# mohammadasim98/mv-ldm

Hardware: AMD Instinct MI355X
Metric: denoised views/sec @ 256x256, 4 views, 50 DDIM steps (higher is better)
Workload: dtype bf16

## Files before the change

### include/mvldm.h

```cpp
#ifndef MVLDM_H
#define MVLDM_H

#include <stddef.h>
#include <stdint.h>

#ifdef __cplusplus
extern "C" {
#endif

#define MVLDM_ABI_VERSION 7

typedef void* mvldm_stream_t;

enum { MVLDM_F32 = 0, MVLDM_BF16 = 1, MVLDM_F16 = 2 };
enum { MVLDM_OK = 0, MVLDM_ERR_ARG = -1, MVLDM_ERR_HIP = -2, MVLDM_ERR_UNSUPPORTED = -3 };

enum { MVLDM_EPI_NONE = 0, MVLDM_EPI_SILU = 1, MVLDM_EPI_GEGLU = 2, MVLDM_EPI_GELU = 3  };
enum { MVLDM_ELT_COPY = 0, MVLDM_ELT_SILU = 1, MVLDM_ELT_GELU = 2 };

int mvldm_abi_version(void);
int mvldm_build_flags(void);
const char* mvldm_last_error(void);
int mvldm_device_info(int* cu_count, size_t* hbm_bytes, char* arch, int arch_len);

typedef struct mvldm_igemm_desc {
    const void* src0;
    const void* src1;
    const void* weight;
    const float* bias;
    const float* row_bias;
    const void* residual;
    void* dst;
    float* workspace;
    int32_t c0, c1;
    int32_t n_img, h_in, w_in, h_out, w_out;
    int32_t ksize, stride, pad, upsample;
    int32_t n_out, n_pad, k_pad;
    int32_t row_bias_ld;
    int32_t epilogue;
    int32_t act_dtype;
    int32_t dst_dtype;
    int32_t splitk;
    int32_t tile;
    int32_t k_order;
    int32_t dst_ld;
    float out_scale;
    size_t workspace_bytes;
} mvldm_igemm_desc;
int mvldm_igemm_fwd(const mvldm_igemm_desc* d, mvldm_stream_t stream);
size_t mvldm_igemm_workspace_bytes(const mvldm_igemm_desc* d);

int mvldm_pack_weight(const float* src, void* dst, int n_out, int c_in, int ksize, int c_pad, int n_pad,
                      int k_pad, int geglu, int k_order, int dst_dtype, int transpose, int c_off, int n_rows,
                      mvldm_stream_t stream);

int mvldm_pack_skinny(const void* packed, void* dst, int n_pad, int k_pad, int geglu, int dtype, mvldm_stream_t stream);
int mvldm_igemm_skinny_config(const mvldm_igemm_desc* d);

typedef struct mvldm_pack_job {
    const float* src; void* dst;
    int n_out, c_in, ksize, c_pad, n_pad, k_pad, geglu, k_order, transpose, c_off, n_rows;
    int kind;
    int blocks;
    int block0;
} mvldm_pack_job;
int mvldm_pack_job_prepare(mvldm_pack_job* job , int dst_dtype);
int mvldm_pack_weight_batch(const mvldm_pack_job* jobs , int n_jobs, const int32_t* block_job, int total_blocks,
                            int dst_dtype, mvldm_stream_t stream);

#define MVLDM_GN_MAX_CHUNKS 32
int mvldm_groupnorm_fwd(const void* x0, const void* x1, void* y, const float* gamma, const float* beta, int n_img,
                        int hw, int c0, int c1, int groups, float eps, int silu, int dtype, void* stats_ws,
                        float* stats_out, mvldm_stream_t stream);
int mvldm_groupnorm_passes(int n_img, int hw, int c, int groups, int dtype);

int mvldm_layernorm_fwd(const void* x, void* y, const float* gamma, const float* beta, int rows, int c, float eps,
                        int dtype, mvldm_stream_t stream);

int mvldm_attention_fwd(const void* q, const void* k, const void* v, void* out, int ld_q, int ld_k, int ld_v,
                        int ld_o, int heads, int head_dim, const int32_t* seg, int n_seg, int max_q_len,
                        float scale, int dtype, float* lse, int lse_ld, mvldm_stream_t stream);

int mvldm_timestep_embed_fwd(const int64_t* timesteps, const float* freqs, void* out, int n, int dim,
                             int flip_sin_to_cos, int dst_dtype, mvldm_stream_t stream);

int mvldm_eltwise_fwd(const void* x, void* y, size_t n, int op, int src_dtype, int dst_dtype, mvldm_stream_t stream);

int mvldm_ddim_cfg_step(const float* eps, const float* x_t, float* x_next, const int32_t* cond_img,
                        const int32_t* uncond_img, int n_tgt, int hw, int c, float cfg_scale, const float* coef,
                        const int32_t* step_ptr, void* unet_in, int unet_in_c, int unet_in_dtype, int n_steps,
                        float clip_range, mvldm_stream_t stream);
int mvldm_ddpm_cfg_step(const float* eps_c, const float* eps_u, const float* x_t, const float* noise, float* x_next, size_t n,
                        float cfg_scale, const float* coef, float clip_range, mvldm_stream_t stream);
int mvldm_ddim_advance(int32_t* step_ptr, const int64_t* t_table, int n_steps, int64_t* timesteps,
                       const int32_t* tgt_rows, int n_rows, mvldm_stream_t stream);

int mvldm_nchw_to_nhwc(const float* src, void* dst, int n_img, int c, int hw, int dst_c, int dst_c_off,
                       int dst_dtype, float scale, float shift, const int32_t* img_map, mvldm_stream_t stream);
int mvldm_nhwc_to_nchw(const void* src, float* dst, int n_img, int c, int hw, int src_c, int src_c_off,
                       int src_dtype, float scale, float shift, int clamp01, mvldm_stream_t stream);

enum { MVLDM_RAYS_RAW = 0, MVLDM_RAYS_POSITIONAL = 1, MVLDM_RAYS_SRT = 2 };
int mvldm_ray_channels(int mode, int n_origin_octaves, int n_dir_octaves);
int mvldm_ray_encode(const float* extrinsics, const float* intrinsics, int n_cam, int h, int w, float* out_nchw,
                     void* out_nhwc, int nhwc_c, int nhwc_c_off, int nhwc_dtype, const int32_t* img_map, int mode,
                     int n_origin_octaves, int n_dir_octaves, int plucker, mvldm_stream_t stream);

int mvldm_posterior_sample(const float* moments, const float* noise, float* out, int n, int c, int hw, float scale,
                           mvldm_stream_t stream);


typedef struct mvldm_wgrad_desc {
    const void* src0; const void* src1; const void* dy;
    float* grad;
    float* workspace; size_t workspace_bytes;
    int32_t c0, c1, c_in;
    int32_t n_img, h_in, w_in, h_out, w_out;
    int32_t ksize, stride, pad, upsample;
    int32_t n_out, dy_ld;
    int32_t act_dtype;
    int32_t accumulate;
} mvldm_wgrad_desc;
int mvldm_igemm_wgrad(const mvldm_wgrad_desc* d, mvldm_stream_t stream);

int mvldm_colsum(const void* x, float* dst, float* workspace, size_t workspace_bytes, int n_seg, int rows_per_seg, int n,
                 int ld, int ld_dst, int per_seg, int accumulate, int dtype, mvldm_stream_t stream);

#define MVLDM_NORM_BWD_STORE 0x100
int mvldm_groupnorm_bwd(const void* x0, const void* x1, const void* dy, void* dx0, void* dx1, const float* gamma,
                        const float* beta, const float* stats, float* dgamma, float* dbeta, int n_img, int hw, int c0,
                        int c1, int groups, int silu, int dtype, float* workspace, size_t workspace_bytes,
                        mvldm_stream_t stream);
int mvldm_layernorm_bwd(const void* x, const void* dy, void* dx, const float* gamma, float* dgamma, float* dbeta,
                        int rows, int c, float eps, int dtype, float* workspace, size_t workspace_bytes,
                        mvldm_stream_t stream);

typedef struct mvldm_attn_bwd_desc {
    const void* q; const void* k; const void* v; const void* out; const void* dout;
    void* dq; void* dk; void* dv;
    const float* lse; float* delta;
    const int32_t* seg;
    int32_t ld_q, ld_k, ld_v, ld_o, ld_do, ld_dq, ld_dk, ld_dv;
    int32_t heads, head_dim, n_seg, max_q_len, max_kv_len, total_q_rows, stat_ld, dtype;
    float scale;
} mvldm_attn_bwd_desc;
int mvldm_attention_bwd(const mvldm_attn_bwd_desc* d, mvldm_stream_t stream);

enum { MVLDM_TE_SILU_BWD = 0, MVLDM_TE_ADD = 1, MVLDM_TE_GEGLU_FWD = 2, MVLDM_TE_GEGLU_BWD = 3, MVLDM_TE_GELU_BWD = 4 };
int mvldm_train_eltwise(int op, const void* a, const void* b, void* out, size_t rows, int d, int a_dtype, int dtype,
                        mvldm_stream_t stream);
int mvldm_pool2x2_sum(const void* du, void* dx, int n_img, int h, int w, int c, int dtype, mvldm_stream_t stream);
int mvldm_zero_insert2x(const void* x, void* out, int n_img, int h, int w, int c, int dtype, mvldm_stream_t stream);

int mvldm_add_noise(const float* x0, const float* noise, const float* coef, void* dst, int n, int c, int hw, int dst_c,
                    int dst_c_off, int dst_dtype, const int32_t* img_map, mvldm_stream_t stream);
int mvldm_mse_loss(const float* pred, const float* noise, const int32_t* tgt_img, int n_tgt, int hw, int c, float* loss,
                   int accumulate, float loss_scale, void* dpred, int dpred_c, int dpred_dtype, float grad_scale,
                   double* workspace, mvldm_stream_t stream);

typedef struct mvldm_amp_state {
    float scale;
    int32_t growth_tracker;
    int32_t adam_step;
    int32_t found_inf;
    int32_t skipped;
    int32_t reserved[3];
} mvldm_amp_state;
int mvldm_mse_loss_amp(const float* pred, const float* noise, const int32_t* tgt_img, int n_tgt, int hw, int c, float* loss,
                       int accumulate, float loss_scale, void* dpred, int dpred_c, int dpred_dtype, float grad_scale,
                       const float* amp_scale, double* workspace, mvldm_stream_t stream);

int mvldm_grad_norm(const float* g, size_t n, const float* sumsq_in, float max_norm, float* norm_out, double* workspace,
                    mvldm_stream_t stream);
int mvldm_adamw_step(float* p, const float* g, float* m, float* v, size_t n, float lr, float beta1, float beta2, float eps,
                     float weight_decay, int step, float grad_scale, const float* clip, mvldm_stream_t stream);
int mvldm_grad_norm_amp(const float* g, size_t n, const float* sumsq_in, float max_norm, float* norm_out, mvldm_amp_state* amp,
                        double* workspace, mvldm_stream_t stream);
int mvldm_adamw_step_amp(float* p, const float* g, float* m, float* v, size_t n, float lr, float beta1, float beta2, float eps,
                         float weight_decay, float grad_scale, const float* clip, const mvldm_amp_state* amp, mvldm_stream_t stream);
int mvldm_amp_update(mvldm_amp_state* amp, float growth_factor, float backoff_factor, int growth_interval, mvldm_stream_t stream);

int mvldm_ema_update(float* avg, const float* p, size_t n, float weight, mvldm_stream_t stream);

int mvldm_gather_rows(const void* src, void* dst, const int32_t* src_index, const int32_t* dst_index, int n_rows, size_t row_bytes,
                      mvldm_stream_t stream);

int mvldm_attention_merge(const void* oa, const float* lse_a, const void* ob, const float* lse_b, void* out, const int32_t* a_img,
                          const int32_t* b_img, const int32_t* out_img, int n_img, int tokens, int heads, int head_dim, int ld_a, int ld_b,
                          int ld_o, int lse_ld_a, int lse_ld_b, int dtype, mvldm_stream_t stream);

size_t mvldm_image_metrics_workspace_bytes(int n_img, int c, int h, int w);
int mvldm_image_metrics(const float* pred, const float* gt, int n_img, int c, int h, int w, int use_sample_covariance, float* psnr,
                        float* ssim, double* workspace, size_t workspace_bytes, mvldm_stream_t stream);

size_t mvldm_lpips_workspace_bytes(int n_img, int h, int w);
int mvldm_lpips_tap_slots(int h, int w, int c);
int mvldm_lpips_prep(const float* in0, const float* in1, void* dst, int n_img, int h, int w, int c_pad, int dtype, int normalize,
                     mvldm_stream_t stream);
int mvldm_lpips_relu(void* x, size_t n, int dtype, mvldm_stream_t stream);
int mvldm_lpips_tap(const void* feat, const float* weight, void* pooled, int n_img, int h, int w, int c, int dtype, double* workspace,
                    size_t workspace_bytes, int slot0, int slots_per_image, mvldm_stream_t stream);
int mvldm_lpips_fold(const double* workspace, size_t workspace_bytes, int n_img, int h, int w, float* out, mvldm_stream_t stream);

enum {
    MVLDM_OP_IGEMM = 1, MVLDM_OP_GROUPNORM, MVLDM_OP_LAYERNORM, MVLDM_OP_ATTENTION, MVLDM_OP_TIMESTEP_EMBED,
    MVLDM_OP_ELTWISE, MVLDM_OP_DDIM_STEP, MVLDM_OP_DDIM_ADVANCE, MVLDM_OP_NCHW_TO_NHWC, MVLDM_OP_NHWC_TO_NCHW,
    MVLDM_OP_MEMCPY, MVLDM_OP_RAY_ENCODE, MVLDM_OP_POSTERIOR_SAMPLE,
    MVLDM_OP_WGRAD, MVLDM_OP_ATTENTION_BWD, MVLDM_OP_GROUPNORM_BWD, MVLDM_OP_LAYERNORM_BWD, MVLDM_OP_COLSUM,
    MVLDM_OP_TRAIN_ELTWISE, MVLDM_OP_POOL2X2, MVLDM_OP_ZERO_INSERT, MVLDM_OP_ADD_NOISE, MVLDM_OP_MSE_LOSS, MVLDM_OP_FILL_ZERO,
    MVLDM_OP_PAR_BEGIN, MVLDM_OP_PAR_NEXT, MVLDM_OP_PAR_END,
// ... 68 lines not shown
```

### mv_ldm_amd/_lib.py

```python
from __future__ import annotations

import ctypes as C
from pathlib import Path

LIB_PATH = Path(__file__).resolve().parent / "csrc" / "libmvldm_hip.so"

ABI_VERSION = 7
F32, BF16, F16 = 0, 1, 2
EPI_NONE, EPI_SILU, EPI_GEGLU, EPI_GELU = 0, 1, 2, 3
RAYS_RAW, RAYS_POSITIONAL, RAYS_SRT = 0, 1, 2
ELT_COPY, ELT_SILU, ELT_GELU = 0, 1, 2
NORM_BWD_STORE = 0x100
GN_MAX_CHUNKS = 32

(OP_IGEMM, OP_GROUPNORM, OP_LAYERNORM, OP_ATTENTION, OP_TIMESTEP_EMBED, OP_ELTWISE, OP_DDIM_STEP, OP_DDIM_ADVANCE,
 OP_NCHW_TO_NHWC, OP_NHWC_TO_NCHW, OP_MEMCPY, OP_RAY_ENCODE, OP_POSTERIOR_SAMPLE,
 OP_WGRAD, OP_ATTENTION_BWD, OP_GROUPNORM_BWD, OP_LAYERNORM_BWD, OP_COLSUM, OP_TRAIN_ELTWISE, OP_POOL2X2, OP_ZERO_INSERT,
 OP_ADD_NOISE, OP_MSE_LOSS, OP_FILL_ZERO, OP_PAR_BEGIN, OP_PAR_NEXT, OP_PAR_END, OP_GATHER_ROWS, OP_ATTN_MERGE) = range(1, 30)
TE_SILU_BWD, TE_ADD, TE_GEGLU_FWD, TE_GEGLU_BWD, TE_GELU_BWD = 0, 1, 2, 3, 4

vp, i32, f32, sz = C.c_void_p, C.c_int32, C.c_float, C.c_size_t


class IgemmDesc(C.Structure):
# ... 10 lines not shown
class _GroupNorm(C.Structure):
    _fields_ = [("x", vp), ("x1", vp), ("y", vp), ("gamma", vp), ("beta", vp), ("stats_ws", vp),
                ("n_img", i32), ("hw", i32), ("c0", i32), ("c1", i32), ("groups", i32), ("silu", i32), ("dtype", i32),
                ("eps", f32), ("stats_out", vp)]


class _LayerNorm(C.Structure):
    _fields_ = [("x", vp), ("y", vp), ("gamma", vp), ("beta", vp), ("rows", i32), ("c", i32), ("dtype", i32), ("eps", f32)]


class _Attention(C.Structure):
    _fields_ = [("q", vp), ("k", vp), ("v", vp), ("out", vp), ("seg", vp),
                ("ld_q", i32), ("ld_k", i32), ("ld_v", i32), ("ld_o", i32), ("heads", i32), ("head_dim", i32),
                ("n_seg", i32), ("max_q_len", i32), ("dtype", i32), ("scale", f32), ("lse", vp), ("lse_ld", i32)]


class _Temb(C.Structure):
    _fields_ = [("timesteps", vp), ("freqs", vp), ("out", vp), ("n", i32), ("dim", i32), ("flip", i32), ("dst_dtype", i32)]


class _Eltwise(C.Structure):
    _fields_ = [("x", vp), ("y", vp), ("n", sz), ("op", i32), ("src_dtype", i32), ("dst_dtype", i32)]


class _Ddim(C.Structure):
    _fields_ = [("eps", vp), ("x_t", vp), ("x_next", vp), ("cond_img", vp), ("uncond_img", vp), ("coef", vp),
                ("step_ptr", vp), ("unet_in", vp),
                ("n_tgt", i32), ("hw", i32), ("c", i32), ("unet_in_c", i32), ("unet_in_dtype", i32), ("cfg_scale", f32),
                ("n_steps", i32), ("clip_range", f32)]


class _Advance(C.Structure):
    _fields_ = [("step_ptr", vp), ("t_table", vp), ("timesteps", vp), ("tgt_rows", vp), ("n_steps", i32), ("n_rows", i32)]


class _Layout(C.Structure):
    _fields_ = [("src", vp), ("dst", vp), ("n_img", i32), ("c", i32), ("hw", i32), ("other_c", i32),
                ("other_c_off", i32), ("dtype", i32), ("clamp01", i32), ("scale", f32), ("shift", f32), ("img_map", vp)]


class _Rays(C.Structure):
    _fields_ = [("extrinsics", vp), ("intrinsics", vp), ("out_nchw", vp), ("out_nhwc", vp), ("img_map", vp),
                ("n_cam", i32), ("h", i32), ("w", i32), ("nhwc_c", i32), ("nhwc_c_off", i32), ("nhwc_dtype", i32),
                ("mode", i32), ("n_origin_octaves", i32), ("n_dir_octaves", i32), ("plucker", i32)]


class _Posterior(C.Structure):
    _fields_ = [("moments", vp), ("noise", vp), ("out", vp), ("n", i32), ("c", i32), ("hw", i32), ("scale", f32)]


class _Memcpy(C.Structure):
    _fields_ = [("src", vp), ("dst", vp), ("bytes", sz)]


class _AttnMerge(C.Structure):
    _fields_ = [("oa", vp), ("ob", vp), ("out", vp), ("lse_a", vp), ("lse_b", vp), ("a_img", vp), ("b_img", vp), ("out_img", vp),
                ("n_img", i32), ("tokens", i32), ("heads", i32), ("head_dim", i32), ("ld_a", i32), ("ld_b", i32), ("ld_o", i32),
                ("lse_ld_a", i32), ("lse_ld_b", i32), ("dtype", i32)]


class _Gather(C.Structure):
    _fields_ = [("src", vp), ("dst", vp), ("src_index", vp), ("dst_index", vp), ("row_bytes", sz), ("n_rows", i32)]


class PackJob(C.Structure):
    _fields_ = [("src", vp), ("dst", vp), ("n_out", i32), ("c_in", i32), ("ksize", i32), ("c_pad", i32), ("n_pad", i32), ("k_pad", i32),
                ("geglu", i32), ("k_order", i32), ("transpose", i32), ("c_off", i32), ("n_rows", i32), ("kind", i32), ("blocks", i32),
                ("block0", i32)]


class WgradDesc(C.Structure):
    _fields_ = [("src0", vp), ("src1", vp), ("dy", vp), ("grad", vp), ("workspace", vp), ("workspace_bytes", sz),
                ("c0", i32), ("c1", i32), ("c_in", i32),
                ("n_img", i32), ("h_in", i32), ("w_in", i32), ("h_out", i32), ("w_out", i32),
                ("ksize", i32), ("stride", i32), ("pad", i32), ("upsample", i32),
                ("n_out", i32), ("dy_ld", i32), ("act_dtype", i32), ("accumulate", i32)]


class AttnBwdDesc(C.Structure):
    _fields_ = [("q", vp), ("k", vp), ("v", vp), ("out", vp), ("dout", vp), ("dq", vp), ("dk", vp), ("dv", vp),
                ("lse", vp), ("delta", vp), ("seg", vp),
                ("ld_q", i32), ("ld_k", i32), ("ld_v", i32), ("ld_o", i32), ("ld_do", i32), ("ld_dq", i32), ("ld_dk", i32), ("ld_dv", i32),
                ("heads", i32), ("head_dim", i32), ("n_seg", i32), ("max_q_len", i32), ("max_kv_len", i32), ("total_q_rows", i32),
                ("stat_ld", i32), ("dtype", i32), ("scale", f32)]


class _GroupNormBwd(C.Structure):
    _fields_ = [("x0", vp), ("x1", vp), ("dy", vp), ("dx0", vp), ("dx1", vp), ("gamma", vp), ("beta", vp), ("stats", vp),
                ("dgamma", vp), ("dbeta", vp), ("workspace", vp), ("workspace_bytes", sz),
                ("n_img", i32), ("hw", i32), ("c0", i32), ("c1", i32), ("groups", i32), ("silu", i32), ("dtype", i32)]


class _LayerNormBwd(C.Structure):
    _fields_ = [("x", vp), ("dy", vp), ("dx", vp), ("gamma", vp), ("dgamma", vp), ("dbeta", vp), ("workspace", vp),
                ("workspace_bytes", sz), ("rows", i32), ("c", i32), ("dtype", i32), ("eps", f32)]


class _Colsum(C.Structure):
    _fields_ = [("x", vp), ("dst", vp), ("workspace", vp), ("workspace_bytes", sz),
                ("n_seg", i32), ("rows_per_seg", i32), ("n", i32), ("ld", i32), ("ld_dst", i32), ("per_seg", i32),
                ("accumulate", i32), ("dtype", i32)]


class _TrainEltwise(C.Structure):
    _fields_ = [("a", vp), ("b", vp), ("out", vp), ("rows", sz), ("op", i32), ("d", i32), ("a_dtype", i32), ("dtype", i32)]


class _Resample(C.Structure):
    _fields_ = [("src", vp), ("dst", vp), ("n_img", i32), ("h", i32), ("w", i32), ("c", i32), ("dtype", i32)]


class _AddNoise(C.Structure):
    _fields_ = [("x0", vp), ("noise", vp), ("coef", vp), ("dst", vp), ("img_map", vp),
                ("n", i32), ("c", i32), ("hw", i32), ("dst_c", i32), ("dst_c_off", i32), ("dst_dtype", i32)]


class _Mse(C.Structure):
    _fields_ = [("pred", vp), ("noise", vp), ("tgt_img", vp), ("loss", vp), ("dpred", vp), ("workspace", vp),
                ("n_tgt", i32), ("hw", i32), ("c", i32), ("accumulate", i32), ("dpred_c", i32), ("dpred_dtype", i32),
                ("loss_scale", f32), ("grad_scale", f32), ("amp_scale", vp)]


class AmpState(C.Structure):
    _fields_ = [("scale", f32), ("growth_tracker", i32), ("adam_step", i32), ("found_inf", i32), ("skipped", i32), ("reserved", i32 * 3)]


class _Fill(C.Structure):
    _fields_ = [("dst", vp), ("bytes", sz)]


class _OpUnion(C.Union):
    _fields_ = [("igemm", IgemmDesc), ("groupnorm", _GroupNorm), ("layernorm", _LayerNorm), ("attention", _Attention),
                ("temb", _Temb), ("eltwise", _Eltwise), ("ddim", _Ddim), ("advance", _Advance), ("layout", _Layout),
                ("memcpy_", _Memcpy), ("gather", _Gather), ("attn_merge", _AttnMerge), ("rays", _Rays), ("posterior", _Posterior),
                ("wgrad", WgradDesc), ("attention_bwd", AttnBwdDesc), ("groupnorm_bwd", _GroupNormBwd),
                ("layernorm_bwd", _LayerNormBwd), ("colsum", _Colsum), ("train_eltwise", _TrainEltwise), ("resample", _Resample),
                ("add_noise", _AddNoise), ("mse", _Mse), ("fill", _Fill)]


class Op(C.Structure):
    _fields_ = [("kind", i32), ("tag", i32), ("u", _OpUnion)]


SIGNATURES = {
    "mvldm_abi_version": (C.c_int, []),
    "mvldm_build_flags": (C.c_int, []),
    "mvldm_last_error": (C.c_char_p, []),
    "mvldm_device_info": (C.c_int, [C.POINTER(C.c_int), C.POINTER(sz), C.c_char_p, C.c_int]),
    "mvldm_igemm_fwd": (C.c_int, [C.POINTER(IgemmDesc), vp]),
    "mvldm_igemm_workspace_bytes": (sz, [C.POINTER(IgemmDesc)]),
    "mvldm_pack_weight": (C.c_int, [vp, vp] + [C.c_int] * 12 + [vp]),
    "mvldm_pack_skinny": (C.c_int, [vp, vp, C.c_int, C.c_int, C.c_int, C.c_int, vp]),
    "mvldm_igemm_skinny_config": (C.c_int, [C.POINTER(IgemmDesc)]),
    "mvldm_pack_job_prepare": (C.c_int, [C.POINTER(PackJob), C.c_int]),
    "mvldm_pack_weight_batch": (C.c_int, [vp, C.c_int, vp, C.c_int, C.c_int, vp]),
    "mvldm_groupnorm_fwd": (C.c_int, [vp, vp, vp, vp, vp, C.c_int, C.c_int, C.c_int, C.c_int, C.c_int, f32, C.c_int, C.c_int, vp, vp, vp]),
    "mvldm_groupnorm_passes": (C.c_int, [C.c_int] * 5),
    "mvldm_layernorm_fwd": (C.c_int, [vp, vp, vp, vp, C.c_int, C.c_int, f32, C.c_int, vp]),
    "mvldm_attention_fwd": (C.c_int, [vp, vp, vp, vp] + [C.c_int] * 6 + [vp, C.c_int, C.c_int, f32, C.c_int, vp, C.c_int, vp]),
    "mvldm_igemm_wgrad": (C.c_int, [C.POINTER(WgradDesc), vp]),
    "mvldm_colsum": (C.c_int, [vp, vp, vp, sz] + [C.c_int] * 8 + [vp]),
    "mvldm_groupnorm_bwd": (C.c_int, [vp] * 10 + [C.c_int] * 7 + [vp, sz, vp]),
    "mvldm_layernorm_bwd": (C.c_int, [vp] * 6 + [C.c_int, C.c_int, f32, C.c_int, vp, sz, vp]),
    "mvldm_attention_bwd": (C.c_int, [C.POINTER(AttnBwdDesc), vp]),
    "mvldm_train_eltwise": (C.c_int, [C.c_int, vp, vp, vp, sz, C.c_int, C.c_int, C.c_int, vp]),
    "mvldm_pool2x2_sum": (C.c_int, [vp, vp] + [C.c_int] * 5 + [vp]),
    "mvldm_zero_insert2x": (C.c_int, [vp, vp] + [C.c_int] * 5 + [vp]),
    "mvldm_add_noise": (C.c_int, [vp, vp, vp, vp] + [C.c_int] * 6 + [vp, vp]),
    "mvldm_mse_loss": (C.c_int, [vp, vp, vp, C.c_int, C.c_int, C.c_int, vp, C.c_int, f32, vp, C.c_int, C.c_int, f32, vp, vp]),
    "mvldm_grad_norm": (C.c_int, [vp, sz, vp, f32, vp, vp, vp]),
    "mvldm_adamw_step": (C.c_int, [vp, vp, vp, vp, sz, f32, f32, f32, f32, f32, C.c_int, f32, vp, vp]),
    "mvldm_mse_loss_amp": (C.c_int, [vp, vp, vp, C.c_int, C.c_int, C.c_int, vp, C.c_int, f32, vp, C.c_int, C.c_int, f32, vp, vp, vp]),
    "mvldm_grad_norm_amp": (C.c_int, [vp, sz, vp, f32, vp, vp, vp, vp]),
    "mvldm_adamw_step_amp": (C.c_int, [vp, vp, vp, vp, sz, f32, f32, f32, f32, f32, f32, vp, vp, vp]),
    "mvldm_amp_update": (C.c_int, [vp, f32, f32, C.c_int, vp]),
    "mvldm_timestep_embed_fwd": (C.c_int, [vp, vp, vp, C.c_int, C.c_int, C.c_int, C.c_int, vp]),
    "mvldm_eltwise_fwd": (C.c_int, [vp, vp, sz, C.c_int, C.c_int, C.c_int, vp]),
    "mvldm_ddim_cfg_step": (C.c_int, [vp, vp, vp, vp, vp, C.c_int, C.c_int, C.c_int, f32, vp, vp, vp, C.c_int, C.c_int, C.c_int, f32, vp]),
    "mvldm_ddim_advance": (C.c_int, [vp, vp, C.c_int, vp, vp, C.c_int, vp]),
    "mvldm_gather_rows": (C.c_int, [vp, vp, vp, vp, C.c_int, sz, vp]),
    "mvldm_attention_merge": (C.c_int, [vp] * 8 + [C.c_int] * 10 + [vp]),
    "mvldm_ddpm_cfg_step": (C.c_int, [vp, vp, vp, vp, vp, sz, f32, vp, f32, vp]),
    "mvldm_ema_update": (C.c_int, [vp, vp, sz, f32, vp]),
    "mvldm_image_metrics_workspace_bytes": (sz, [C.c_int] * 4),
    "mvldm_image_metrics": (C.c_int, [vp, vp] + [C.c_int] * 5 + [vp, vp, vp, sz, vp]),
    "mvldm_lpips_workspace_bytes": (sz, [C.c_int] * 3),
    "mvldm_lpips_tap_slots": (C.c_int, [C.c_int] * 3),
    "mvldm_lpips_prep": (C.c_int, [vp, vp, vp] + [C.c_int] * 6 + [vp]),
    "mvldm_lpips_relu": (C.c_int, [vp, sz, C.c_int, vp]),
    "mvldm_lpips_tap": (C.c_int, [vp, vp, vp] + [C.c_int] * 5 + [vp, sz, C.c_int, C.c_int, vp]),
    "mvldm_lpips_fold": (C.c_int, [vp, sz, C.c_int, C.c_int, C.c_int, vp, vp]),
    "mvldm_nchw_to_nhwc": (C.c_int, [vp, vp] + [C.c_int] * 6 + [f32, f32, vp, vp]),
    "mvldm_ray_channels": (C.c_int, [C.c_int, C.c_int, C.c_int]),
    "mvldm_ray_encode": (C.c_int, [vp, vp, C.c_int, C.c_int, C.c_int, vp, vp, C.c_int, C.c_int, C.c_int, vp] + [C.c_int] * 4 + [vp]),
    "mvldm_posterior_sample": (C.c_int, [vp, vp, vp, C.c_int, C.c_int, C.c_int, f32, vp]),
    "mvldm_nhwc_to_nchw": (C.c_int, [vp, vp] + [C.c_int] * 6 + [f32, f32, C.c_int, vp]),
    "mvldm_op_run": (C.c_int, [C.POINTER(Op), vp]),
    "mvldm_plan_create": (C.c_int, [C.POINTER(Op), C.c_int, C.POINTER(vp)]),
    "mvldm_plan_num_ops": (C.c_int, [vp]),
    "mvldm_plan_run": (C.c_int, [vp, vp]),
    "mvldm_plan_run_range": (C.c_int, [vp, C.c_int, C.c_int, vp]),
    "mvldm_plan_capture": (C.c_int, [vp, vp]),
    "mvldm_plan_replay": (C.c_int, [vp, vp]),
    "mvldm_plan_profile": (C.c_int, [vp, vp, C.c_int, C.POINTER(f32)]),
    "mvldm_plan_destroy": (None, [vp]),
}

_lib = None


class MvldmError(RuntimeError):
    pass


_EXPERIMENT_KNOBS = ("MVLDM_ADAMW_NT", "MVLDM_ATTN_QB", "MVLDM_ATTN_WIDE_VALU", "MVLDM_GN_NTHR", "MVLDM_GN_SPAN", "MVLDM_GN_TWOPASS", "MVLDM_GN_WIDE",
                     "MVLDM_IGEMM_FAKE", "MVLDM_IGEMM_GROUP", "MVLDM_IGEMM_NOSTAGE", "MVLDM_IGEMM_PX", "MVLDM_IGEMM_SYNC", "MVLDM_IGEMM_TARGET",
                     "MVLDM_LPP_CPT", "MVLDM_LPP_FAKE", "MVLDM_PLAN_SERIAL", "MVLDM_PW_FAKE", "MVLDM_PW_GM", "MVLDM_PW_TN", "MVLDM_RS_FAKE", "MVLDM_SK_FAKE",
                     "MVLDM_STREAM_STORES", "MVLDM_WGRAD_DIRECT", "MVLDM_WGRAD_TARGET", "MVLDM_WGRAD_WIDE", "MVLDM_WGRAD_WIDE_BP",
                     "MVLDM_WGRAD_WIDE_TARGET", "MVLDM_WGRAD_XCD", "MVLDM_WS_FAKE")


def load(required: bool = True):
    global _lib
    if _lib is not None:
        return _lib
    if not LIB_PATH.exists():
        if required:
            raise MvldmError(f"{LIB_PATH} is missing: run `python -c 'import __graft_entry__ as g; g.build()'` "
                             "(there is no CPU / PyTorch fallback for the HIP path)")
        return None
    lib = C.CDLL(str(LIB_PATH))
    for name, (res, args) in SIGNATURES.items():
        fn = getattr(lib, name)
        fn.restype, fn.argtypes = res, args
    if lib.mvldm_abi_version() != ABI_VERSION:
        raise MvldmError("libmvldm_hip.so ABI version mismatch")
    if not (lib.mvldm_build_flags() & 1) and "_exp" not in LIB_PATH.name:
        import os
        stale = sorted(k for k in _EXPERIMENT_KNOBS if k in os.environ)
        if stale:
            raise MvldmError(f"{', '.join(stale)} set, but {LIB_PATH.name} was built without -DMVLDM_EXPERIMENTS and ignores it: build an "
                             "experiment library (MVLDM_EXPERIMENTS=1 python -m mv_ldm_amd._build --force, or tools/*_probe.sh + --lib) or unset it")
    _lib = lib
    return lib


def check(rc: int):
    if rc != 0:
        raise MvldmError(f"mvldm error {rc}: {load().mvldm_last_error().decode()}")
```

### mv_ldm_amd/csrc/igemm.hip

```cpp
#include <algorithm>
#include <cstdio>
#include <cstdlib>

#include "igemm_common.h"

namespace mvldm {

template <typename T> __global__ __launch_bounds__(256) void igemm_splitk_reduce(const IgemmParams p) {
    const bool geglu = p.epilogue == MVLDM_EPI_GEGLU;
    const size_t total = (size_t)p.M * p.n_dst;
    const size_t slab = (size_t)p.M * p.n_pad;
    for (size_t idx = (size_t)blockIdx.x * 256 + threadIdx.x; idx < total; idx += (size_t)gridDim.x * 256) {
        const int m = (int)(idx / p.n_dst), col = (int)(idx - (size_t)m * p.n_dst);
        float v;
        if (geglu) {
            const int nv = (col >> 5) * 64 + (col & 31), ng = nv + 32;
            float a = 0.f, g = 0.f;
            for (int s = 0; s < p.splitk; ++s) {
                a += p.ws[s * slab + (size_t)m * p.n_pad + nv];
                g += p.ws[s * slab + (size_t)m * p.n_pad + ng];
            }
            if (p.bias) { a += p.bias[col]; g += p.bias[p.n_dst + col]; }
            v = a * gelu_erf_fast(g);
        } else {
            float a = 0.f;
            for (int s = 0; s < p.splitk; ++s) a += p.ws[s * slab + (size_t)m * p.n_pad + col];
            if (p.bias) a += p.bias[col];
            if (p.row_bias) a += p.row_bias[(size_t)(m / p.hw_out) * p.row_bias_ld + col];
            if (p.epilogue == MVLDM_EPI_SILU) a = silu_f(a);
            else if (p.epilogue == MVLDM_EPI_GELU) a = gelu_erf_fast(a);
            v = a;
        }
        epilogue_store<T, true>(p, m, col, v);
    }
}

template <typename T> __global__ __launch_bounds__(256) void igemm_splitk_reduce_vec(const IgemmParams p) {
    const bool geglu = p.epilogue == MVLDM_EPI_GEGLU;
    const int cpr = p.n_dst / 8;
    const size_t total = (size_t)p.M * cpr;
    const size_t slab = (size_t)p.M * p.n_pad;
    for (size_t idx = (size_t)blockIdx.x * 256 + threadIdx.x; idx < total; idx += (size_t)gridDim.x * 256) {
        const int m = (int)(idx / cpr), col = (int)(idx - (size_t)m * cpr) * 8;
        const int nv = geglu ? (col >> 5) * 64 + (col & 31) : col;
        const float* w0 = p.ws + (size_t)m * p.n_pad + nv;
        float a[8], g[8];
#pragma unroll
        for (int e = 0; e < 8; ++e) a[e] = g[e] = 0.f;
        int s = 0;
        for (; s + 4 <= p.splitk; s += 4) {
            f32x4 lo[4], hi[4], gl[4], gh[4];
#pragma unroll
            for (int u = 0; u < 4; ++u) {
                lo[u] = *reinterpret_cast<const f32x4*>(w0 + (s + u) * slab);
                hi[u] = *reinterpret_cast<const f32x4*>(w0 + (s + u) * slab + 4);
                if (geglu) {
                    gl[u] = *reinterpret_cast<const f32x4*>(w0 + (s + u) * slab + 32);
                    gh[u] = *reinterpret_cast<const f32x4*>(w0 + (s + u) * slab + 36);
                }
            }
#pragma unroll
            for (int u = 0; u < 4; ++u) {
#pragma unroll
                for (int e = 0; e < 4; ++e) { a[e] += lo[u][e]; a[4 + e] += hi[u][e]; }
                if (geglu) {
#pragma unroll
                    for (int e = 0; e < 4; ++e) { g[e] += gl[u][e]; g[4 + e] += gh[u][e]; }
                }
            }
        }
        for (; s < p.splitk; ++s) {
            const f32x4 lo = *reinterpret_cast<const f32x4*>(w0 + s * slab), hi = *reinterpret_cast<const f32x4*>(w0 + s * slab + 4);
#pragma unroll
            for (int e = 0; e < 4; ++e) { a[e] += lo[e]; a[4 + e] += hi[e]; }
            if (geglu) {
                const f32x4 gl = *reinterpret_cast<const f32x4*>(w0 + s * slab + 32), gh = *reinterpret_cast<const f32x4*>(w0 + s * slab + 36);
#pragma unroll
                for (int e = 0; e < 4; ++e) { g[e] += gl[e]; g[4 + e] += gh[e]; }
            }
        }
        if (p.bias) {
#pragma unroll
            for (int e = 0; e < 8; ++e) a[e] += p.bias[col + e];
        }
        if (geglu) {
#pragma unroll
            for (int e = 0; e < 8; ++e) a[e] *= gelu_erf_fast(g[e] + (p.bias ? p.bias[p.n_dst + col + e] : 0.f));
        } else {
            if (p.row_bias) {
                const float* rb = p.row_bias + (size_t)(m / p.hw_out) * p.row_bias_ld + col;
#pragma unroll
                for (int e = 0; e < 8; ++e) a[e] += rb[e];
            }
            if (p.epilogue == MVLDM_EPI_SILU) {
#pragma unroll
                for (int e = 0; e < 8; ++e) a[e] = silu_f(a[e]);
            } else if (p.epilogue == MVLDM_EPI_GELU) {
#pragma unroll
                for (int e = 0; e < 8; ++e) a[e] = gelu_erf_fast(a[e]);
            }
        }
#pragma unroll
        for (int e = 0; e < 8; ++e) a[e] *= p.out_scale;
        if (p.residual) {
            const Chunk<T> rc = load_chunk<T>(reinterpret_cast<const T*>(p.residual) + (size_t)m * p.n_dst + col);
#pragma unroll
            for (int e = 0; e < 8; ++e) a[e] += rc.get(e);
        }
        size_t drow = (size_t)m;
        if (p.scatter) {
            const int img = m / p.hw_out, rem = m - img * p.hw_out;
            const int i = rem / p.w_out, j = rem - i * p.w_out;
            drow = ((size_t)img * (2 * p.h_out) + 2 * i + p.ph_y) * (size_t)(2 * p.w_out) + 2 * j + p.ph_x;
        }
        Chunk<T> oc;
#pragma unroll
        for (int e = 0; e < 8; ++e) oc.set(e, a[e]);
        store_chunk<T>(reinterpret_cast<T*>(p.dst) + drow * p.dst_ld + col, oc);
    }
}

static int env_int(const char* name, int dflt) { return knob_int(name, dflt); }
static const int kEnvTarget = env_int("MVLDM_IGEMM_TARGET", 0);
static const int kEnvSync = env_int("MVLDM_IGEMM_SYNC", 0);
static const int kEnvPx = env_int("MVLDM_IGEMM_PX", 0);
static const int kEnvNoStage = env_int("MVLDM_IGEMM_NOSTAGE", 0);
#ifdef MVLDM_EXPERIMENTS
static const int kEnvFake = env_int("MVLDM_IGEMM_FAKE", 0);
#else
static constexpr int kEnvFake = 0;
#endif

static thread_local int t_force_sync = 0;

static int launch_igemm(const IgemmParams& p, int tile, int act_dtype, hipStream_t s) {
    if (tile >= 1 && tile <= 5) return igemm_launch_small(p, tile, act_dtype, s);
    if (tile >= 6 && tile <= 8) return igemm_launch_large(p, tile, act_dtype, s);
    if (tile == 9 || tile == 10 || tile == 18) return igemm_launch_xl(p, tile, act_dtype, s);
    if (tile == 11 || tile == 17) return igemm_launch_halo(p, tile, act_dtype, s);
    return set_error(MVLDM_ERR_ARG, "igemm: bad tile %d", tile);
}


static void choose_config(const mvldm_igemm_desc& d, int M, int k_tiles, int& tile, int& splitk, size_t ws_bytes) {
    const int target = kEnvTarget ? kEnvTarget : 512;
    if (tile == 0) {
        const bool can10 = d.act_dtype != MVLDM_F32 && d.k_order == 1 && d.dst_dtype != MVLDM_F32 && d.n_pad % 320 == 0 &&
                           d.epilogue != MVLDM_EPI_GEGLU && d.upsample != 1 && d.n_out % 8 == 0 && (d.dst_ld <= 0 || d.dst_ld % 8 == 0) &&
                           !(d.ksize == 3 && d.src1);
        const int wgs10 = cdiv(M, 256) * (d.n_pad / 320);
        const double eff10 = (double)wgs10 / (256.0 * cdiv(wgs10, 256));
        if (can10 && (wgs10 >= 1024 || (wgs10 >= 512 && (eff10 >= 0.9 || d.ksize == 1)))) tile = 10;
        else if (M <= 32) tile = 5;
        else if (M <= 64) tile = 4;
        else if (d.ksize >= 2) tile = cdiv(M, 256) * cdiv(d.n_pad, 128) >= 300 ? 7 : 2;
        else if (d.n_pad >= 768 && d.act_dtype != MVLDM_F32 && d.k_order == 1 && d.dst_dtype != MVLDM_F32 &&
                 cdiv(M, 256) * cdiv(d.n_pad, 256) >= 1024)
            tile = 9;
        else if (d.k_pad >= 1024 && d.n_pad >= 1024 && cdiv(M, 128) * cdiv(d.n_pad, 256) >= 300) tile = 8;
        else tile = d.n_pad < 640 ? 2 : 3;
    }
    const int tm = cdiv(M, kTiles[tile].bm), tn = cdiv(d.n_pad, kTiles[tile].bn);
    if (splitk == 0) {
        splitk = 1;
        const int wgs = tm * tn;
        if (wgs < target) splitk = std::min(std::max(k_tiles / 4, 1), cdiv(target, wgs));
        if (d.workspace == nullptr) splitk = 1;
        while (splitk > 1 && (size_t)splitk * M * d.n_pad * sizeof(float) > ws_bytes) --splitk;
    }
    splitk = std::max(1, std::min(splitk, k_tiles));
}

static int fill_params(const mvldm_igemm_desc& d, IgemmParams& p, int& tile) {
    const int epc = d.act_dtype == MVLDM_F32 ? 4 : 8;
    const int bk = d.act_dtype == MVLDM_F32 ? 32 : 64;
    MVLDM_REQUIRE(d.src0 && d.weight && d.dst, "igemm: null pointer");
    const bool phase = d.upsample >= 2;
    MVLDM_REQUIRE(d.upsample >= 0 && d.upsample <= 5, "igemm: upsample %d", d.upsample);
    MVLDM_REQUIRE(phase ? (d.ksize == 2 && d.stride == 1 && d.h_out == d.h_in && d.w_out == d.w_in && !d.src1 && !d.residual &&
                           !d.row_bias && d.act_dtype != MVLDM_F32 && d.dst_dtype == d.act_dtype && d.k_order == 1)
                        : (d.ksize == 1 || d.ksize == 3),
                  "igemm: ksize %d / upsample %d", d.ksize, d.upsample);
    MVLDM_REQUIRE(d.stride == 1 || d.stride == 2, "igemm: stride %d", d.stride);
    MVLDM_REQUIRE(d.c0 % epc == 0 && d.c1 % epc == 0 && d.c0 > 0, "igemm: channels (%d,%d) must be multiples of %d", d.c0, d.c1, epc);
    MVLDM_REQUIRE((d.c1 == 0) == (d.src1 == nullptr), "igemm: src1/c1 mismatch");
    MVLDM_REQUIRE(d.k_pad % bk == 0 && d.k_pad >= d.ksize * d.ksize * (d.c0 + d.c1), "igemm: k_pad %d", d.k_pad);
    MVLDM_REQUIRE(d.n_pad % 64 == 0 && d.n_pad >= d.n_out, "igemm: n_pad %d (n_out %d)", d.n_pad, d.n_out);
    MVLDM_REQUIRE(d.dst_dtype == d.act_dtype || d.dst_dtype == MVLDM_F32, "igemm: dst dtype");
    if (d.epilogue == MVLDM_EPI_GEGLU)
        MVLDM_REQUIRE(d.n_out % 64 == 0 && !d.row_bias, "igemm: GEGLU needs n_out %% 64 == 0");
    p.src0 = d.src0; p.src1 = d.src1; p.weight = d.weight; p.bias = d.bias; p.row_bias = d.row_bias;
    p.residual = d.residual; p.dst = d.dst; p.ws = d.workspace;
    p.c0 = d.c0; p.c1 = d.c1; p.ctot = d.c0 + d.c1;
    p.n_img = d.n_img; p.h_in = d.h_in; p.w_in = d.w_in; p.h_out = d.h_out; p.w_out = d.w_out;
    p.hw_out = d.h_out * d.w_out;
    p.ksize = d.ksize; p.stride = d.stride; p.pad = d.pad; p.upsample = phase ? 0 : d.upsample; p.taps = d.ksize * d.ksize;
    p.scatter = phase; p.ph_y = phase ? (d.upsample - 2) >> 1 : 0; p.ph_x = phase ? (d.upsample - 2) & 1 : 0;
    p.ty0 = phase ? p.ph_y - 1 : -d.pad; p.tx0 = phase ? p.ph_x - 1 : -d.pad;
    p.cy = phase ? 1 - p.ph_y : d.ksize / 2; p.cx = phase ? 1 - p.ph_x : d.ksize / 2;
    p.M = d.n_img * p.hw_out; p.n_out = d.n_out; p.n_pad = d.n_pad; p.k_pad = d.k_pad;
    p.n_dst = d.epilogue == MVLDM_EPI_GEGLU ? d.n_out / 2 : d.n_out;
    p.rb_vec = d.row_bias && ((uintptr_t)d.row_bias % 16 == 0) && d.row_bias_ld % 4 == 0;
    p.bias_vec = d.bias && ((uintptr_t)d.bias % 16 == 0);
    p.row_bias_ld = d.row_bias_ld; p.epilogue = d.epilogue; p.dst_f32 = d.dst_dtype == MVLDM_F32;
    p.out_scale = d.out_scale;
    p.dst_ld = d.dst_ld > 0 ? d.dst_ld : p.n_dst;
    MVLDM_REQUIRE(p.dst_ld >= p.n_dst, "igemm: dst_ld %d < n_dst %d", p.dst_ld, p.n_dst);
    p.k_tiles = d.k_pad / bk;
    tile = d.tile & 63;
    t_force_sync = (d.tile >> 12) & 1;
    const int force_px = (d.tile >> 8) & 15;
    int splitk = d.splitk;
    MVLDM_REQUIRE(((tile >= 0 && tile <= kNumTiles) || tile == 17 || deep_tile(tile)) && splitk >= 0, "igemm: tile/splitk");
    choose_config(d, p.M, p.k_tiles, tile, splitk, d.workspace_bytes);
    if (splitk > 1)
        MVLDM_REQUIRE(d.workspace && (size_t)splitk * p.M * d.n_pad * sizeof(float) <= d.workspace_bytes,
                      "igemm: split-K workspace too small");
    const double es = 2.0;
    const double b0 = (double)d.n_img * d.h_in * d.w_in * d.c0 * es, b1 = (double)d.n_img * d.h_in * d.w_in * d.c1 * es;
    const double bw = (double)d.n_pad * d.k_pad * es;
    p.use_bl = d.act_dtype != MVLDM_F32 && d.k_order == 1 && !t_force_sync && !kEnvSync &&
               b0 < 4.0e9 && b1 < 4.0e9 && bw < 4.0e9;
    if (d.act_dtype != MVLDM_F32 && d.k_order == 1 && !t_force_sync && !kEnvSync && !p.use_bl) {
        static bool warned = false;
        if (!warned) {
            warned = true;
            fprintf(stderr, "[mvldm] igemm: operand of %.2f GB exceeds the 4 GB range of the fast 16-bit loop; using the slower "
                            "64-bit-address loop (split the batch to avoid this)\n", std::max(std::max(b0, b1), bw) / 1e9);
        }
    }
    p.src0_bytes = (unsigned)b0; p.src1_bytes = (unsigned)b1; p.w_bytes = (unsigned)bw;
    p.fake = kEnvFake;
    p.nt_store = stream_stores((size_t)p.M * (size_t)p.n_dst * (p.dst_f32 || d.act_dtype == MVLDM_F32 ? 4 : 2));
    if (kEnvFake & 1) p.src0_bytes = p.src1_bytes = 0;
    if (kEnvFake & 2) p.w_bytes = 0;
    if (tile >= 6 && !p.use_bl) tile = 2;
    if (deep_tile(tile) && d.upsample) tile = 2;
    p.splitk = splitk;
    if (p.use_bl) {
        const int cbs = p.k_tiles / p.taps;
        const int per = cdiv(cbs, std::min(splitk, cbs));
        p.k_tiles_per_split = per * p.taps;
        p.splitk = cdiv(cbs, per);
    } else {
        p.k_tiles_per_split = cdiv(p.k_tiles, splitk);
        p.splitk = cdiv(p.k_tiles, p.k_tiles_per_split);
    }
    p.stage_epi = d.act_dtype != MVLDM_F32 && !kEnvNoStage && (p.splitk > 1 || (!p.dst_f32 && p.n_dst % 8 == 0 && p.dst_ld % 8 == 0));
    if (tile >= 9 && tile <= 10 && (!p.stage_epi || (tile == 10 && d.epilogue == MVLDM_EPI_GEGLU))) tile = 7;
    if (tile == 11 && !(p.use_bl && p.stage_epi && p.splitk == 1 && d.ksize == 3 && d.stride == 1 && d.pad == 1 && !d.upsample &&
                        d.h_out == d.h_in && d.w_out == d.w_in && halo_rows_for(d.w_in) <= 384 && halo_smem(d.w_in) <= 160 * 1024))
        tile = 7;
    if (tile == 17 && !(p.use_bl && p.stage_epi && p.splitk == 1 && d.ksize == 3 && d.stride == 1 && d.pad == 1 && !d.upsample && d.c1 == 0 &&
                        d.h_out == d.h_in && d.w_out == d.w_in && d.epilogue != MVLDM_EPI_GEGLU && halow_smem(d.w_in) <= 160 * 1024))
        tile = 7;
    if (phase) {
        MVLDM_REQUIRE(p.use_bl && p.stage_epi, "igemm: 2x2 phase conv needs the lean 16-bit loop and an 8-aligned 16-bit output");
        if (tile != 7 && tile != 10) tile = 2;
    }
    if (p.use_bl && d.upsample == 1 && tile != 7) tile = 2;
    if (p.use_bl && d.upsample != 1) {
        const int hc = (d.h_out - 1) * d.stride + p.ty0 + p.cy, wc = (d.w_out - 1) * d.stride + p.tx0 + p.cx;
        MVLDM_REQUIRE(p.ty0 + p.cy >= 0 && p.tx0 + p.cx >= 0 && hc < d.h_in && wc < d.w_in,
                      "igemm: conv geometry (pad %d, stride %d) not supported", d.pad, d.stride);
    }
    p.tiles_m = cdiv(p.M, kTiles[tile].bm);
    p.tiles_n = cdiv(d.n_pad, kTiles[tile].bn);
    p.korder = d.k_order;
    if (d.k_order)
        MVLDM_REQUIRE(d.k_order == 1 && p.ctot % bk == 0 && d.c0 % bk == 0 && d.k_pad == p.taps * p.ctot,
                      "igemm: k_order 1 needs channel counts (%d,%d) multiples of %d", d.c0, d.c1, bk);
    {
        const double a_bytes = (double)d.n_img * d.h_in * d.w_in * p.ctot, w_bytes = (double)d.n_pad * d.k_pad;
        double best = 1e300;
        for (int px = 1; px <= 8; px *= 2) {
            const int py = 8 / px;
            const int sm = cdiv(p.tiles_m, px), sn = cdiv(p.tiles_n, py);
            const double waste = (double)(8 * sm * sn) / ((double)p.tiles_m * p.tiles_n);
            const double cost = (py * a_bytes + px * w_bytes) * waste * waste;
            if (cost < best) { best = cost; p.px = px; p.sub_m = sm; p.sub_n = sn; }
        }
        p.m_fast = w_bytes >= a_bytes;
        const int fpx = force_px ? force_px : kEnvPx;
        if (fpx > 0 && fpx <= 8 && (8 % fpx) == 0) {
            p.px = fpx; p.sub_m = cdiv(p.tiles_m, p.px); p.sub_n = cdiv(p.tiles_n, 8 / p.px);
        }
        p.grp_m = p.grp_n = 1;
        static const int kGroup = knob_int("MVLDM_IGEMM_GROUP", -1);
        if (kGroup != 0 && ((tile >= 7 && tile <= 10) || tile == 17) && p.sub_m * p.sub_n > 32) {
            const double ax = a_bytes / p.px, wx = w_bytes / (8 / p.px);
            double bestc = 1e300;
            for (int gm = 1; gm <= 32; gm *= 2) {
                if (kGroup > 0 && gm != kGroup) continue;
                const int gme = std::min(gm, p.sub_m), gne = std::min(32 / gm, p.sub_n);
                const double c = ax * cdiv(p.sub_n, gne) + wx * cdiv(p.sub_m, gme);
                if (c < bestc) { bestc = c; p.grp_m = gme; p.grp_n = gne; }
            }
        }
    }
    return MVLDM_OK;
}

int linear_pp_run(const mvldm_igemm_desc& d, hipStream_t s);
int linear_pw_run(const mvldm_igemm_desc& d, hipStream_t s);
int linear_ws_run(const mvldm_igemm_desc& d, hipStream_t s);
int skinny_run(const mvldm_igemm_desc& d, hipStream_t s);
int linear_rs_run(const mvldm_igemm_desc& d, hipStream_t s);

int igemm_run(const mvldm_igemm_desc& d, hipStream_t s) {
    IgemmParams p;
    int tile = 0;
    if (d.n_img == 0 || d.h_out == 0 || d.w_out == 0) return MVLDM_OK;
    const int req = d.tile & 63;
    if (req == 15) return skinny_run(d, s);
    if (req == 12 || req == 13 || req == 14 || req == 19) {
        MVLDM_REQUIRE(d.src0 && d.weight && d.dst, "igemm: null pointer");
        return req == 12 ? linear_pp_run(d, s) : req == 13 ? linear_pw_run(d, s) : req == 14 ? linear_ws_run(d, s) : linear_rs_run(d, s);
    }
    MVLDM_REQUIRE(d.k_order != 2, "igemm: the fragment-order pack (k_order 2) is read by tile 15 only");
    int rc = fill_params(d, p, tile);
    if (rc) return rc;
    if (p.M == 0) return MVLDM_OK;
    rc = dispatch_dtype(d.act_dtype, [&](auto t) {
        using T = decltype(t);
        int r = launch_igemm(p, tile, Elt<T>::DT, s);
        if (r) return r;
        if (p.splitk > 1) {
            if constexpr (sizeof(T) == 2) {
                if (!p.dst_f32 && p.n_dst % 8 == 0 && p.dst_ld % 8 == 0 && ((uintptr_t)p.ws % 16) == 0 &&
                    (!p.residual || ((uintptr_t)p.residual % 16) == 0) && ((uintptr_t)p.dst % 16) == 0) {
                    const size_t chunks = (size_t)p.M * (p.n_dst / 8);
                    hipLaunchKernelGGL(igemm_splitk_reduce_vec<T>, dim3((unsigned)std::min<size_t>((chunks + 255) / 256, 4096)), dim3(256), 0, s, p);
                    return check_launch();
                }
            }
            const size_t total = (size_t)p.M * p.n_dst;
            const int blocks = (int)std::min<size_t>((total + 255) / 256, 4096);
            hipLaunchKernelGGL(igemm_splitk_reduce<T>, dim3(blocks), dim3(256), 0, s, p);
            return check_launch();
        }
        return (int)MVLDM_OK;
    });
    return rc;
}

}

using namespace mvldm;

extern "C" int mvldm_igemm_fwd(const mvldm_igemm_desc* d, mvldm_stream_t stream) {
    MVLDM_REQUIRE(d != nullptr, "igemm: null desc");
    return igemm_run(*d, (hipStream_t)stream);
}

extern "C" size_t mvldm_igemm_workspace_bytes(const mvldm_igemm_desc* d) {
    if (!d) return 0;
    const size_t M = (size_t)d->n_img * d->h_out * d->w_out;
    return (size_t)16 * M * d->n_pad * sizeof(float);
}
```

### mv_ldm_amd/csrc/igemm_bl.h

```cpp
#pragma once
#include "igemm_common.h"

namespace mvldm {

template <typename T, int BM, int BN, int WM, int WN>
__global__ __launch_bounds__(WM* WN * 64) void igemm_kernel(const IgemmParams p) {
    using M_ = Mma<T>;
    constexpr int NT = WM * WN * 64;
    constexpr int EPC = Elt<T>::EPC;
    constexpr int BK = M_::BK;
    constexpr int TM = BM / WM / 32, TN = BN / WN / 32;
    constexpr int A_BYTES = BM * M_::PITCH, B_BYTES = BN * M_::PITCH;
    constexpr int A_IT = BM * 8 / NT, B_IT = BN * 8 / NT;
    static_assert(A_IT >= 1 && B_IT >= 1 && TM >= 1 && TN >= 1, "bad tile");
    extern __shared__ __attribute__((aligned(16))) char smem[];

    const int tid = threadIdx.x, lane = tid & 63, wave = tid >> 6;
    const int wm = wave / WN, wn = wave % WN;
    const int hi = lane >> 5, l31 = lane & 31;

    int split, tm, tn;
    if (!map_block(p, split, tm, tn)) return;
    const int kt0 = split * p.k_tiles_per_split;
    const int kt1 = min(kt0 + p.k_tiles_per_split, p.k_tiles);
// ... 31 lines not shown
        const bool tap_ok = tap < p.taps;
        const int ky = tap / p.ksize, kx = tap - ky * p.ksize;
        const bool from0 = c < p.c0;
        const T* sbase = from0 ? reinterpret_cast<const T*>(p.src0) + c
                               : reinterpret_cast<const T*>(p.src1) + (c - p.c0);
        const int cs = from0 ? p.c0 : p.c1;
#pragma unroll
        for (int it = 0; it < A_IT; ++it) {
            int iy = a_y[it] + ky, ix = a_x[it] + kx;
            const bool ok = tap_ok && a_img[it] >= 0 && iy >= 0 && iy < hs && ix >= 0 && ix < wsz;
            if (p.upsample) { iy >>= 1; ix >>= 1; }
            if (ok) {
                const size_t off = ((size_t)(a_img[it] * p.h_in + iy) * p.w_in + ix) * cs;
                areg[it] = *reinterpret_cast<const u32x4*>(sbase + off);
            } else {
                areg[it] = u32x4{0u, 0u, 0u, 0u};
            }
        }
#pragma unroll
        for (int it = 0; it < B_IT; ++it) {
            const int n = tn * BN + r0 + it * (NT / 8);
            if (n < p.n_pad)
                breg[it] = *reinterpret_cast<const u32x4*>(wbase + (size_t)it * (NT / 8) * p.k_pad + (size_t)kt * BK);
            else
                breg[it] = u32x4{0u, 0u, 0u, 0u};
        }
    };
    auto store_tile = [&](int stage) {
        char* at = smem + stage * (A_BYTES + B_BYTES);
        char* bt = at + A_BYTES;
#pragma unroll
        for (int it = 0; it < A_IT; ++it) M_::store(at, r0 + it * (NT / 8), kc, areg[it]);
#pragma unroll
        for (int it = 0; it < B_IT; ++it) M_::store(bt, r0 + it * (NT / 8), kc, breg[it]);
    };

    f32x16 acc[TM][TN];
#pragma unroll
    for (int i = 0; i < TM; ++i)
#pragma unroll
        for (int j = 0; j < TN; ++j)
#pragma unroll
            for (int r = 0; r < 16; ++r) acc[i][j][r] = 0.f;

    if (kt0 < kt1) {
        load_tile(kt0);
        store_tile(0);
    }
    __syncthreads();
    int cur = 0;
    for (int kt = kt0; kt < kt1; ++kt) {
        const bool more = kt + 1 < kt1;
        if (more) load_tile(kt + 1);
        const char* at = smem + cur * (A_BYTES + B_BYTES);
        const char* bt = at + A_BYTES;
#pragma unroll
        for (int kk = 0; kk < BK / M_::KI; ++kk) {
            typename M_::Frag a[TM], b[TN];
#pragma unroll
            for (int i = 0; i < TM; ++i) a[i] = M_::load(at, wm * (BM / WM) + i * 32 + l31, kk, hi);
#pragma unroll
            for (int j = 0; j < TN; ++j) b[j] = M_::load(bt, wn * (BN / WN) + j * 32 + l31, kk, hi);
#pragma unroll
            for (int i = 0; i < TM; ++i)
#pragma unroll
                for (int j = 0; j < TN; ++j) acc[i][j] = M_::mma(a[i], b[j], acc[i][j]);
        }
        if (more) store_tile(cur ^ 1);
        __syncthreads();
        cur ^= 1;
    }

    if constexpr (sizeof(T) == 2) {
        if (p.stage_epi) {
            igemm_epilogue_staged<T, BM, BN, WM, WN>(p, acc, tm, tn, split, wm, wn, wave, lane, smem);
            return;
        }
    }
    igemm_epilogue<T, BM, BN, WM, WN>(p, acc, tm, tn, split, wm, wn, hi, l31);
}


template <int TAPS, int A_IT, bool DUAL, bool UPS> struct BlAddr {
    unsigned a0[UPS ? TAPS : 1][A_IT];
    unsigned a1[DUAL ? (UPS ? TAPS : 1) : 1][DUAL ? A_IT : 1];
    unsigned mask[UPS ? 1 : A_IT];
};

template <typename T, int BM, int BN, int NW, int KS, bool DUAL, int A_IT, int B_IT, int STAGES, bool UPS, int t, int LO = 0, int HI = 1 << 20>
__device__ __forceinline__ void bl_issue(const IgemmParams& p, char* stage_base, int wave, int cb,
                                         const BlAddr<KS * KS, A_IT, DUAL, UPS>& ad, const unsigned (&vb)[B_IT]) {
    constexpr int BK = 64, TAPS = KS * KS;
    const int lead = (!UPS && KS > 1) ? p.w_in + 1 : 0;
    const int disp = UPS ? 0 : (t / KS - p.cy) * p.w_in + (t % KS - p.cx) + lead;
    const unsigned lead0 = (unsigned)lead * (unsigned)p.c0 * 2u, lead1 = (unsigned)lead * (unsigned)p.c1 * 2u;
    const __amdgpu_buffer_rsrc_t r0 = __builtin_amdgcn_make_buffer_rsrc(
        const_cast<char*>(reinterpret_cast<const char*>(p.src0)) - lead0, 0, p.src0_bytes + lead0, 0x00020000);
    const __amdgpu_buffer_rsrc_t r1 = __builtin_amdgcn_make_buffer_rsrc(
        const_cast<char*>(reinterpret_cast<const char*>(DUAL ? p.src1 : p.src0)) - (DUAL ? lead1 : lead0), 0,
        DUAL ? p.src1_bytes + lead1 : p.src0_bytes + lead0, 0x00020000);
    const __amdgpu_buffer_rsrc_t rw = __builtin_amdgcn_make_buffer_rsrc(const_cast<void*>(p.weight), 0, p.w_bytes, 0x00020000);
    char* at = stage_base;
    char* bt = at + BM * 128;
    const int c = cb * BK;
    const bool from0 = !DUAL || c < p.c0;
    const int soff = ((from0 ? c : c - p.c0) + disp * (from0 ? p.c0 : p.c1)) * 2;
#pragma unroll
    for (int it = (LO > 0 ? LO : 0); it < (HI < A_IT ? HI : A_IT); ++it) {
        __attribute__((address_space(3))) void* dst = (__attribute__((address_space(3))) void*)(at + (wave + NW * it) * 1024);
        unsigned v0, v1;
        if constexpr (UPS) {
            v0 = ad.a0[t][it];
            v1 = ad.a1[DUAL ? t : 0][DUAL ? it : 0];
        } else {
            const bool ok = (ad.mask[it] >> t) & 1u;
            v0 = ok ? ad.a0[0][it] : kBufOob;
            v1 = ok ? ad.a1[0][DUAL ? it : 0] : kBufOob;
        }
        if (from0) __builtin_amdgcn_raw_ptr_buffer_load_lds(r0, dst, 16, v0, soff, 0, 0);
        else __builtin_amdgcn_raw_ptr_buffer_load_lds(r1, dst, 16, v1, soff, 0, 0);
    }
    const int koff = (cb * TAPS + t) * (BK * 2);
#pragma unroll
    for (int it = (LO > A_IT ? LO - A_IT : 0); it < (HI - A_IT < B_IT ? HI - A_IT : B_IT); ++it)
        __builtin_amdgcn_raw_ptr_buffer_load_lds(rw, (__attribute__((address_space(3))) void*)(bt + (wave + NW * it) * 1024), 16,
                                                 vb[it], koff, 0, 0);
}

template <typename T, int BM, int BN, int WM, int WN>
__device__ __forceinline__ void bl_compute(const char* stage_base, f32x16 (&acc)[BM / WM / 32][BN / WN / 32], int wm, int wn,
                                           int hi, int l31) {
    constexpr int TM = BM / WM / 32, TN = BN / WN / 32;
#pragma unroll
    for (int kk = 0; kk < 64 / Mma<T>::KI; ++kk) {
        BlFrags<T, TM, TN> f;
        bl_load<T, BM, BN, WM, WN>(stage_base, f, kk, wm, wn, hi, l31);
        bl_mma<T, TM, TN>(f, acc);
    }
}

template <int LPT, int MAXY>
__device__ __forceinline__ void bl_wait_young(int young) {
    if constexpr (MAXY >= 1) {
        if (young >= MAXY) {
            asm volatile("s_waitcnt vmcnt(%0) lgkmcnt(0)" ::"n"(MAXY * LPT) : "memory");
            return;
        }
        bl_wait_young<LPT, MAXY - 1>(young);
    } else {
        asm volatile("s_waitcnt vmcnt(0) lgkmcnt(0)" ::: "memory");
    }
}

template <typename T, int BM, int BN, int WM, int WN, int KS, bool DUAL, int STAGES, bool UPS>
__global__ __launch_bounds__(WM* WN * 64) void igemm_bl_kernel(const IgemmParams p) {
    using M_ = Mma<T>;
    static_assert(sizeof(T) == 2, "16-bit activation types only");
    constexpr int NW = WM * WN, TAPS = KS * KS;
    constexpr int BK = 64, EPC = 8;
    constexpr int TM = BM / WM / 32, TN = BN / WN / 32;
    constexpr int A_BYTES = BM * 128, B_BYTES = BN * 128, STAGE_BYTES = A_BYTES + B_BYTES;
    constexpr int A_IT = BM / 8 / NW, B_IT = BN / 8 / NW, LPT = A_IT + B_IT;
    static_assert(A_IT >= 1 && B_IT >= 1 && (BM / 8) % NW == 0 && (BN / 8) % NW == 0, "bad tile");
    static_assert(STAGES >= 2 && STAGES <= 8, "ring depth");
    extern __shared__ __attribute__((aligned(16))) char smem[];

    const auto [lane, wave, wm, wn, hi, l31] = wave_lane<WN>();
    int split, tm, tn;
    if (!map_block(p, split, tm, tn)) return;
    const int cb0 = split * (p.k_tiles_per_split / TAPS);
    const int cb1 = min(cb0 + p.k_tiles_per_split / TAPS, p.k_tiles / TAPS);

    const int slot = lane & 7, rsub = lane >> 3;
    BlAddr<TAPS, A_IT, DUAL, UPS> ad;
#pragma unroll
    for (int it = 0; it < A_IT; ++it) {
        const int row = (wave + NW * it) * 8 + rsub;
        const int m = tm * BM + row;
        const unsigned chunk = (unsigned)((slot ^ ((row >> 1) & 7)) * EPC);
        const bool live = m < p.M;
        const int img = live ? m / p.hw_out : 0, rem = live ? m - img * p.hw_out : 0;
        const int oy = rem / p.w_out, ox = rem - oy * p.w_out;
        if constexpr (UPS) {
            const unsigned hs = 2 * p.h_in, wsz = 2 * p.w_in;
            const int y0 = live ? oy * p.stride - p.pad : -(1 << 20), x0 = ox * p.stride - p.pad;
#pragma unroll
            for (int t = 0; t < TAPS; ++t) {
                const int iy = y0 + t / KS, ix = x0 + t % KS;
                const bool ok = (unsigned)iy < hs && (unsigned)ix < wsz;
                const unsigned pix = (unsigned)(img * p.h_in + (iy >> 1)) * (unsigned)p.w_in + (unsigned)(ix >> 1);
                ad.a0[t][it] = ok ? (pix * (unsigned)p.c0 + chunk) * 2u : kBufOob;
                if constexpr (DUAL) ad.a1[t][it] = ok ? (pix * (unsigned)p.c1 + chunk) * 2u : kBufOob;
            }
        } else {
            const int yc = oy * p.stride + p.ty0 + p.cy, xc = ox * p.stride + p.tx0 + p.cx;
            const unsigned pix = (unsigned)(img * p.h_in + yc) * (unsigned)p.w_in + (unsigned)xc;
            unsigned msk = 0;
#pragma unroll
            for (int t = 0; t < TAPS; ++t) {
                const int iy = yc + t / KS - p.cy, ix = xc + t % KS - p.cx;
                msk |= (live && (unsigned)iy < (unsigned)p.h_in && (unsigned)ix < (unsigned)p.w_in) ? (1u << t) : 0u;
            }
            ad.a0[0][it] = (pix * (unsigned)p.c0 + chunk) * 2u;
            if constexpr (DUAL) ad.a1[0][it] = (pix * (unsigned)p.c1 + chunk) * 2u;
            ad.mask[it] = msk;
        }
    }
    unsigned vb[B_IT];
#pragma unroll
    for (int it = 0; it < B_IT; ++it) {
        const int row = (wave + NW * it) * 8 + rsub;
        const int n = tn * BN + row;
        const unsigned chunk = (unsigned)((slot ^ ((row >> 1) & 7)) * EPC);
        vb[it] = n < p.n_pad ? ((unsigned)n * (unsigned)p.k_pad + chunk) * 2u : kBufOob;
    }

    f32x16 acc[TM][TN];
#pragma unroll
    for (int i = 0; i < TM; ++i)
#pragma unroll
        for (int j = 0; j < TN; ++j)
#pragma unroll
            for (int r = 0; r < 16; ++r) acc[i][j][r] = 0.f;

#define MVLDM_BL_ISSUE(stage_, cb_, t_) \
    bl_issue<T, BM, BN, NW, KS, DUAL, A_IT, B_IT, STAGES, UPS, t_>(p, smem + (stage_) * STAGE_BYTES, wave, cb_, ad, vb)
#define MVLDM_BL_ISSUE_R(stage_, cb_, t_, lo_, hi_) \
    bl_issue<T, BM, BN, NW, KS, DUAL, A_IT, B_IT, STAGES, UPS, t_, lo_, hi_>(p, smem + (stage_) * STAGE_BYTES, wave, cb_, ad, vb)
#define MVLDM_BL_NEXT(t_, d_) (((t_) + (d_)) % TAPS)
#define MVLDM_BL_LOAD(f_, slot_, kk_) bl_load<T, BM, BN, WM, WN>(smem + (slot_) * STAGE_BYTES, f_, kk_, wm, wn, hi, l31)
#define MVLDM_BL_MMA(f_)                  \
    __builtin_amdgcn_sched_barrier(0);    \
    bl_mma<T, TM, TN>(f_, acc);           \
    __builtin_amdgcn_sched_barrier(0);
#define MVLDM_BL_STEP(t_)                                                                                         \
    {                                                                                                             \
        static_assert(64 / M_::KI == 4, "four k-sub-steps per K-tile");                                          \
        MVLDM_BL_LOAD(f1, slot_c, 1);                                                                             \
        MVLDM_BL_MMA(f0)                                                                                          \
        MVLDM_BL_LOAD(f0, slot_c, 2);                                                                             \
        MVLDM_BL_MMA(f1)                                                                                          \
        MVLDM_BL_LOAD(f1, slot_c, 3);                                                                             \
        MVLDM_BL_MMA(f0)                                                                                          \
            \
                             \
        if (STAGES == 3 && cb + ((t_) + 2) / TAPS < cb1) asm volatile("s_waitcnt vmcnt(%0) lgkmcnt(0)" ::"n"(LPT) : "memory"); \
        else asm volatile("s_waitcnt vmcnt(0) lgkmcnt(0)" ::: "memory");                                          \
        __builtin_amdgcn_s_barrier();                                                                             \
        {                                                                                                         \
                   \
            const int cbn_ = cb + ((t_) + STAGES) / TAPS;                                                         \
            if (cbn_ < cb1) { MVLDM_BL_ISSUE(slot_c, cbn_, MVLDM_BL_NEXT(t_, STAGES)); }                          \
        }                                                                                                         \
        slot_c = slot_c + 1 == STAGES ? 0 : slot_c + 1;                                                           \
        MVLDM_BL_LOAD(f0, slot_c, 0);                                                                             \
        MVLDM_BL_MMA(f1)                                                                                          \
    }
#ifdef MVLDM_BL_BURST
    constexpr bool SPREAD_S = false;
#elif defined(MVLDM_BL_SPREAD_ALL)
    constexpr bool SPREAD_S = true;
#else
    constexpr bool SPREAD_S = NW == 8;
#endif
#define MVLDM_BL_STEP_SIMPLE(t_)                                                                                  \
    {                                                                                                             \
        asm volatile("s_waitcnt vmcnt(0) lgkmcnt(0)" ::: "memory");                                               \
        __builtin_amdgcn_s_barrier();                                                                             \
        if constexpr (!SPREAD_S) {                                                                                \
            const int cbn_ = cb + ((t_) + 1) / TAPS;                                                              \
            if (cbn_ < cb1) { MVLDM_BL_ISSUE(slot_c ^ 1, cbn_, MVLDM_BL_NEXT(t_, 1)); }                           \
            bl_compute<T, BM, BN, WM, WN>(smem + slot_c * STAGE_BYTES, acc, wm, wn, hi, l31);                     \
        } else {                                                                                                  \
            constexpr int Q0_ = (4 * LPT + 8) / 9, Q1_ = Q0_ + (LPT - Q0_ + 1) / 2;                              \
            const int cbn_ = cb + ((t_) + 1) / TAPS;                                                              \
            const bool more_ = cbn_ < cb1;                                                                        \
            if (more_) { MVLDM_BL_ISSUE_R(slot_c ^ 1, cbn_, MVLDM_BL_NEXT(t_, 1), 0, Q0_); }                      \
            {                                                                                                     \
                BlFrags<T, TM, TN> fs_;                                                                           \
                MVLDM_BL_LOAD(fs_, slot_c, 0);                                                                    \
                bl_mma<T, TM, TN>(fs_, acc);                                                                      \
            }                                                                                                     \
            if (more_) { MVLDM_BL_ISSUE_R(slot_c ^ 1, cbn_, MVLDM_BL_NEXT(t_, 1), Q0_, Q1_); }                    \
            {                                                                                                     \
                BlFrags<T, TM, TN> fs_;                                                                           \
                MVLDM_BL_LOAD(fs_, slot_c, 1);                                                                    \
                bl_mma<T, TM, TN>(fs_, acc);                                                                      \
            }                                                                                                     \
            if (more_) { MVLDM_BL_ISSUE_R(slot_c ^ 1, cbn_, MVLDM_BL_NEXT(t_, 1), Q1_, LPT); }                    \
            {                                                                                                     \
                BlFrags<T, TM, TN> fs_;                                                                           \
                MVLDM_BL_LOAD(fs_, slot_c, 2);                                                                    \
                bl_mma<T, TM, TN>(fs_, acc);                                                                      \
                MVLDM_BL_LOAD(fs_, slot_c, 3);                                                                    \
                bl_mma<T, TM, TN>(fs_, acc);                                                                      \
            }                                                                                                     \
        }                                                                                                         \
        slot_c ^= 1;                                                                                              \
    }
#define MVLDM_BL_STEP_DEEP(t_)                                                                                    \
    {                                                                                                             \
        bl_wait_young<LPT, STAGES - 2>((cb1 - cb) * TAPS - (t_) - 1);       \
        __builtin_amdgcn_s_barrier();                                       \
        {                                                                                                         \
            const int cbn_ = cb + ((t_) + STAGES - 1) / TAPS;                                                     \
            if (cbn_ < cb1) { MVLDM_BL_ISSUE(slot_c == 0 ? STAGES - 1 : slot_c - 1, cbn_, MVLDM_BL_NEXT(t_, STAGES - 1)); } \
        }                                                                                                         \
        bl_compute<T, BM, BN, WM, WN>(smem + slot_c * STAGE_BYTES, acc, wm, wn, hi, l31);                         \
        slot_c = slot_c + 1 == STAGES ? 0 : slot_c + 1;                                                           \
    }
#define MVLDM_BL_PRO(j_)                                                                                          \
    if constexpr (STAGES - 1 > (j_)) {                                                                            \
        if (cb0 + (j_) / TAPS < cb1) { MVLDM_BL_ISSUE((j_), cb0 + (j_) / TAPS, ((j_) % TAPS)); }                  \
    }
    constexpr bool PIPE = NW == 8 && TM * TN <= 8 && STAGES <= 3;
    if constexpr (STAGES > 3) {
        static_assert((STAGES - 2) * LPT <= 63, "vmcnt is a 6-bit counter");
        if (cb0 < cb1) {
            MVLDM_BL_ISSUE(0, cb0, 0);
            MVLDM_BL_PRO(1) MVLDM_BL_PRO(2) MVLDM_BL_PRO(3) MVLDM_BL_PRO(4) MVLDM_BL_PRO(5) MVLDM_BL_PRO(6)
            int slot_c = 0;
            for (int cb = cb0; cb < cb1; ++cb) {
// ... 122 lines not shown
```

### mv_ldm_amd/csrc/skinny.hip

```cpp
#include <algorithm>
#include <cstdio>
#include <cstdlib>
#include <cstring>

#include "common.h"

namespace mvldm {

struct SkParams {
    const void* src0; const void* src1; const void* w;
    const float* bias; const float* row_bias; const void* residual; void* dst;
    int c0, c1;
    int n_img, h_in, w_in, hw_in, h_out, w_out, hw_out;
    int stride, ty0, tx0, ksize;
    int M, n_out, n_dst, dst_ld, row_bias_ld, rb_hw;
    int epilogue, dst_f32;
    float out_scale;
    int n_tiles;
    int n_groups, m_groups, G;
    int n_cbs, cb0;
    int n_stages;
    int ksteps;
    int scatter, ph_y, ph_x;
    int hw_sh, w_sh, rb_sh;
// ... 519 lines not shown
                    for (int jn = 0; jn < NT; ++jn) acc[i][jn] = SkMma<T>::mma(*reinterpret_cast<Frag*>(&wr[j][it][jn]), bq[it & 1][i], acc[i][jn]);
                __builtin_amdgcn_sched_barrier(0);
                iw_issue_w<C>(p, wr[j][it], cb_next, it, lane, tile0);
            }
            iw_issue_a<C>(p, a_voff, a_voff1, wb + j * C::SLOT, cb_next);
        }
    }
#ifdef MVLDM_EXPERIMENTS
    if (p.fake & 16) return;
#endif
    __builtin_amdgcn_s_waitcnt(waitcnt_vmcnt(0));
    __syncthreads();
#pragma unroll
    for (int i = 0; i < MT; ++i)
#pragma unroll
        for (int j = 0; j < NT; ++j) *reinterpret_cast<f32x4*>(smem + ((wave * MT + i) * NT + j) * 1024 + lane * 16) = acc[i][j];
    __syncthreads();
    epi.finish(p, smem, tid, tile0, row0, rows);
}

__global__ __launch_bounds__(256) void pack_skinny_kernel(const u32x4* __restrict__ src, u32x4* __restrict__ dst, int n_tiles, int ksteps, int geglu) {
    const size_t total = (size_t)n_tiles * ksteps * 64;
    for (size_t u = (size_t)blockIdx.x * 256 + threadIdx.x; u < total; u += (size_t)gridDim.x * 256) {
        const int lane = (int)(u & 63);
        const size_t f = u >> 6;
        const int kg = (int)(f % ksteps), nt = (int)(f / ksteps);
        int row;
        if (geglu) { const int q = nt >> 1, gate = nt & 1; row = (q >> 1) * 64 + gate * 32 + (q & 1) * 16 + (lane & 15); }
        else row = nt * 16 + (lane & 15);
        dst[u] = src[(size_t)row * (ksteps * 4) + 4 * kg + (lane >> 4)];
    }
}

struct SkinnyCfgInfo { int taps, nw, sc, mt, nt, ds, sm, bal; };
static const SkinnyCfgInfo kSkCfgs[] = {
    {0, 0, 0, 0, 0, 0, 0, 0},
    {9, 9, 1, 3, 1, 10, 1, 0},
    {9, 9, 1, 4, 1, 10, 1, 0},
    {0, 0, 0, 0, 0, 0, 0, 0}, {0, 0, 0, 0, 0, 0, 0, 0},
    {9, 9, 1, 3, 1, 5, 4, 0},
    {4, 8, 2, 3, 1, 5, 1, 0},
    {4, 8, 2, 4, 1, 5, 1, 0},
    {1, 8, 4, 3, 4, 5, 1, 0},
    {1, 8, 4, 3, 2, 5, 1, 0},
    {1, 8, 4, 1, 4, 5, 1, 0},
    {0, 0, 0, 0, 0, 0, 0, 0},
    {1, 8, 4, 3, 1, 5, 1, 0},
    {1, 4, 2, 6, 2, 5, 1, 0},
    {0, 0, 0, 0, 0, 0, 0, 0}, {0, 0, 0, 0, 0, 0, 0, 0},
    {0, 0, 0, 0, 0, 0, 0, 0},
    {0, 0, 0, 0, 0, 0, 0, 0},
    {9, 9, 1, 12, 1, 3, 1, 0},
    {4, 8, 2, 12, 1, 3, 1, 0},
    {1, 8, 4, 1, 2, 5, 1, 0},
    {0, 0, 0, 0, 0, 0, 0, 0}, {0, 0, 0, 0, 0, 0, 0, 0}, {0, 0, 0, 0, 0, 0, 0, 0}, {0, 0, 0, 0, 0, 0, 0, 0}, {0, 0, 0, 0, 0, 0, 0, 0}, {0, 0, 0, 0, 0, 0, 0, 0},
    {0, 0, 0, 0, 0, 0, 0, 0}, {0, 0, 0, 0, 0, 0, 0, 0}, {0, 0, 0, 0, 0, 0, 0, 0}, {0, 0, 0, 0, 0, 0, 0, 0}, {0, 0, 0, 0, 0, 0, 0, 0},
    {0, 0, 0, 0, 0, 0, 0, 0}, {0, 0, 0, 0, 0, 0, 0, 0}, {0, 0, 0, 0, 0, 0, 0, 0}, {0, 0, 0, 0, 0, 0, 0, 0}, {0, 0, 0, 0, 0, 0, 0, 0}, {0, 0, 0, 0, 0, 0, 0, 0},
    {1, 4, 0, 3, 1, 5, 1, 0},
    {1, 4, 0, 3, 2, 5, 1, 0},
    {1, 4, 0, 3, 4, 5, 1, 0},
    {1, 4, 0, 1, 2, 5, 1, 0},
    {1, 4, 0, 1, 4, 5, 1, 0},
    {1, 8, 0, 3, 1, 2, 1, 0},
    {1, 4, 0, 6, 2, 2, 1, 0},
    {0, 0, 0, 0, 0, 0, 0, 0},
    {1, 8, 0, 3, 2, 2, 1, 0},
};
constexpr int kNumSkCfgs = sizeof(kSkCfgs) / sizeof(kSkCfgs[0]);

template <typename T, typename C> static int sk_launch(const SkParams& p, int grid, hipStream_t s) {
    static std::atomic<uint64_t> done{0};
    if (int rc0 = ensure_dyn_smem(reinterpret_cast<const void*>(skinny_kernel<T, C>), C::SMEM, done)) return rc0;
    hipLaunchKernelGGL((skinny_kernel<T, C>), dim3(grid), dim3(C::NW * 64), C::SMEM, s, p);
    return check_launch();
}

template <typename T, typename C> static int iw_launch(const SkParams& p, int grid, hipStream_t s) {
    static std::atomic<uint64_t> done{0};
    if (int rc0 = ensure_dyn_smem(reinterpret_cast<const void*>(skinny_iws_kernel<T, C>), C::SMEM, done)) return rc0;
    hipLaunchKernelGGL((skinny_iws_kernel<T, C>), dim3(grid), dim3(C::NW * 64), C::SMEM, s, p);
    return check_launch();
}

template <typename T> static int sk_dispatch(int cfg, const SkParams& p, int grid, hipStream_t s) {
    if (p.c1 > 0) {
        switch (cfg) {
            case 38: return iw_launch<T, IwCfg<1, 4, 3, 1, 5, 1, true>>(p, grid, s);
            case 39: return iw_launch<T, IwCfg<1, 4, 3, 2, 5, 1, true>>(p, grid, s);
            case 40: return iw_launch<T, IwCfg<1, 4, 3, 4, 5, 1, true>>(p, grid, s);
            case 44: return iw_launch<T, IwCfg<1, 4, 6, 2, 2, 1, true>>(p, grid, s);
            case 8: return sk_launch<T, SkCfg<1, 8, 4, 3, 4, 5, 1, true>>(p, grid, s);
            case 9: return sk_launch<T, SkCfg<1, 8, 4, 3, 2, 5, 1, true>>(p, grid, s);
            case 10: return sk_launch<T, SkCfg<1, 8, 4, 1, 4, 5, 1, true>>(p, grid, s);
            case 12: return sk_launch<T, SkCfg<1, 8, 4, 3, 1, 5, 1, true>>(p, grid, s);
            case 13: return sk_launch<T, SkCfg<1, 4, 2, 6, 2, 5, 1, true>>(p, grid, s);
            case 20: return sk_launch<T, SkCfg<1, 8, 4, 1, 2, 5, 1, true>>(p, grid, s);
            default: return set_error(MVLDM_ERR_UNSUPPORTED, "igemm: tile 15: configuration %d does not take two sources", cfg);
        }
    }
    switch (cfg) {
        case 1: return sk_launch<T, SkCfg<9, 9, 1, 3, 1, 10, 1>>(p, grid, s);
        case 2: return sk_launch<T, SkCfg<9, 9, 1, 4, 1, 10, 1>>(p, grid, s);
        case 5: return sk_launch<T, SkCfg<9, 9, 1, 3, 1, 5, 4>>(p, grid, s);
        case 6: return sk_launch<T, SkCfg<4, 8, 2, 3, 1, 5, 1>>(p, grid, s);
        case 7: return sk_launch<T, SkCfg<4, 8, 2, 4, 1, 5, 1>>(p, grid, s);
        case 8: return sk_launch<T, SkCfg<1, 8, 4, 3, 4, 5, 1>>(p, grid, s);
        case 9: return sk_launch<T, SkCfg<1, 8, 4, 3, 2, 5, 1>>(p, grid, s);
        case 10: return sk_launch<T, SkCfg<1, 8, 4, 1, 4, 5, 1>>(p, grid, s);
        case 12: return sk_launch<T, SkCfg<1, 8, 4, 3, 1, 5, 1>>(p, grid, s);
        case 13: return sk_launch<T, SkCfg<1, 4, 2, 6, 2, 5, 1>>(p, grid, s);
        case 18: return sk_launch<T, SkCfg<9, 9, 1, 12, 1, 3, 1>>(p, grid, s);
        case 19: return sk_launch<T, SkCfg<4, 8, 2, 12, 1, 3, 1>>(p, grid, s);
        case 20: return sk_launch<T, SkCfg<1, 8, 4, 1, 2, 5, 1>>(p, grid, s);
        case 38: return iw_launch<T, IwCfg<1, 4, 3, 1, 5, 1>>(p, grid, s);
        case 39: return iw_launch<T, IwCfg<1, 4, 3, 2, 5, 1>>(p, grid, s);
        case 40: return iw_launch<T, IwCfg<1, 4, 3, 4, 5, 1>>(p, grid, s);
        case 41: return iw_launch<T, IwCfg<1, 4, 1, 2, 5, 1>>(p, grid, s);
        case 42: return iw_launch<T, IwCfg<1, 4, 1, 4, 5, 1>>(p, grid, s);
        case 43: return iw_launch<T, IwCfg<1, 8, 3, 1, 2, 1>>(p, grid, s);
        case 44: return iw_launch<T, IwCfg<1, 4, 6, 2, 2, 1>>(p, grid, s);
        case 46: return iw_launch<T, IwCfg<1, 8, 3, 2, 2, 1>>(p, grid, s);
        default: return set_error(MVLDM_ERR_ARG, "igemm: tile 15: bad configuration %d", cfg);
    }
}

struct SkGeom { int n_img, h_in, w_in, h_out, w_out; };
static SkGeom sk_geom(const mvldm_igemm_desc& d) {
    if (d.ksize == 1 && d.stride == 1 && d.pad == 0 && d.h_in == d.h_out && d.w_in == d.w_out) return {d.n_img * d.h_out * d.w_out, 1, 1, 1, 1};
    return {d.n_img, d.h_in, d.w_in, d.h_out, d.w_out};
}

static bool sk_cfg_fits(const SkinnyCfgInfo& c, const mvldm_igemm_desc& d) {
    const SkGeom g = sk_geom(d);
    const int taps = d.ksize * d.ksize, hw_out = g.h_out * g.w_out, hw_in = g.h_in * g.w_in;
    if (c.taps != taps) return false;
    const int rows = c.mt * 16;
    if (hw_out > rows || rows % hw_out) return false;
    const int G = rows / hw_out;
    if (G * hw_in > rows * c.sm) return false;
    if (d.epilogue == MVLDM_EPI_GEGLU && (c.nt & 1)) return false;
    if (c.taps == 0) return false;
    if (d.c1 > 0) {
        const bool sk2 = c.sc > 0 && c.taps == 1 && ((c.nw == 8 && c.sc == 4 && (c.mt == 3 || c.mt == 1)) || (c.nw == 4 && c.mt == 6));
        const bool iw2 = c.sc == 0 && c.taps == 1 && c.nw == 4 && (c.mt == 3 || c.mt == 6) && !(c.mt == 1);
        if (!sk2 && !iw2) return false;
    }
    return true;
}

bool skinny_applicable(const mvldm_igemm_desc& d) {
    if (d.act_dtype == MVLDM_F32 || d.k_order != 2) return false;
    if (!(d.ksize == 1 || d.ksize == 3 || (d.ksize == 2 && d.upsample >= 2)) || (d.upsample == 1)) return false;
    if (d.ksize != 2 && d.upsample != 0) return false;
    if (d.c0 % 64 || d.c1 % 64 || d.c0 <= 0 || (d.c1 == 0) != (d.src1 == nullptr)) return false;
    if (d.k_pad != d.ksize * d.ksize * (d.c0 + d.c1) || d.n_pad % 64 || d.n_out % 4 || d.n_out > d.n_pad) return false;
    if (d.dst_dtype != d.act_dtype && d.dst_dtype != MVLDM_F32) return false;
    if (d.epilogue == MVLDM_EPI_GEGLU && (d.n_out % 64 || d.row_bias || d.n_out != d.n_pad)) return false;
    const int n_dst = d.epilogue == MVLDM_EPI_GEGLU ? d.n_out / 2 : d.n_out;
    const int dst_ld = d.dst_ld > 0 ? d.dst_ld : n_dst;
    if (dst_ld % 4 || dst_ld < n_dst) return false;
    if (d.bias && ((uintptr_t)d.bias % 16)) return false;
    if (d.row_bias && (((uintptr_t)d.row_bias % 16) || d.row_bias_ld % 4)) return false;
    if (((uintptr_t)d.dst % 16) || ((uintptr_t)d.weight % 16) || (d.residual && ((uintptr_t)d.residual % 8))) return false;
    if (((uintptr_t)d.src0 % 16) || (d.src1 && ((uintptr_t)d.src1 % 16))) return false;
    const double px = (double)d.n_img * d.h_in * d.w_in;
    if (px * d.c0 * 2.0 >= 4.0e9 || px * d.c1 * 2.0 >= 4.0e9 || (double)d.n_pad * d.k_pad * 2.0 >= 4.0e9) return false;
    if (d.residual && d.upsample >= 2) return false;
    return true;
}

static int sk_choose(const mvldm_igemm_desc& d) {
    const SkGeom g = sk_geom(d);
    const int hw = g.h_out * g.w_out, taps = d.ksize * d.ksize, M = g.n_img * hw;
    int pref[6] = {0, 0, 0, 0, 0, 0};
    if (taps == 9) {
        if (d.stride == 2) { pref[0] = 5; }
        else if (hw > 48) { pref[0] = g.n_img >= 2 ? 18 : 2; pref[1] = 2; pref[2] = 18; }
        else { pref[0] = 1; pref[1] = 18; pref[2] = 2; }
    } else if (taps == 4) {
        if (hw > 48) { pref[0] = g.n_img >= 2 ? 19 : 7; pref[1] = 7; pref[2] = 19; }
        else { pref[0] = 6; pref[1] = 7; pref[2] = 19; }
    } else {
        if (M <= 16) { pref[0] = 20; pref[1] = 41; pref[2] = 10; }
        else if (M <= 160) {
            if (d.n_pad >= 2560) { pref[0] = 8; pref[1] = 40; }
            else { pref[0] = 38; pref[1] = 12; }
            pref[2] = 9;
        } else {
            if (d.n_pad <= 1280) { pref[0] = 44; pref[1] = 13; pref[2] = 9; }
            else { pref[0] = 8; pref[1] = 40; }
        }
        pref[4] = 12; pref[5] = 8;
    }
    for (int c : pref)
        if (c > 0 && c < kNumSkCfgs && sk_cfg_fits(kSkCfgs[c], d)) return c;
    for (int c = 1; c < kNumSkCfgs; ++c)
        if (sk_cfg_fits(kSkCfgs[c], d)) return c;
    return 0;
}

int skinny_run(const mvldm_igemm_desc& d, hipStream_t s) {
    MVLDM_REQUIRE(d.src0 && d.weight && d.dst, "igemm: null pointer");
    MVLDM_REQUIRE(skinny_applicable(d), "igemm: tile 15 (skinny weight-streaming GEMM) does not apply to this problem (needs the fragment-order "
                                        "pack, k_order 2, 16-bit activations, channels in multiples of 64, ksize 1 / 3 or a 2x2 phase conv)");
    int cfg = (d.tile >> 8) & 63;
    if (cfg == 0) cfg = sk_choose(d);
    MVLDM_REQUIRE(cfg > 0 && cfg < kNumSkCfgs && sk_cfg_fits(kSkCfgs[cfg], d), "igemm: tile 15: configuration %d does not compute this problem", cfg);
    const SkinnyCfgInfo& k = kSkCfgs[cfg];
    SkParams p;
    const bool phase = d.upsample >= 2;
    p.src0 = d.src0; p.src1 = d.src1; p.w = d.weight; p.bias = d.bias; p.row_bias = d.row_bias; p.residual = d.residual; p.dst = d.dst;
    p.c0 = d.c0; p.c1 = d.c1;
    const SkGeom g = sk_geom(d);
    p.n_img = g.n_img; p.h_in = g.h_in; p.w_in = g.w_in; p.hw_in = g.h_in * g.w_in; p.h_out = g.h_out; p.w_out = g.w_out; p.hw_out = g.h_out * g.w_out;
    p.rb_hw = d.h_out * d.w_out;
    auto lg2 = [](int v) { int sh = 0; while ((1 << sh) < v) ++sh; return (1 << sh) == v ? sh : -1; };
    p.hw_sh = lg2(p.hw_out); p.w_sh = lg2(p.w_out); p.rb_sh = lg2(p.rb_hw);
    p.stride = d.stride; p.ksize = d.ksize;
    p.scatter = phase; p.ph_y = phase ? (d.upsample - 2) >> 1 : 0; p.ph_x = phase ? (d.upsample - 2) & 1 : 0;
    p.ty0 = phase ? p.ph_y - 1 : -d.pad; p.tx0 = phase ? p.ph_x - 1 : -d.pad;
    p.M = p.n_img * p.hw_out; p.n_out = d.n_out;
    p.n_dst = d.epilogue == MVLDM_EPI_GEGLU ? d.n_out / 2 : d.n_out;
    p.dst_ld = d.dst_ld > 0 ? d.dst_ld : p.n_dst;
    p.row_bias_ld = d.row_bias_ld; p.epilogue = d.epilogue; p.dst_f32 = d.dst_dtype == MVLDM_F32; p.out_scale = d.out_scale;
    p.n_tiles = d.n_pad / 16;
    p.n_groups = (p.n_tiles + k.nt - 1) / k.nt;
    p.G = k.mt * 16 / p.hw_out;
    p.m_groups = (p.n_img + p.G - 1) / p.G;
    p.n_cbs = (d.c0 + d.c1) / 64; p.cb0 = d.c0 / 64;
    p.n_stages = k.sc ? (p.n_cbs + k.sc - 1) / k.sc : p.n_cbs;
    p.ksteps = p.n_cbs * k.taps * 2;
    const double px = (double)d.n_img * d.h_in * d.w_in;
    p.src0_bytes = (unsigned)(px * d.c0 * 2.0); p.src1_bytes = (unsigned)(px * d.c1 * 2.0);
    p.w_bytes = (unsigned)((double)d.n_pad * d.k_pad * 2.0);
    p.fake = kSkFake;
    p.trace = nullptr;
#ifdef MVLDM_SK_TRACE
    static unsigned long long* trace = nullptr;
    if (getenv("MVLDM_SK_TRACE")) {
        if (!trace) hipHostMalloc((void**)&trace, 16 * 40 * 8 * 8, hipHostMallocMapped);
        memset(trace, 0, 16 * 40 * 8 * 8);
        p.trace = trace;
    }
#endif
    if (kSkFake & 1) p.w_bytes = 0;
    if (kSkFake & 2) p.src0_bytes = p.src1_bytes = 0;
    if (kSkFake & 4) p.n_stages = 0;
    if (p.M == 0) return MVLDM_OK;
    const int grid = 8 * ((p.n_groups + 7) / 8) * p.m_groups;
    const int rc = dispatch_dtype(d.act_dtype, [&](auto t) -> int {
        using T = decltype(t);
        if constexpr (sizeof(T) == 2) return sk_dispatch<T>(cfg, p, grid, s);
        else return set_error(MVLDM_ERR_ARG, "igemm: tile 15 needs a 16-bit activation type");
    });
#ifdef MVLDM_SK_TRACE
    if (p.trace && getenv("MVLDM_SK_TRACE_DUMP")) {
        hipDeviceSynchronize();
        const unsigned long long t0 = p.trace[0];
        for (int w = 0; w < k.nw; ++w) {
            fprintf(stderr, "wave %d:", w);
            for (int st = 0; st < std::min(p.n_stages, 24); ++st) {
                const unsigned long long* e = p.trace + (w * 40 + st) * 8;
                fprintf(stderr, " [s%d +%llu w%llu b%llu c%llu i%llu]", st, e[0] - t0, e[1] - e[0], e[2] - e[1], e[3] - e[2], e[4] - e[3]);
            }
            fprintf(stderr, "\n");
        }
    }
#endif
    return rc;
}

}

using namespace mvldm;

extern "C" int mvldm_igemm_skinny_config(const mvldm_igemm_desc* d) {
    if (!d) return 0;
    mvldm_igemm_desc t = *d;
    t.k_order = 2;
    if (!t.weight) t.weight = t.src0;
    if (!skinny_applicable(t)) return 0;
    return sk_choose(t);
}

extern "C" int mvldm_pack_skinny(const void* packed, void* dst, int n_pad, int k_pad, int geglu, int dtype, mvldm_stream_t stream) {
    MVLDM_REQUIRE(packed && dst, "pack_skinny: null pointer");
    MVLDM_REQUIRE(dtype == MVLDM_BF16 || dtype == MVLDM_F16, "pack_skinny: 16-bit types only");
    MVLDM_REQUIRE(n_pad > 0 && n_pad % 64 == 0 && k_pad > 0 && k_pad % 64 == 0, "pack_skinny: n_pad %d / k_pad %d must be multiples of 64", n_pad, k_pad);
    const int n_tiles = n_pad / 16, ksteps = k_pad / 32;
    const size_t total = (size_t)n_tiles * ksteps * 64;
    const int blocks = (int)std::min<size_t>((total + 255) / 256, 8192);
    hipLaunchKernelGGL(pack_skinny_kernel, dim3(blocks), dim3(256), 0, (hipStream_t)stream, reinterpret_cast<const u32x4*>(packed),
                       reinterpret_cast<u32x4*>(dst), n_tiles, ksteps, geglu);
    return check_launch();
}
```

### mv_ldm_amd/modules.py

```python
from __future__ import annotations

import math
import os
from types import SimpleNamespace
from typing import List, Optional, Sequence

import torch
from torch import nn

from . import _lib as L
from . import ops
from .ops import PackedWeight
from .plan import Builder
from .runtime import from_nhwc, get_compute_dtype, require_gpu, to_nhwc


_EPOCH_COUNTER = [0]


def bump_weights_epoch(module=None) -> int:
    _EPOCH_COUNTER[0] += 1
    e = _EPOCH_COUNTER[0]
    if module is None:
        _GLOBAL_FLOOR[0] = e
# ... 217 lines not shown
        bo = self.to_out[0].bias
        if extra is None:
            return self.to_out[0]._f32("bias")
        return self._cache(("bsum",), [bo, extra], lambda: (bo.detach().float() + extra.detach().float()).contiguous())

    def emit_self(self, b: Builder, xn, residual, seg, lens, extra_bias=None, name="attn", kv_lens=None):
        C = self.inner
        qkv = b.linear(xn, self._packed_cat(b.dtype, [self.to_q, self.to_k, self.to_v]),
                       self._bias_cat([self.to_q, self.to_k, self.to_v]), name=name + ".to_qkv")
        a = b.attention(qkv[:, :C], qkv[:, C:2 * C], qkv[:, 2 * C:], self.heads, self.dim_head, seg, lens, lens if kv_lens is None else kv_lens,
                        name=name + ".sdpa")
        b.free(qkv)
        out = b.linear(a, self.to_out[0].packed(b.dtype), self.out_bias(extra_bias), residual=residual, name=name + ".to_out")
        b.free(a)
        return out

    def emit_cross(self, b: Builder, xn, ctx, residual, seg, q_lens, kv_lens, name="attn"):
        C = self.inner
        q = self.to_q.emit(b, xn, name=name + ".to_q")
        kv = b.linear(ctx, self._packed_cat(b.dtype, [self.to_k, self.to_v]), self._bias_cat([self.to_k, self.to_v]), name=name + ".to_kv")
        a = b.attention(q, kv[:, :C], kv[:, C:], self.heads, self.dim_head, seg, q_lens, kv_lens, name=name + ".sdpa")
        b.free(q)
        b.free(kv)
        out = b.linear(a, self.to_out[0].packed(b.dtype), self.out_bias(), residual=residual, name=name + ".to_out")
        b.free(a)
        return out


class GEGLU(nn.Module):
    def __init__(self, dim_in, dim_out):
        super().__init__()
        self.proj = Linear(dim_in, dim_out * 2)


class FeedForward(nn.Module):

    def __init__(self, dim, mult=4):
        super().__init__()
        self.net = nn.ModuleList([GEGLU(dim, dim * mult), nn.Dropout(0.0), Linear(dim * mult, dim)])

    def emit(self, b: Builder, xn, residual, name="ff"):
        p = self.net[0].proj
        g = b.linear(xn, p.packed(b.dtype, geglu=True), p._f32("bias"), epilogue=L.EPI_GEGLU, name=name + ".geglu")
        out = self.net[2].emit(b, g, residual=residual, name=name + ".out")
        b.free(g)
        return out


def _segments(b: Builder, q_lens, kv_lens=None):
    key = (tuple(q_lens), None if kv_lens is None else tuple(kv_lens))
    cache = b.__dict__.setdefault("_segcache", {})
    if key not in cache:
        cache[key] = ops.make_segments(list(q_lens), None if kv_lens is None else list(kv_lens), device=b.device)
        b.keep.append(cache[key])
    return cache[key]


class BasicTransformerBlock(nn.Module):

    def __init__(self, dim, num_attention_heads, attention_head_dim, cross_attention_dim):
        super().__init__()
        self.norm1 = LayerNorm(dim, eps=1e-5)
        self.attn1 = Attention(dim, None, num_attention_heads, attention_head_dim)
        self.norm2 = LayerNorm(dim, eps=1e-5)
        self.attn2 = Attention(dim, cross_attention_dim, num_attention_heads, attention_head_dim)
        self.norm3 = LayerNorm(dim, eps=1e-5)
        self.ff = FeedForward(dim)

    def emit(self, b: Builder, hs, n_img, tokens, ctx=None, ctx_tokens=0, zero_ctx=False):
        lens = [tokens] * n_img
        n1 = self.norm1.emit(b, hs, name="norm1")
        extra = self.attn2.to_out[0].bias if zero_ctx else None
        h1 = self.attn1.emit_self(b, n1, hs, _segments(b, lens), lens, extra_bias=extra, name="attn1")
        b.free(n1)
        if not zero_ctx:
            n2 = self.norm2.emit(b, h1, name="norm2")
            kv_lens = [ctx_tokens] * n_img
            h2 = self.attn2.emit_cross(b, n2, ctx, h1, _segments(b, lens, kv_lens), lens, kv_lens, name="attn2")
            b.free(n2)
            b.free(h1)
            h1 = h2
        n3 = self.norm3.emit(b, h1, name="norm3")
        out = self.ff.emit(b, n3, h1, name="ff")
        b.free(n3)
        b.free(h1)
        return out


class Transformer2DModel(nn.Module):

    def __init__(self, num_attention_heads, attention_head_dim, in_channels, cross_attention_dim,
                 use_linear_projection=False, norm_num_groups=32, num_layers=1):
        super().__init__()
        inner = num_attention_heads * attention_head_dim
        self.use_linear_projection, self.cross_attention_dim = use_linear_projection, cross_attention_dim
        self.norm = GroupNorm(norm_num_groups, in_channels, eps=1e-6)
        self.proj_in = Linear(in_channels, inner) if use_linear_projection else Conv2d(in_channels, inner, 1)
        self.transformer_blocks = nn.ModuleList([
            BasicTransformerBlock(inner, num_attention_heads, attention_head_dim, cross_attention_dim)
            for _ in range(num_layers)])
        self.proj_out = Linear(inner, in_channels) if use_linear_projection else Conv2d(inner, in_channels, 1)

    def _proj(self, b, mod, x2d, **kw):
        if isinstance(mod, Linear):
            return mod.emit(b, x2d, **kw)
        return b.linear(x2d, mod.packed(b.dtype, x2d.shape[-1]), mod._f32("bias"), **kw)

    def emit(self, b: Builder, x, ctx=None, zero_ctx=False, out=None):
        n, h, w, c = x.shape
        g = self.norm.emit(b, x, name="norm")
        hs = self._proj(b, self.proj_in, g.view(n * h * w, c), name="proj_in")
        b.free(g)
        ctx2d, ctx_tokens = None, 0
        if not zero_ctx:
            assert ctx is not None and ctx.shape[0] == n, "encoder_hidden_states must be [n_img, tokens, dim]"
            ctx_tokens = ctx.shape[1]
            ctx2d = ctx.reshape(n * ctx_tokens, ctx.shape[2])
        for i, blk in enumerate(self.transformer_blocks):
            with b.scope(f"transformer_blocks.{i}"):
                nxt = blk.emit(b, hs, n, h * w, ctx2d, ctx_tokens, zero_ctx)
            b.free(hs)
            hs = nxt
        out = self._proj(b, self.proj_out, hs, residual=x.view(n * h * w, c), name="proj_out", **({} if out is None else {"out": out.view(n * h * w, c)}))
        b.free(hs)
        return out.view(n, h, w, c)

    def forward(self, hidden_states, encoder_hidden_states=None, **_unused):
        b = eager_builder(hidden_states)
        x = to_nhwc(hidden_states, b.dtype)
        ctx = encoder_hidden_states
        if ctx is None:
            raise ValueError("Transformer2DModel needs encoder_hidden_states (the reference always passes one)")
        require_gpu(ctx)
        if ctx.dtype != b.dtype or not ctx.is_contiguous():
            ctx = ops.convert(ctx.contiguous(), b.dtype)
        return SimpleNamespace(sample=from_nhwc(self.emit(b, x, ctx)))


class Downsample2D(nn.Module):
    def __init__(self, channels, out_channels=None, padding=1):
        super().__init__()
        self.padding = padding
        self.conv = Conv2d(channels, out_channels or channels, 3, stride=2, padding=padding)

    def emit(self, b: Builder, x, out=None):
        return self.conv.emit(b, x, name="downsample", **({} if out is None else {"out": out}))

    def forward(self, x):
        b = eager_builder(x)
        return from_nhwc(self.emit(b, to_nhwc(x, b.dtype)))


class Upsample2D(nn.Module):
    def __init__(self, channels, out_channels=None):
        super().__init__()
        self.conv = Conv2d(channels, out_channels or channels, 3, padding=1)

    def emit(self, b: Builder, x):
        c = x.shape[-1]
        if b.dtype != torch.float32 and c % ops.block_k(b.dtype) == 0 and self.conv.out_channels % 8 == 0:
            pws = self.conv._cache(("wphase", b.dtype), [self.conv.weight],
                                   lambda: [ops.pack_weight(w, b.dtype) for w in ops.upsample_phase_weights(self.conv.weight)])
            return b.conv_upsample_phases(x, pws, self.conv._f32("bias"), name="upsample")
        return self.conv.emit(b, x, upsample=True, name="upsample")

    def forward(self, x):
        b = eager_builder(x)
        return from_nhwc(self.emit(b, to_nhwc(x, b.dtype)))


class DownBlock2D(nn.Module):
    def __init__(self, in_channels, out_channels, temb_channels, num_layers=2, resnet_eps=1e-5, resnet_groups=32,
                 add_downsample=True, downsample_padding=1):
        super().__init__()
        self.resnets = nn.ModuleList([ResnetBlock2D(in_channels if i == 0 else out_channels, out_channels, temb_channels,
                                                    resnet_groups, resnet_eps) for i in range(num_layers)])
        self.downsamplers = (nn.ModuleList([Downsample2D(out_channels, out_channels, downsample_padding)])
                             if add_downsample else None)


class CrossAttnDownBlock2D(DownBlock2D):
    def __init__(self, in_channels, out_channels, temb_channels, num_layers=2, resnet_eps=1e-5, resnet_groups=32,
                 num_attention_heads=1, cross_attention_dim=1280, use_linear_projection=False, add_downsample=True,
                 downsample_padding=1):
        super().__init__(in_channels, out_channels, temb_channels, num_layers, resnet_eps, resnet_groups, add_downsample,
                         downsample_padding)
        self.has_cross_attention = True
        self.attentions = nn.ModuleList([
            Transformer2DModel(num_attention_heads, out_channels // num_attention_heads, out_channels, cross_attention_dim,
                               use_linear_projection, resnet_groups) for _ in range(num_layers)])


class UNetMidBlock2DCrossAttn(nn.Module):
    def __init__(self, in_channels, temb_channels, num_layers=1, resnet_eps=1e-5, resnet_groups=32,
                 num_attention_heads=1, cross_attention_dim=1280, use_linear_projection=False):
        super().__init__()
        self.has_cross_attention = True
        self.resnets = nn.ModuleList([ResnetBlock2D(in_channels, in_channels, temb_channels, resnet_groups, resnet_eps)
                                      for _ in range(num_layers + 1)])
        self.attentions = nn.ModuleList([
            Transformer2DModel(num_attention_heads, in_channels // num_attention_heads, in_channels, cross_attention_dim,
                               use_linear_projection, resnet_groups) for _ in range(num_layers)])


class VaeAttention(nn.Module, _PackMixin):

    def __init__(self, channels, groups=32, eps=1e-6):
        super().__init__()
        self.channels = channels
        self.group_norm = GroupNorm(groups, channels, eps=eps)
        self.to_q = Linear(channels, channels)
        self.to_k = Linear(channels, channels)
        self.to_v = Linear(channels, channels)
        self.to_out = nn.ModuleList([Linear(channels, channels), nn.Dropout(0.0)])

    def emit(self, b: Builder, x):
        n, h, w, c = x.shape
        g = self.group_norm.emit(b, x, name="group_norm")
        ws = [self.to_q.weight, self.to_k.weight, self.to_v.weight]
        bs = [self.to_q.bias, self.to_k.bias, self.to_v.bias]
        pw = self._cache(("qkv", b.dtype), ws, lambda: ops.pack_weight(torch.cat([t.detach() for t in ws], 0), b.dtype))
        bias = self._cache(("qkvb",), bs, lambda: torch.cat([t.detach().float() for t in bs], 0).contiguous())
        qkv = b.linear(g.view(n * h * w, c), pw, bias, name="to_qkv")
        b.free(g)
        lens = [h * w] * n
        a = b.attention(qkv[:, :c], qkv[:, c:2 * c], qkv[:, 2 * c:], 1, c, _segments(b, lens), lens, lens, name="sdpa")
        b.free(qkv)
        out = self.to_out[0].emit(b, a, residual=x.view(n * h * w, c), name="to_out")
        b.free(a)
        return out.view(n, h, w, c)


class UNetMidBlock2D(nn.Module):

    def __init__(self, in_channels, temb_channels, num_layers=1, resnet_eps=1e-6, resnet_groups=32, add_attention=True):
        super().__init__()
        self.resnets = nn.ModuleList([ResnetBlock2D(in_channels, in_channels, temb_channels, resnet_groups, resnet_eps)
                                      for _ in range(num_layers + 1)])
        self.attentions = nn.ModuleList([VaeAttention(in_channels, resnet_groups, resnet_eps) for _ in range(num_layers)]
                                        if add_attention else [])

    def emit(self, b: Builder, x, temb=None):
        h = self.resnets[0].emit(b, x, temb)
        for i, (a, r) in enumerate(zip(self.attentions, self.resnets[1:])):
            if a is not None:
                with b.scope(f"attentions.{i}"):
                    h2 = a.emit(b, h)
                b.free(h)
                h = h2
            with b.scope(f"resnets.{i + 1}"):
                h2 = r.emit(b, h, temb)
            b.free(h)
            h = h2
        return h


class UpBlock2D(nn.Module):
    def __init__(self, in_channels, prev_output_channel, out_channels, temb_channels, num_layers=3, resnet_eps=1e-5,
                 resnet_groups=32, add_upsample=True):
        super().__init__()
        res = []
        for i in range(num_layers):
            skip = in_channels if i == num_layers - 1 else out_channels
            rin = prev_output_channel if i == 0 else out_channels
            res.append(ResnetBlock2D(rin + skip, out_channels, temb_channels, resnet_groups, resnet_eps))
        self.resnets = nn.ModuleList(res)
        self.upsamplers = nn.ModuleList([Upsample2D(out_channels, out_channels)]) if add_upsample else None


class CrossAttnUpBlock2D(UpBlock2D):
    def __init__(self, in_channels, prev_output_channel, out_channels, temb_channels, num_layers=3, resnet_eps=1e-5,
                 resnet_groups=32, num_attention_heads=1, cross_attention_dim=1280, use_linear_projection=False,
                 add_upsample=True):
        super().__init__(in_channels, prev_output_channel, out_channels, temb_channels, num_layers, resnet_eps,
                         resnet_groups, add_upsample)
        self.has_cross_attention = True
        self.attentions = nn.ModuleList([
            Transformer2DModel(num_attention_heads, out_channels // num_attention_heads, out_channels, cross_attention_dim,
                               use_linear_projection, resnet_groups) for _ in range(num_layers)])


SD21_UNET_CONFIG = dict(
    in_channels=4, out_channels=4,
    down_block_types=("CrossAttnDownBlock2D", "CrossAttnDownBlock2D", "CrossAttnDownBlock2D", "DownBlock2D"),
    mid_block_type="UNetMidBlock2DCrossAttn",
    up_block_types=("UpBlock2D", "CrossAttnUpBlock2D", "CrossAttnUpBlock2D", "CrossAttnUpBlock2D"),
    block_out_channels=(320, 640, 1280, 1280), layers_per_block=2, attention_head_dim=(5, 10, 20, 20),
    cross_attention_dim=1024, use_linear_projection=True, norm_num_groups=32, norm_eps=1e-5)


def _per_block(v, n):
    return tuple(v) if isinstance(v, (list, tuple)) else (v,) * n


class UNet2DConditionModel(nn.Module):

    def __init__(self, in_channels=4, out_channels=4,
                 down_block_types: Sequence[str] = ("CrossAttnDownBlock2D",) * 3 + ("DownBlock2D",),
                 mid_block_type: Optional[str] = "UNetMidBlock2DCrossAttn",
                 up_block_types: Sequence[str] = ("UpBlock2D",) + ("CrossAttnUpBlock2D",) * 3,
                 only_cross_attention=False, block_out_channels: Sequence[int] = (320, 640, 1280, 1280),
                 layers_per_block=2, downsample_padding=1, norm_num_groups=32, norm_eps=1e-5, cross_attention_dim=1280,
                 attention_head_dim=8, use_linear_projection=False, flip_sin_to_cos=True, freq_shift=0):
        super().__init__()
        if only_cross_attention:
            raise NotImplementedError("only_cross_attention=True is not on the reference's path")
        n, boc = len(down_block_types), tuple(block_out_channels)
        heads, xdim = _per_block(attention_head_dim, n), _per_block(cross_attention_dim, n)
        self.config = SimpleNamespace(in_channels=in_channels, out_channels=out_channels, block_out_channels=boc,
                                      cross_attention_dim=cross_attention_dim, norm_num_groups=norm_num_groups,
                                      norm_eps=norm_eps)
        temb = boc[0] * 4
        self.conv_in = Conv2d(in_channels, boc[0], 3, padding=1)
        self.time_proj = Timesteps(boc[0], flip_sin_to_cos, freq_shift)
        self.time_embedding = TimestepEmbedding(boc[0], temb)
        self.down_blocks = nn.ModuleList()
# ... 59 lines not shown
```

### mv_ldm_amd/ops.py

```python
from __future__ import annotations

import ctypes as C
import os
from dataclasses import dataclass
from typing import Optional, Sequence

import math

import torch

from . import _lib as L

_DT = {torch.float32: L.F32, torch.bfloat16: L.BF16, torch.float16: L.F16}


def dt(t) -> int:
    return _DT[t if isinstance(t, torch.dtype) else t.dtype]


def epc(dtype: torch.dtype) -> int:
    return 4 if dtype == torch.float32 else 8


def stream() -> int:
    return torch.cuda.current_stream().cuda_stream


def ptr(t: Optional[torch.Tensor]) -> Optional[int]:
    return None if t is None else t.data_ptr()


def _roundup(a: int, b: int) -> int:
    return (a + b - 1) // b * b


_WS: dict = {}


def workspace(nbytes: int, device, key: str = "splitk") -> torch.Tensor:
    k = (str(device), key)
    cur = _WS.get(k)
    if cur is None or cur.numel() < nbytes:
        cur = torch.empty(max(nbytes, 1 << 20), dtype=torch.uint8, device=device)
        _WS[k] = cur
    return cur


@dataclass
class PackedWeight:
    data: torch.Tensor
    n_out: int
    n_pad: int
    k_pad: int
    c_pad: int
    ksize: int
    geglu: bool = False
    k_order: int = 0
    _skinny: Optional[torch.Tensor] = None
    _skinny_pinned: bool = False

    def can_skinny(self) -> bool:
        return self.k_order == 1 and self.data.dtype != torch.float32 and self.c_pad % 64 == 0 and self.k_pad == self.ksize * self.ksize * self.c_pad \
            and self.ksize in (1, 2, 3) and self.n_out % 4 == 0

    def skinny(self) -> torch.Tensor:
        if self._skinny is None:
            assert self.can_skinny(), "tile 15 needs a 16-bit block-major pack with channels in multiples of 64"
            out = torch.empty_like(self.data)
            L.check(L.load().mvldm_pack_skinny(self.data.data_ptr(), out.data_ptr(), self.n_pad, self.k_pad, int(self.geglu), dt(self.data), stream()))
            self._skinny = out
        return self._skinny

    def drop_skinny(self):
        if not self._skinny_pinned:
            self._skinny = None


def block_k(dtype: torch.dtype) -> int:
    return 32 if dtype == torch.float32 else 64


def pack_weight_t(w: torch.Tensor, dtype: torch.dtype, c_off: int = 0, n_rows: Optional[int] = None,
                  out: Optional[torch.Tensor] = None) -> PackedWeight:
    assert w.is_cuda and w.dtype == torch.float32 and w.is_contiguous()
    n_out, c_in = w.shape[0], w.shape[1]
    ksize = w.shape[2] if w.ndim == 4 else 1
    n_rows = c_in - c_off if n_rows is None else n_rows
    c_pad = _roundup(n_out, epc(dtype))
    bk = block_k(dtype)
    k_pad = _roundup(ksize * ksize * c_pad, bk)
    n_pad = _roundup(n_rows, 64)
    k_order = int(c_pad % bk == 0)
    data = torch.zeros(n_pad, k_pad, dtype=dtype, device=w.device) if out is None else out
    L.check(L.load().mvldm_pack_weight(w.data_ptr(), data.data_ptr(), n_out, c_in, ksize, c_pad, n_pad, k_pad, 0, k_order, dt(dtype),
                                       1, c_off, n_rows, stream()))
    return PackedWeight(data, n_rows, n_pad, k_pad, c_pad, ksize, False, k_order)


def pack_weight(w: torch.Tensor, dtype: torch.dtype, c_pad: Optional[int] = None, geglu: bool = False,
                c_split: Optional[int] = None, out: Optional[torch.Tensor] = None) -> PackedWeight:
    assert w.is_cuda, "pack_weight needs a device tensor (no CPU path)"
    w = w.detach().to(torch.float32).contiguous()
    n_out, c_in = w.shape[0], w.shape[1]
    ksize = w.shape[2] if w.ndim == 4 else 1
    e = epc(dtype)
    c_pad = _roundup(c_in, e) if c_pad is None else c_pad
    bk = block_k(dtype)
    k_pad = _roundup(ksize * ksize * c_pad, bk)
    n_pad = _roundup(n_out, 64)
    k_order = int(c_pad % bk == 0 and (c_split is None or c_split % bk == 0))
    out = torch.empty(n_pad, k_pad, dtype=dtype, device=w.device) if out is None else out
    L.check(L.load().mvldm_pack_weight(w.data_ptr(), out.data_ptr(), n_out, c_in, ksize, c_pad, n_pad, k_pad,
                                       int(geglu), k_order, dt(dtype), 0, 0, n_out, stream()))
    return PackedWeight(out, n_out, n_pad, k_pad, c_pad, ksize, geglu, k_order)


def pack_job(w: torch.Tensor, pw: PackedWeight, *, transpose: bool = False, c_off: int = 0) -> "L.PackJob":
    assert w.is_cuda and w.dtype == torch.float32 and w.is_contiguous()
    j = L.PackJob()
    j.src, j.dst = w.data_ptr(), pw.data.data_ptr()
    j.n_out, j.c_in, j.ksize = w.shape[0], w.shape[1], pw.ksize
    j.c_pad, j.n_pad, j.k_pad, j.geglu, j.k_order = pw.c_pad, pw.n_pad, pw.k_pad, int(pw.geglu), pw.k_order
    j.transpose, j.c_off, j.n_rows = int(transpose), c_off, (pw.n_out if transpose else w.shape[0])
    L.check(L.load().mvldm_pack_job_prepare(C.byref(j), dt(pw.data.dtype)))
    return j


class PackBatch:

    def __init__(self, jobs: Sequence["L.PackJob"], dtype: torch.dtype, device):
        self.n, self.dtype = len(jobs), dtype
        arr = (L.PackJob * max(len(jobs), 1))()
        b0 = 0
        for i, j in enumerate(jobs):
            C.memmove(C.byref(arr[i]), C.byref(j), C.sizeof(L.PackJob))
            arr[i].block0 = b0
            b0 += j.blocks
        self.total_blocks = b0
        raw = torch.frombuffer(bytearray(bytes(arr)), dtype=torch.uint8).clone()
        self.table = raw.to(device)
        self.block_job = None
        if jobs:
            self.block_job = torch.repeat_interleave(torch.arange(len(jobs), dtype=torch.int32), torch.tensor([j.blocks for j in jobs])).to(device)
            assert self.block_job.numel() == b0

    def run(self):
        L.check(L.load().mvldm_pack_weight_batch(self.table.data_ptr(), self.n, None if self.block_job is None else self.block_job.data_ptr(),
                                                 self.total_blocks, dt(self.dtype), stream()))


def conv_out_hw(h: int, w: int, ksize: int, stride: int, pad: int, upsample) -> tuple:
    if int(upsample) >= 2:
        return h, w
    hs, ws = (2 * h, 2 * w) if upsample else (h, w)
    if ksize == 3 and stride == 2 and pad == 0:
        return (hs + 1 - 3) // 2 + 1, (ws + 1 - 3) // 2 + 1
    return (hs + 2 * pad - ksize) // stride + 1, (ws + 2 * pad - ksize) // stride + 1


def use_skinny(d, pw: PackedWeight) -> torch.Tensor:
    t = pw.skinny()
    d.weight, d.k_order = ptr(t), 2
    return t


def igemm_desc(src0, src1, pw: PackedWeight, dst, *, n_img, h_in, w_in, h_out, w_out, stride=1, pad=None, upsample=False,
               bias=None, row_bias=None, residual=None, epilogue=L.EPI_NONE, out_scale=1.0, ws=None, splitk=0,
               tile=0, into=None) -> L.IgemmDesc:
    d = L.IgemmDesc() if into is None else into
    c0 = src0.shape[-1]
    c1 = 0 if src1 is None else src1.shape[-1]
    assert c0 + c1 == pw.c_pad, f"weight packed for {pw.c_pad} channels, sources give {c0}+{c1}"
    assert not pw.k_order or c0 % block_k(src0.dtype) == 0, "weight packed block-major but the source split is unaligned"
    d.src0, d.src1, d.weight = ptr(src0), ptr(src1), ptr(pw.data)
    d.bias, d.row_bias, d.residual, d.dst = ptr(bias), ptr(row_bias), ptr(residual), ptr(dst)
    d.c0, d.c1 = c0, c1
    d.n_img, d.h_in, d.w_in, d.h_out, d.w_out = n_img, h_in, w_in, h_out, w_out
    d.ksize, d.stride, d.upsample = pw.ksize, stride, int(upsample)
    d.pad = (pw.ksize // 2) if pad is None else pad
    d.n_out, d.n_pad, d.k_pad = pw.n_out, pw.n_pad, pw.k_pad
    d.row_bias_ld = 0 if row_bias is None else row_bias.stride(0)
    d.epilogue, d.act_dtype, d.dst_dtype = epilogue, dt(src0), dt(dst)
    d.splitk, d.tile, d.out_scale = splitk, tile, out_scale
    n_dst = pw.n_out // 2 if epilogue == L.EPI_GEGLU else pw.n_out
    d.dst_ld = 0 if dst.shape[-1] == n_dst else dst.shape[-1]
    d.k_order = pw.k_order
    if (tile & 63) == 15:
        use_skinny(d, pw)
    if ws is not None:
        d.workspace, d.workspace_bytes = ws.data_ptr(), ws.numel() * ws.element_size()
    else:
        d.workspace, d.workspace_bytes = None, 0
        if splitk == 0:
            d.splitk = 1
    return d


def conv2d(x: torch.Tensor, pw: PackedWeight, bias=None, *, x2=None, stride=1, pad=None, upsample=False, row_bias=None,
           residual=None, epilogue=L.EPI_NONE, out_dtype=None, out_scale=1.0, splitk=0, tile=0, out=None) -> torch.Tensor:
    assert x.is_cuda and x.is_contiguous() and (x2 is None or x2.is_contiguous())
    n, h, w, _ = x.shape
    pad = (pw.ksize // 2) if pad is None else pad
    ho, wo = conv_out_hw(h, w, pw.ksize, stride, pad, upsample)
    n_dst = pw.n_out // 2 if epilogue == L.EPI_GEGLU else pw.n_out
    if out is None:
        out = torch.empty(n, ho, wo, n_dst, dtype=out_dtype or x.dtype, device=x.device)
    else:
        assert out.is_contiguous() and out.numel() == n * ho * wo * n_dst and out.dtype == (out_dtype or x.dtype)
        out = out.view(n, ho, wo, n_dst)
    scratch = None
    if splitk != 1:
        scratch = workspace(min(16 * n * ho * wo * pw.n_pad * 4, 256 << 20), x.device)
    d = igemm_desc(x, x2, pw, out, n_img=n, h_in=h, w_in=w, h_out=ho, w_out=wo, stride=stride, pad=pad,
                   upsample=upsample, bias=bias, row_bias=row_bias, residual=residual, epilogue=epilogue,
                   out_scale=out_scale, ws=scratch, splitk=splitk, tile=tile)
    L.check(L.load().mvldm_igemm_fwd(C.byref(d), stream()))
    return out


def upsample_phase_weights(w: torch.Tensor) -> list:
    assert w.ndim == 4 and w.shape[2:] == (3, 3)
    w = w.detach().to(torch.float32)
    rows = {0: (w[:, :, 0], w[:, :, 1] + w[:, :, 2]), 1: (w[:, :, 0] + w[:, :, 1], w[:, :, 2])}
    out = []
    for py in (0, 1):
        for px in (0, 1):
            taps = []
            for r in rows[py]:
                cols = (r[:, :, 0], r[:, :, 1] + r[:, :, 2]) if px == 0 else (r[:, :, 0] + r[:, :, 1], r[:, :, 2])
                taps.append(torch.stack(cols, dim=-1))
            out.append(torch.stack(taps, dim=-2).contiguous())
    return out


def conv2d_upsample_phases(x: torch.Tensor, pws, bias=None, tile=0, splitk=0) -> torch.Tensor:
    n, h, w, _ = x.shape
    out = torch.empty(n, 2 * h, 2 * w, pws[0].n_out, dtype=x.dtype, device=x.device)
    scratch = workspace(min(16 * n * h * w * pws[0].n_pad * 4, 256 << 20), x.device)
    for phase, pw in enumerate(pws):
        d = igemm_desc(x, None, pw, out, n_img=n, h_in=h, w_in=w, h_out=h, w_out=w, stride=1, pad=0, upsample=2 + phase,
                       bias=bias, splitk=splitk, tile=tile, ws=scratch)
        L.check(L.load().mvldm_igemm_fwd(C.byref(d), stream()))
    return out


def linear(x: torch.Tensor, pw: PackedWeight, bias=None, *, residual=None, epilogue=L.EPI_NONE, out_dtype=None,
           splitk=0, tile=0, out=None) -> torch.Tensor:
    rows, c = x.shape
    y = conv2d(x.view(rows, 1, 1, c), pw, bias, residual=None if residual is None else residual.view(rows, 1, 1, -1),
               epilogue=epilogue, out_dtype=out_dtype, splitk=splitk, tile=tile, out=out)
    return y.view(rows, -1)


def groupnorm(x: torch.Tensor, gamma, beta, groups: int, eps: float, silu: bool, x2=None, stats_out=None) -> torch.Tensor:
    assert x.is_cuda and x.is_contiguous() and (x2 is None or x2.is_contiguous())
    n, c0 = x.shape[0], x.shape[-1]
    c1 = 0 if x2 is None else x2.shape[-1]
    hw = math.prod(x.shape[1:-1])
    y = torch.empty(*x.shape[:-1], c0 + c1, dtype=x.dtype, device=x.device)
    ws = workspace(max(n, 1) * L.GN_MAX_CHUNKS * groups * 2 * 8, x.device, "gn")
    L.check(L.load().mvldm_groupnorm_fwd(x.data_ptr(), ptr(x2), y.data_ptr(), gamma.data_ptr(), beta.data_ptr(), n, hw, c0, c1,
                                         groups, eps, int(silu), dt(x), ws.data_ptr(), ptr(stats_out), stream()))
    return y


def layernorm(x: torch.Tensor, gamma, beta, eps: float = 1e-5) -> torch.Tensor:
    assert x.is_cuda and x.is_contiguous()
    c = x.shape[-1]
    rows = x.numel() // c
    y = torch.empty_like(x)
    L.check(L.load().mvldm_layernorm_fwd(x.data_ptr(), y.data_ptr(), gamma.data_ptr(), beta.data_ptr(), rows, c, eps,
                                         dt(x), stream()))
    return y


def make_segments(q_lens, kv_lens=None, device="cuda") -> torch.Tensor:
    kv_lens = q_lens if kv_lens is None else kv_lens
    rows, q0, k0 = [], 0, 0
    for ql, kl in zip(q_lens, kv_lens):
        rows.append([q0, ql, k0, kl])
        q0, k0 = q0 + ql, k0 + kl
    return torch.tensor(rows, dtype=torch.int32, device=device)


def attention(q: torch.Tensor, k: torch.Tensor, v: torch.Tensor, heads: int, head_dim: int, seg: torch.Tensor,
              max_q_len: int, scale: Optional[float] = None, lse: Optional[torch.Tensor] = None) -> torch.Tensor:
    assert q.is_cuda and q.stride(1) == 1 and k.stride(1) == 1 and v.stride(1) == 1
    out = torch.empty(q.shape[0], heads * head_dim, dtype=q.dtype, device=q.device)
    scale = head_dim ** -0.5 if scale is None else scale
    L.check(L.load().mvldm_attention_fwd(q.data_ptr(), k.data_ptr(), v.data_ptr(), out.data_ptr(), q.stride(0), k.stride(0),
                                         v.stride(0), out.stride(0), heads, head_dim, seg.data_ptr(), seg.shape[0],
                                         max_q_len, scale, dt(q), ptr(lse), 0 if lse is None else lse.stride(0), stream()))
    return out


def timestep_embed(timesteps: torch.Tensor, freqs: torch.Tensor, dim: int, flip_sin_to_cos: bool,
                   dtype=torch.float32) -> torch.Tensor:
    assert timesteps.dtype == torch.int64 and timesteps.is_cuda
    out = torch.empty(timesteps.numel(), dim, dtype=dtype, device=timesteps.device)
    L.check(L.load().mvldm_timestep_embed_fwd(timesteps.data_ptr(), freqs.data_ptr(), out.data_ptr(), timesteps.numel(),
                                              dim, int(flip_sin_to_cos), dt(dtype), stream()))
    return out


def eltwise(x: torch.Tensor, op: int, out_dtype=None) -> torch.Tensor:
    assert x.is_cuda and x.is_contiguous()
    y = torch.empty(x.shape, dtype=out_dtype or x.dtype, device=x.device)
    L.check(L.load().mvldm_eltwise_fwd(x.data_ptr(), y.data_ptr(), x.numel(), op, dt(x), dt(y), stream()))
    return y


def silu(x, out_dtype=None):
    return eltwise(x, L.ELT_SILU, out_dtype)


def convert(x, out_dtype):
    return eltwise(x, L.ELT_COPY, out_dtype)


def nchw_to_nhwc(src: torch.Tensor, dtype, dst: Optional[torch.Tensor] = None, c_off: int = 0,
                 dst_c: Optional[int] = None, scale: float = 1.0, shift: float = 0.0,
                 img_map: Optional[torch.Tensor] = None) -> torch.Tensor:
    assert src.is_cuda and src.dtype == torch.float32 and src.is_contiguous()
    n, c, h, w = src.shape
    if dst is None:
        dst_c = c if dst_c is None else dst_c
        dst = torch.zeros(n, h, w, dst_c, dtype=dtype, device=src.device)
    L.check(L.load().mvldm_nchw_to_nhwc(src.data_ptr(), dst.data_ptr(), n, c, h * w, dst.shape[-1], c_off, dt(dst), scale, shift,
                                        ptr(img_map), stream()))
    return dst


def ray_channels(mode: int = 0, n_origin_octaves: int = 0, n_dir_octaves: int = 0) -> int:
    return int(L.load(required=False).mvldm_ray_channels(mode, n_origin_octaves, n_dir_octaves)) if L.load(required=False) is not None else \
        {0: 6, 1: (6 * n_origin_octaves or 3) + (6 * n_dir_octaves or 3), 2: 6 * (n_origin_octaves + n_dir_octaves)}[mode]


def ray_encode(extrinsics: torch.Tensor, intrinsics: torch.Tensor, h: int, w: int, out_nchw: Optional[torch.Tensor] = None,
               out_nhwc: Optional[torch.Tensor] = None, c_off: int = 0, img_map: Optional[torch.Tensor] = None,
               mode: int = 0, n_origin_octaves: int = 0, n_dir_octaves: int = 0, plucker: bool = False):
    n = extrinsics.shape[0]
    assert extrinsics.is_cuda and extrinsics.dtype == torch.float32 and extrinsics.is_contiguous() and extrinsics.shape[1:] == (4, 4)
    assert intrinsics.dtype == torch.float32 and intrinsics.is_contiguous() and intrinsics.shape == (n, 3, 3)
    if out_nchw is None and out_nhwc is None:
        out_nchw = torch.empty(n, ray_channels(mode, n_origin_octaves, n_dir_octaves), h, w, dtype=torch.float32, device=extrinsics.device)
    L.check(L.load().mvldm_ray_encode(extrinsics.data_ptr(), intrinsics.data_ptr(), n, h, w, ptr(out_nchw), ptr(out_nhwc),
                                      0 if out_nhwc is None else out_nhwc.shape[-1], c_off,
                                      L.F32 if out_nhwc is None else dt(out_nhwc), ptr(img_map), mode, n_origin_octaves, n_dir_octaves,
                                      int(plucker), stream()))
    return out_nchw if out_nchw is not None else out_nhwc


def posterior_sample(moments: torch.Tensor, noise: torch.Tensor, scale: float = 1.0) -> torch.Tensor:
    n, c2, h, w = moments.shape
    assert moments.is_cuda and moments.dtype == torch.float32 and moments.is_contiguous()
    assert noise.dtype == torch.float32 and noise.is_contiguous() and noise.numel() == n * (c2 // 2) * h * w
    out = torch.empty(n, c2 // 2, h, w, dtype=torch.float32, device=moments.device)
    L.check(L.load().mvldm_posterior_sample(moments.data_ptr(), noise.data_ptr(), out.data_ptr(), n, c2 // 2, h * w, scale, stream()))
    return out


def nhwc_to_nchw(src: torch.Tensor, c: Optional[int] = None, c_off: int = 0, scale=1.0, shift=0.0,
                 clamp01=False) -> torch.Tensor:
    assert src.is_cuda and src.is_contiguous()
    n, h, w, sc = src.shape
    c = sc if c is None else c
    out = torch.empty(n, c, h, w, dtype=torch.float32, device=src.device)
    L.check(L.load().mvldm_nhwc_to_nchw(src.data_ptr(), out.data_ptr(), n, c, h * w, sc, c_off, dt(src), scale, shift,
                                        int(clamp01), stream()))
    return out


def ddim_cfg_step(eps, x_t, cond_img, uncond_img, cfg_scale, coef, step_ptr, unet_in=None, clip_range: float = 0.0) -> torch.Tensor:
    n_tgt, h, w, c = x_t.shape
    out = torch.empty_like(x_t)
    L.check(L.load().mvldm_ddim_cfg_step(eps.data_ptr(), x_t.data_ptr(), out.data_ptr(), cond_img.data_ptr(), ptr(uncond_img),
                                         n_tgt, h * w, c, cfg_scale, coef.data_ptr(), step_ptr.data_ptr(), ptr(unet_in),
                                         0 if unet_in is None else unet_in.shape[-1],
                                         dt(unet_in) if unet_in is not None else L.F32, coef.shape[0], clip_range, stream()))
    return out


def ddpm_cfg_step(eps_c, eps_u, x_t, noise, cfg_scale, coef, clip_range: float = 0.0) -> torch.Tensor:
    for t in (eps_c, eps_u, x_t, noise):
        assert t is None or (t.dtype == torch.float32 and t.is_contiguous() and t.numel() == x_t.numel())
    out = torch.empty_like(x_t)
    L.check(L.load().mvldm_ddpm_cfg_step(eps_c.data_ptr(), ptr(eps_u), x_t.data_ptr(), ptr(noise), out.data_ptr(), x_t.numel(),
                                         cfg_scale, coef.data_ptr(), clip_range, stream()))
    return out


# ... 230 lines not shown
```

### mv_ldm_amd/plan.py

```python
from __future__ import annotations

import ctypes as C
import json
import os
import sys
from dataclasses import dataclass
from typing import List, Optional

import torch

from . import _lib as L
from .ops import PackedWeight, conv_out_hw, dt, igemm_desc, ptr, use_skinny


def _PIN_TILE() -> int:
    v = os.environ.get("MVLDM_IGEMM_TILE")
    return int(v) if v else 0


@dataclass
class OpMeta:
    name: str
    kind: int
    flops: float = 0.0
    bytes: float = 0.0


class Builder:
    def __init__(self, device, dtype: torch.dtype, record: bool = False, splitk_ws_bytes: int = 256 << 20):
        self.device, self.dtype, self.record = torch.device(device), dtype, record
        self.ops: List[L.Op] = []
        self.meta: List[OpMeta] = []
        self.keep: list = []
        self._pool: dict = {}
        self._ws = None
        self._ws_bytes = splitk_ws_bytes
        self._gn_ws = None
        self._scope: List[str] = []
        self._lane = 0
        self._lane_ws: dict = {}
        self._deferred: Optional[list] = None
        self.skinny = True
        self._skinny_pw: dict = {}

    def empty(self, *shape, dtype=None) -> torch.Tensor:
        dtype = dtype or self.dtype
        if self.record:
            nbytes = int(torch.Size(shape).numel()) * torch.empty(0, dtype=dtype).element_size()
            free = self._pool.get(nbytes)
            if free:
                base = free.pop()
                return base.view(dtype).view(*shape)
        t = torch.empty(*shape, dtype=dtype, device=self.device)
        if self.record:
            self.keep.append(t)
            self.__dict__.setdefault("_own_ptrs", set()).add(t.data_ptr())
        return t

    def free(self, t: Optional[torch.Tensor]):
        if t is None or not self.record:
            return
        base = t.reshape(-1).view(torch.uint8)
        if self._deferred is not None:
            self._deferred.append(base)
            return
        self._pool.setdefault(base.numel(), []).append(base)

    class _Parallel:

        def __init__(self, b):
            self.b, self.n = b, 0

        def __enter__(self):
            assert self.b._deferred is None, "parallel groups do not nest"
            self.b._marker(L.OP_PAR_BEGIN, "par_begin")
            self.b._deferred = []
            return self

        def lane(self):
            if self.n:
                self.b._marker(L.OP_PAR_NEXT, "par_next")
            self.b._lane = self.n
            self.n += 1

        def __exit__(self, *a):
            b = self.b
            b._marker(L.OP_PAR_END, "par_end")
            b._lane = 0
            deferred, b._deferred = b._deferred, None
            for base in deferred:
                b._pool.setdefault(base.numel(), []).append(base)

    def parallel(self):
        return Builder._Parallel(self)

    def _marker(self, kind: int, name: str):
        op = L.Op()
        op.kind = kind
        self._emit(op, name)

    def splitk_ws(self) -> torch.Tensor:
        if self._lane:
            ws = self._lane_ws.get(("splitk", self._lane))
            if ws is None:
                ws = torch.empty(min(self._ws_bytes, 64 << 20), dtype=torch.uint8, device=self.device)
                self._lane_ws[("splitk", self._lane)] = ws
                self.keep.append(ws)
            return ws
        if self._ws is None:
            self._ws = torch.empty(self._ws_bytes, dtype=torch.uint8, device=self.device)
            self.keep.append(self._ws)
        return self._ws

    def gn_ws(self, n_img: int, groups: int) -> torch.Tensor:
        need = n_img * L.GN_MAX_CHUNKS * groups * 16
        if self._lane:
            ws = self._lane_ws.get(("gn", self._lane))
            if ws is None or ws.numel() < need:
                ws = torch.empty(max(need, 1 << 16), dtype=torch.uint8, device=self.device)
                self._lane_ws[("gn", self._lane)] = ws
                self.keep.append(ws)
            return ws
        if self._gn_ws is None or self._gn_ws.numel() < need:
            self._gn_ws = torch.empty(max(need, 1 << 16), dtype=torch.uint8, device=self.device)
            self.keep.append(self._gn_ws)
        return self._gn_ws

    class _Scope:
        def __init__(self, b, name):
            self.b, self.name = b, name

        def __enter__(self):
            self.b._scope.append(self.name)

        def __exit__(self, *a):
            self.b._scope.pop()

    def scope(self, name: str):
        return Builder._Scope(self, name)

    def _emit(self, op: L.Op, name: str, flops=0.0, nbytes=0.0, refs=()):
        if self.record:
            op.tag = len(self.ops)
            self.ops.append(op)
            self.meta.append(OpMeta("/".join(self._scope + [name]), op.kind, flops, nbytes))
            self.keep.extend(r for r in refs if r is not None)
        else:
            L.check(L.load().mvldm_op_run(C.byref(op), torch.cuda.current_stream().cuda_stream))

    def conv(self, x, pw: PackedWeight, bias=None, *, x2=None, stride=1, pad=None, upsample=False, row_bias=None,
             residual=None, epilogue=L.EPI_NONE, out_dtype=None, out_scale=1.0, out=None, name="conv", splitk=0, tile=0):
        n, h, w, c0 = x.shape
        c1 = 0 if x2 is None else x2.shape[-1]
        pad = (pw.ksize // 2) if pad is None else pad
        ho, wo = conv_out_hw(h, w, pw.ksize, stride, pad, upsample)
        n_dst = pw.n_out // 2 if epilogue == L.EPI_GEGLU else pw.n_out
        if out is None:
            out = self.empty(n, ho, wo, n_dst, dtype=out_dtype or x.dtype)
        ws = self.splitk_ws() if splitk != 1 else None
        if tile == 0 and _PIN_TILE() and x.dtype != torch.float32 and pw.k_order == 1:
            tile, splitk = _PIN_TILE(), 1
        m = n * ho * wo
        k_real = pw.ksize * pw.ksize * (c0 + c1)
        es = x.element_size()
        nbytes = (pw.n_out * k_real + n * h * w * (c0 + c1)) * es + m * n_dst * out.element_size() \
            + (m * n_dst * es if residual is not None else 0)
        self._igemm(x, x2, pw, bias, row_bias, residual, out, ws, name, 2.0 * m * pw.n_out * k_real, nbytes, h_out=ho, w_out=wo,
                    stride=stride, pad=pad, upsample=upsample, epilogue=epilogue, out_scale=out_scale, splitk=splitk, tile=tile)
        return out

    def _igemm(self, x, x2, pw, bias, row_bias, residual, out, ws, name, flops, nbytes, *, h_out, w_out, tile=0, **desc):
        n, h, w, c0 = x.shape
        c1 = 0 if x2 is None else x2.shape[-1]
        op = L.Op()
        op.kind = L.OP_IGEMM
        d = igemm_desc(x, x2, pw, out, n_img=n, h_in=h, w_in=w, h_out=h_out, w_out=w_out, bias=bias, row_bias=row_bias,
                       residual=residual, ws=ws, tile=tile, into=op.u.igemm, **desc)
        m = n * h_out * w_out
        can_sk = tile == 0 and self.skinny and skinny_candidate(pw, m, c0, c1, d.upsample, x.dtype) \
            and x.is_cuda and L.load().mvldm_igemm_skinny_config(C.byref(d)) > 0
        if can_sk and skinny_rule(m, pw.n_pad):
            tile = d.tile = 15
            use_skinny(d, pw)
        elif can_sk and self.record:
            self._skinny_pw[len(self.ops)] = pw
        if self.record:
            own = self.__dict__.get("_own_ptrs", ())
            self.__dict__.setdefault("_tune_srcs", {})[len(self.ops)] = tuple(t if (t is not None and t.data_ptr() in own) else None
                                                                              for t in (x, x2))
        self._emit(op, name, flops, nbytes, (x, x2, pw.data, pw._skinny if (tile & 63) == 15 else None, bias, row_bias, residual, out))

    def small_launch(self, rows: int, n_out: int) -> bool:
        limit = int(os.environ.get("MVLDM_PAR_ROWS", "0"))
        return self.record and rows * max(n_out, 1) <= limit * 640 and limit > 0

    def conv_upsample_phases(self, x, pws, bias=None, name="upsample"):
        n, h, w, c0 = x.shape
        out = self.empty(n, 2 * h, 2 * w, pws[0].n_out, dtype=x.dtype)
        lanes = self.parallel() if self.small_launch(n * h * w, pws[0].n_out) else None
        if lanes is not None:
            lanes.__enter__()
        for phase, pw in enumerate(pws):
            if lanes is not None:
                lanes.lane()
            self._phase_conv(x, pw, bias, out, phase, name)
        if lanes is not None:
            lanes.__exit__(None, None, None)
        return out

    def _phase_conv(self, x, pw, bias, out, phase, name, tile=0, splitk=0):
        n, h, w, c0 = x.shape
        ws = self.splitk_ws()
        assert pw.ksize == 2 and pw.k_order == 1 and c0 == pw.c_pad
        m = n * h * w
        es = x.element_size()
        nbytes = (pw.n_out * 4 * c0 + (m * c0 if phase == 0 else 0)) * es + m * pw.n_out * es
        self._igemm(x, None, pw, bias, None, None, out, ws, f"{name}.p{phase}", 2.0 * m * pw.n_out * 4 * c0, nbytes, h_out=h, w_out=w,
                    stride=1, pad=0, upsample=2 + phase, splitk=splitk, tile=tile)

    def linear(self, x, pw: PackedWeight, bias=None, *, residual=None, epilogue=L.EPI_NONE, out_dtype=None, out=None,
               name="linear", row_bias=None):
        rows, c = x.shape
        y = self.conv(x.view(rows, 1, 1, c), pw, bias, residual=None if residual is None else residual.view(rows, 1, 1, -1),
                      epilogue=epilogue, out_dtype=out_dtype, out=None if out is None else out.view(rows, 1, 1, -1),
                      name=name, row_bias=row_bias)
        return y.view(rows, -1)

    def groupnorm(self, x, gamma, beta, groups, eps, silu, x2=None, name="groupnorm", stats_out=None):
        n, c0 = x.shape[0], x.shape[-1]
        c1 = 0 if x2 is None else x2.shape[-1]
        hw = x.numel() // (n * c0)
        y = self.empty(*x.shape[:-1], c0 + c1, dtype=x.dtype)
        op = L.Op()
        op.kind = L.OP_GROUPNORM
        g = op.u.groupnorm
        g.x, g.x1, g.y, g.gamma, g.beta = ptr(x), ptr(x2), ptr(y), ptr(gamma), ptr(beta)
        g.stats_ws = self.gn_ws(n, groups).data_ptr()
        g.n_img, g.hw, g.c0, g.c1, g.groups, g.silu, g.dtype, g.eps = n, hw, c0, c1, groups, int(silu), dt(x), eps
        g.stats_out = ptr(stats_out)
        passes = L.load().mvldm_groupnorm_passes(n, hw, c0 + c1, groups, dt(x))
        self._emit(op, name, 0.0, float(passes) * y.numel() * y.element_size(), (x, x2, y, gamma, beta, stats_out))
        return y

    def layernorm(self, x, gamma, beta, eps=1e-5, name="layernorm"):
        c = x.shape[-1]
        rows = x.numel() // c
        y = self.empty(*x.shape, dtype=x.dtype)
        op = L.Op()
        op.kind = L.OP_LAYERNORM
        l = op.u.layernorm
        l.x, l.y, l.gamma, l.beta, l.rows, l.c, l.dtype, l.eps = ptr(x), ptr(y), ptr(gamma), ptr(beta), rows, c, dt(x), eps
        self._emit(op, name, 0.0, 2.0 * y.numel() * y.element_size(), (x, y, gamma, beta))
        return y

    def attention(self, q, k, v, heads, head_dim, seg, q_lens, kv_lens, scale=None, name="attention", lse=None, out=None):
        assert q.stride(1) == 1 and k.stride(1) == 1 and v.stride(1) == 1
        if out is None:
            out = self.empty(q.shape[0], heads * head_dim, dtype=q.dtype)
        op = L.Op()
        op.kind = L.OP_ATTENTION
        a = op.u.attention
        a.q, a.k, a.v, a.out, a.seg = ptr(q), ptr(k), ptr(v), ptr(out), ptr(seg)
        a.ld_q, a.ld_k, a.ld_v, a.ld_o = q.stride(0), k.stride(0), v.stride(0), out.stride(0)
        a.heads, a.head_dim, a.n_seg, a.max_q_len, a.dtype = heads, head_dim, seg.shape[0], max(q_lens), dt(q)
        a.scale = head_dim ** -0.5 if scale is None else scale
        a.lse, a.lse_ld = ptr(lse), (0 if lse is None else lse.stride(0))
        pairs = sum(ql * kl for ql, kl in zip(q_lens, kv_lens))
        es = q.element_size()
        nbytes = (sum(q_lens) * 2 + sum(kv_lens) * 2) * heads * head_dim * es
        self._emit(op, name, 4.0 * pairs * heads * head_dim, nbytes, (q, k, v, out, seg, lse))
        return out

    def attention_merge(self, oa, lse_a, ob, lse_b, out, a_img, b_img, out_img, tokens, heads, head_dim, name="attention_merge"):
        n = a_img.numel()
        assert b_img.numel() == n and out_img.numel() == n and all(i.dtype == torch.int32 for i in (a_img, b_img, out_img))
        assert lse_a.dtype == torch.float32 and lse_b.dtype == torch.float32 and oa.dtype == ob.dtype == out.dtype
        op = L.Op()
        op.kind = L.OP_ATTN_MERGE
        m = op.u.attn_merge
        m.oa, m.ob, m.out, m.lse_a, m.lse_b, m.a_img, m.b_img, m.out_img = ptr(oa), ptr(ob), ptr(out), ptr(lse_a), ptr(lse_b), ptr(a_img), ptr(b_img), ptr(out_img)
        m.n_img, m.tokens, m.heads, m.head_dim = n, tokens, heads, head_dim
        m.ld_a, m.ld_b, m.ld_o, m.lse_ld_a, m.lse_ld_b, m.dtype = oa.stride(0), ob.stride(0), out.stride(0), lse_a.stride(0), lse_b.stride(0), dt(oa)
        self._emit(op, name, 0.0, 3.0 * n * tokens * heads * head_dim * oa.element_size(), (oa, lse_a, ob, lse_b, out, a_img, b_img, out_img))

    def timestep_embed(self, timesteps, freqs, dim, flip, dtype, name="time_proj"):
        out = self.empty(timesteps.numel(), dim, dtype=dtype)
        op = L.Op()
        op.kind = L.OP_TIMESTEP_EMBED
        t = op.u.temb
        t.timesteps, t.freqs, t.out, t.n, t.dim, t.flip, t.dst_dtype = ptr(timesteps), ptr(freqs), ptr(out), timesteps.numel(), dim, int(flip), dt(out)
        self._emit(op, name, 0.0, out.numel() * out.element_size(), (timesteps, freqs, out))
        return out

    def eltwise(self, x, op_code, out_dtype=None, name="eltwise"):
        y = self.empty(*x.shape, dtype=out_dtype or x.dtype)
        op = L.Op()
        op.kind = L.OP_ELTWISE
        e = op.u.eltwise
        e.x, e.y, e.n, e.op, e.src_dtype, e.dst_dtype = ptr(x), ptr(y), x.numel(), op_code, dt(x), dt(y)
        self._emit(op, name, 0.0, x.numel() * (x.element_size() + y.element_size()), (x, y))
        return y

    def ddim_step(self, eps, x_t, x_next, cond_img, uncond_img, cfg_scale, coef, step_ptr, unet_in, name="ddim_cfg_step",
                  clip_range: float = 0.0):
        n_tgt, h, w, c = x_t.shape
        op = L.Op()
        op.kind = L.OP_DDIM_STEP
        d = op.u.ddim
        d.eps, d.x_t, d.x_next, d.cond_img, d.uncond_img = ptr(eps), ptr(x_t), ptr(x_next), ptr(cond_img), ptr(uncond_img)
        d.coef, d.step_ptr, d.unet_in = ptr(coef), ptr(step_ptr), ptr(unet_in)
        d.n_tgt, d.hw, d.c, d.cfg_scale = n_tgt, h * w, c, cfg_scale
        d.unet_in_c = 0 if unet_in is None else unet_in.shape[-1]
        d.unet_in_dtype = L.F32 if unet_in is None else dt(unet_in)
        d.n_steps, d.clip_range = coef.shape[0], clip_range
        self._emit(op, name, 0.0, 5.0 * x_t.numel() * 4, (eps, x_t, x_next, cond_img, uncond_img, coef, step_ptr, unet_in))
        return x_next

    def ddim_advance(self, step_ptr, t_table, timesteps, tgt_rows, name="ddim_advance"):
        op = L.Op()
        op.kind = L.OP_DDIM_ADVANCE
        a = op.u.advance
        a.step_ptr, a.t_table, a.timesteps, a.tgt_rows = ptr(step_ptr), ptr(t_table), ptr(timesteps), ptr(tgt_rows)
        a.n_steps, a.n_rows = t_table.numel(), 0 if tgt_rows is None else tgt_rows.numel()
        self._emit(op, name, 0.0, 0.0, (step_ptr, t_table, timesteps, tgt_rows))

    def memcpy(self, dst, src, name="memcpy"):
        assert dst.is_contiguous() and src.is_contiguous() and dst.numel() * dst.element_size() == src.numel() * src.element_size()
        op = L.Op()
        op.kind = L.OP_MEMCPY
        op.u.memcpy_.src, op.u.memcpy_.dst, op.u.memcpy_.bytes = ptr(src), ptr(dst), src.numel() * src.element_size()
        self._emit(op, name, 0.0, 2.0 * src.numel() * src.element_size(), (dst, src))

    def gather_rows(self, src, dst, src_index=None, dst_index=None, n_rows=None, name="gather_rows"):
        idx = src_index if src_index is not None else dst_index
        n = int(n_rows if n_rows is not None else (idx.numel() if idx is not None else dst.shape[0]))
        row_bytes = dst[0].numel() * dst.element_size()
        assert src[0].numel() * src.element_size() == row_bytes and row_bytes % 16 == 0 and dst.is_contiguous() and src.is_contiguous()
        assert all(i is None or (i.dtype == torch.int32 and i.numel() == n) for i in (src_index, dst_index))
        assert (src_index is not None or src.shape[0] >= n) and (dst_index is not None or dst.shape[0] >= n)
        op = L.Op()
        op.kind = L.OP_GATHER_ROWS
        g = op.u.gather
        g.src, g.dst, g.src_index, g.dst_index, g.row_bytes, g.n_rows = ptr(src), ptr(dst), ptr(src_index), ptr(dst_index), row_bytes, n
        self._emit(op, name, 0.0, 2.0 * n * row_bytes, (src, dst, src_index, dst_index))

    def nhwc_to_nchw(self, src, dst, c=None, c_off=0, scale=1.0, shift=0.0, clamp01=False, name="nhwc_to_nchw"):
        n, h, w, sc = src.shape
        op = L.Op()
        op.kind = L.OP_NHWC_TO_NCHW
        l = op.u.layout
        l.src, l.dst, l.n_img, l.c, l.hw, l.other_c, l.other_c_off, l.dtype = ptr(src), ptr(dst), n, c or sc, h * w, sc, c_off, dt(src)
        l.clamp01, l.scale, l.shift = int(clamp01), scale, shift
        self._emit(op, name, 0.0, src.numel() * src.element_size() + dst.numel() * 4, (src, dst))
        return dst

    def nchw_to_nhwc(self, src, dst, c_off=0, scale=1.0, shift=0.0, img_map=None, name="nchw_to_nhwc"):
        n, c, h, w = src.shape
        op = L.Op()
        op.kind = L.OP_NCHW_TO_NHWC
        l = op.u.layout
        l.src, l.dst, l.n_img, l.c, l.hw, l.other_c, l.other_c_off, l.dtype = ptr(src), ptr(dst), n, c, h * w, dst.shape[-1], c_off, dt(dst)
        l.scale, l.shift, l.img_map = scale, shift, ptr(img_map)
        self._emit(op, name, 0.0, src.numel() * 4 + src.numel() * dst.element_size(), (src, dst, img_map))
        return dst

    def ray_encode(self, extr, intr, h, w, out_nhwc, c_off, img_map=None, out_nchw=None, name="ray_encode", mode=0, n_origin_octaves=0,
                   n_dir_octaves=0, plucker=False):
        op = L.Op()
        op.kind = L.OP_RAY_ENCODE
        r = op.u.rays
        r.extrinsics, r.intrinsics, r.out_nchw, r.out_nhwc, r.img_map = ptr(extr), ptr(intr), ptr(out_nchw), ptr(out_nhwc), ptr(img_map)
        r.n_cam, r.h, r.w = extr.shape[0], h, w
        r.nhwc_c, r.nhwc_c_off, r.nhwc_dtype = (0, 0, L.F32) if out_nhwc is None else (out_nhwc.shape[-1], c_off, dt(out_nhwc))
        r.mode, r.n_origin_octaves, r.n_dir_octaves, r.plucker = mode, n_origin_octaves, n_dir_octaves, int(plucker)
        self._emit(op, name, 0.0, extr.shape[0] * h * w * 6 * 4.0, (extr, intr, out_nhwc, out_nchw, img_map))

    def posterior_sample(self, moments, noise, out, scale=1.0, name="posterior_sample"):
        n, c2, h, w = moments.shape
        op = L.Op()
        op.kind = L.OP_POSTERIOR_SAMPLE
        q = op.u.posterior
        q.moments, q.noise, q.out, q.n, q.c, q.hw, q.scale = ptr(moments), ptr(noise), ptr(out), n, c2 // 2, h * w, scale
        self._emit(op, name, 0.0, moments.numel() * 4 * 2.0, (moments, noise, out))
        return out

    def finalize(self, autotune: Optional[bool] = None) -> "Plan":
        assert self.record
        if autotune is None:
            autotune = os.environ.get("MVLDM_AUTOTUNE", "1") != "0"
        if autotune and torch.device(self.device).type == "cuda":
            autotune_igemm(self.ops, srcs=self.__dict__.get("_tune_srcs"), skinny=self._skinny_pw, keep=self.keep)
            autotune_wgrad(self.ops)
            if type(self) is Builder and _BATCH_SPLIT:
                self.ops, self.meta = autosplit_igemm(self.ops, self.meta, skinny=self._skinny_pw, keep=self.keep)
        return Plan(self.ops, self.meta, self.keep, self.device)


_TUNE_CACHE = {}
_WGRAD_CACHE = {}
_SPLIT_CACHE = {}
_VALIDATED = set()
_TUNE_TILES = tuple(int(t) for t in os.environ["MVLDM_TUNE_TILES"].split(",")) if os.environ.get("MVLDM_TUNE_TILES") else (0, 1, 2, 3, 4, 5, 6, 7, 8, 9, 10, 11, 12, 13, 14)


def tune_cache_state() -> dict:
    return {"version": 2, "igemm": {json.dumps(list(k)): (int(v) if isinstance(v, int) else list(v)) for k, v in _TUNE_CACHE.items()},
            "wgrad": {json.dumps(list(k)): int(v) for k, v in _WGRAD_CACHE.items()},
            "split": {json.dumps(list(k)): int(v) for k, v in _SPLIT_CACHE.items()}}


def set_tune_cache_state(state: dict, replace: bool = False) -> None:
    if replace:
        _TUNE_CACHE.clear()
        _WGRAD_CACHE.clear()
        _SPLIT_CACHE.clear()
    for name, cache in (("igemm", _TUNE_CACHE), ("wgrad", _WGRAD_CACHE), ("split", _SPLIT_CACHE)):
        for k, v in (state.get(name) or {}).items():
            cache[tuple(json.loads(k))] = int(v) if isinstance(v, int) else list(v)


def save_tune_cache(path: Optional[str] = None) -> Optional[str]:
    path = path or os.environ.get("MVLDM_TUNE_CACHE")
    if not path:
        return None
    tmp = f"{path}.{os.getpid()}.tmp"
    with open(tmp, "w") as f:
        json.dump(tune_cache_state(), f, indent=0, sort_keys=True)
    os.replace(tmp, path)
    return path


def load_tune_cache(path: Optional[str] = None) -> int:
    path = path or os.environ.get("MVLDM_TUNE_CACHE")
    if not path or not os.path.exists(path):
        return 0
    with open(path) as f:
        set_tune_cache_state(json.load(f))
    return len(_TUNE_CACHE) + len(_WGRAD_CACHE) + len(_SPLIT_CACHE)


def broadcast_tune_cache(dist, src: int = 0, device=None) -> None:
    box = [tune_cache_state() if dist.get_rank() == src else None]
    dist.broadcast_object_list(box, src=src, device=device)
    set_tune_cache_state(box[0], replace=True)


load_tune_cache()


def _igemm_signature(d) -> tuple:
    return (d.n_img, d.h_in, d.w_in, d.h_out, d.w_out, d.c0, d.c1, d.ksize, d.stride, d.pad, d.upsample, d.n_out, d.n_pad,
            d.k_pad, d.epilogue, d.act_dtype, d.dst_dtype, d.k_order, d.dst_ld, bool(d.residual), bool(d.row_bias),
            bool(d.bias), d.splitk, d.workspace_bytes)


_SMALL_ROWS = int(os.environ.get("MVLDM_TUNE_SMALL_ROWS", "64"))
_SPLITS = (0, 1, 2, 4, 8, 16, 32)
_MID_ROWS = int(os.environ.get("MVLDM_TUNE_MID_ROWS", "40000"))
_MID_SPLITS = (0, 1, 2, 3, 4, 6, 8)
_SMALL_TILES = tuple(int(t) for t in os.environ.get("MVLDM_TUNE_SMALL_TILES", "0,1,2,3,4,5").split(","))


_SKINNY = os.environ.get("MVLDM_SKINNY", "1") != "0"
_SKINNY_ROWS = int(os.environ.get("MVLDM_SKINNY_ROWS", "2304"))
_SKINNY_CFGS = tuple(int(c) for c in os.environ.get("MVLDM_SKINNY_CFGS", "0,1,2,5,6,7,8,9,10,12,13,18,19,20,38,39,40,41,42,43,44,46").split(","))


def skinny_rule(rows: int, n_pad: int) -> bool:
    if os.environ.get("MVLDM_AUTOTUNE", "1") != "0" or os.environ.get("MVLDM_SKINNY_RULE", "1") == "0":
        return False
    return rows <= 160 or (rows <= 1152 and n_pad <= 1280)


def skinny_candidate(pw: PackedWeight, rows: int, c0: int, c1: int, upsample, dtype) -> bool:
    return (_SKINNY and dtype != torch.float32 and rows <= _SKINNY_ROWS and not (upsample is True or upsample == 1) and pw.can_skinny()
            and c0 % 64 == 0 and c1 % 64 == 0)


def _unpack_choice(v):
    return (int(v), None) if isinstance(v, int) else (int(v[0]), None if v[1] is None else int(v[1]))


_TUNE_COLD = int(os.environ.get("MVLDM_TUNE_COLD", "9216"))
_THRASH = []
_THRASH_FILLS = [0]


def _thrash(device=None):
    if not _THRASH or (device is not None and _THRASH[0].device != torch.device(device)):
        _THRASH[:] = [torch.empty(640 << 20, dtype=torch.uint8, device=torch.cuda.current_device() if device is None else device)]
    return _THRASH[0]


def autotune_igemm(ops, min_rows: int = 2048, iters: int = 4, srcs=None, skinny=None, keep=None) -> int:
    lib = L.load()
    stream = torch.cuda.current_stream().cuda_stream
    e0, e1 = torch.cuda.Event(enable_timing=True), torch.cuda.Event(enable_timing=True)
    timed = 0
    tune_dev = next((t.device for pair in (srcs or {}).values() for t in pair if t is not None), None)
    if srcs:
        seen, gen = set(), None
        for pair in srcs.values():
            for t in pair:
                if t is not None and t.is_floating_point() and t.data_ptr() not in seen:
                    seen.add(t.data_ptr())
                    if gen is None:
                        gen = torch.Generator(device=t.device)
                        gen.manual_seed(0x5EED)
                    t.normal_(generator=gen)
    for idx, op in enumerate(ops):
        if op.kind != L.OP_IGEMM:
            continue
        d = op.u.igemm
        rows = d.n_img * d.h_out * d.w_out
        sk_pw = (skinny or {}).get(idx)
        if d.tile != 0 or d.act_dtype == L.F32 or d.k_order != 1 or (rows < min(min_rows, _SMALL_ROWS) and sk_pw is None):
            continue
        small = rows < min_rows
        key = _igemm_signature(d) + (("sk",) if sk_pw is not None else ())
        best = _TUNE_CACHE.get(key)
        if best is not None and (_unpack_choice(best)[0] & 63) not in (set(_TUNE_TILES) | set(_SMALL_TILES) | {17, 19} | ({15} if sk_pw is not None else set())):
            best = None
        if best is None:
            trial = L.Op()
            C.memmove(C.byref(trial), C.byref(op), C.sizeof(L.Op))
            can_split = small and bool(d.workspace) and d.splitk == 0
            mid = (not small) and rows < _MID_ROWS and bool(d.workspace) and d.splitk == 0
            cands = [(t, sk) for t in _TUNE_TILES for sk in _MID_SPLITS] if mid else [(t, None) for t in _TUNE_TILES] if not small else \
                    [(t, sk) for t in _SMALL_TILES if t in _TUNE_TILES or not os.environ.get("MVLDM_TUNE_TILES") for sk in (_SPLITS if can_split else (None,))]
            n_it = iters if not small else 3 * iters
            cold = _TUNE_COLD > 0 and rows <= _TUNE_COLD
            if not small and 17 not in _TUNE_TILES and not os.environ.get("MVLDM_TUNE_TILES") and d.ksize == 3 and d.stride == 1 \
                    and d.src1 is None and not d.upsample and d.w_in <= 24:
                cands = cands + [(17, None)]
            if not small and d.ksize == 1 and not os.environ.get("MVLDM_TUNE_TILES"):
                cands = cands + [(19, None), (13 | (1 << 13), None)]
            if sk_pw is not None:
                cands = cands + [(15 | (c << 8), 1) for c in _SKINNY_CFGS]
            results = []
            for tile, sk in cands:
                trial.u.igemm.tile = tile
                trial.u.igemm.splitk = d.splitk if sk is None else sk
                trial.u.igemm.weight, trial.u.igemm.k_order = d.weight, d.k_order
                if (tile & 63) == 15:
                    use_skinny(trial.u.igemm, sk_pw)
                if lib.mvldm_op_run(C.byref(trial), stream) != 0:
                    continue
                if cold:
                    t_sum = 0.0
                    for _ in range(n_it):
                        _thrash(tune_dev).zero_()
                        _THRASH_FILLS[0] += 1
                        e0.record()
                        lib.mvldm_op_run(C.byref(trial), stream)
                        e1.record()
                        e1.synchronize()
                        t_sum += e0.elapsed_time(e1)
                    results.append((t_sum, tile, sk))
                    continue
                e0.record()
                for _ in range(n_it):
                    lib.mvldm_op_run(C.byref(trial), stream)
                e1.record()
                e1.synchronize()
                results.append((e0.elapsed_time(e1), tile, sk))
            t_rule = next(t for t, tile, sk in results if tile == 0 and sk in (None, 0))
            t_best, tile_best, sk_best = min(results, key=lambda r: r[0])
            best = [tile_best, sk_best] if t_best < 0.97 * t_rule else [0, None]
            _TUNE_CACHE[key] = best
            _VALIDATED.add(key)
            timed += 1
        tile, sk = _unpack_choice(best)
        if tile != 0 and key not in _VALIDATED:
            trial = L.Op()
            C.memmove(C.byref(trial), C.byref(op), C.sizeof(L.Op))
            trial.u.igemm.tile = tile
            if sk is not None:
                trial.u.igemm.splitk = sk
            if (tile & 63) == 15:
                if sk_pw is None:
                    tile, sk = 0, None
                else:
                    use_skinny(trial.u.igemm, sk_pw)
            if tile != 0 and lib.mvldm_op_run(C.byref(trial), stream) != 0:
                tile, sk = 0, None
                _TUNE_CACHE[key] = [0, None]
            _VALIDATED.add(key)
        d.tile = tile
        if sk is not None:
            d.splitk = sk
        if (tile & 63) == 15:
            t = use_skinny(d, sk_pw)
            sk_pw._skinny_pinned = True
            if keep is not None:
                keep.append(t)
        elif sk_pw is not None:
            sk_pw.drop_skinny()
    if timed:
        save_tune_cache()
        _THRASH.clear()
    return timed


_BATCH_SPLIT = os.environ.get("MVLDM_BATCH_SPLIT", "1") != "0"
_SPLIT_MIN_ROWS = int(os.environ.get("MVLDM_BATCH_SPLIT_MIN_ROWS", "16384"))


def _split_candidates(d) -> list:
    rpi = d.h_out * d.w_out
    rows = d.n_img * rpi
    out = []
    for bn in (320, 256):
        n_tiles = -(-d.n_pad // bn)
        m_tiles = -(-rows // 256)
        if m_tiles * n_tiles <= 256 or (m_tiles * n_tiles) % 256 == 0 or (m_tiles * n_tiles) % 256 > 216:
            continue
        for m1 in range(m_tiles - 1, 0, -1):
            if (m1 * n_tiles) % 256 == 0 and (m1 * 256) % rpi == 0:
                n1 = m1 * 256 // rpi
                frac = 1.0 - n1 / d.n_img
                if 0.03 <= frac <= 0.45 and n1 not in out:
                    out.append(n1)
                break
    return out


def _image_range(op, i0: int, n: int):
    q = L.Op()
    C.memmove(C.byref(q), C.byref(op), C.sizeof(L.Op))
    d = q.u.igemm
    es = 4 if d.act_dtype == L.F32 else 2
    ds = 4 if d.dst_dtype == L.F32 else 2
    n_dst = d.n_out // 2 if d.epilogue == L.EPI_GEGLU else d.n_out
    px_in, px_out = d.h_in * d.w_in, d.h_out * d.w_out

    def off(p, nbytes):
        return (p + nbytes) if p else p
    d.src0 = off(d.src0, i0 * px_in * d.c0 * es)
    d.src1 = off(d.src1, i0 * px_in * d.c1 * es)
    d.dst = off(d.dst, i0 * px_out * (d.dst_ld or n_dst) * ds)
    d.residual = off(d.residual, i0 * px_out * n_dst * es)
    d.row_bias = off(d.row_bias, i0 * d.row_bias_ld * 4)
    d.n_img = n
    d.tile, d.splitk = 0, 0
    return q


def _time_ops(ops, iters: int) -> float:
    lib = L.load()
    stream = torch.cuda.current_stream().cuda_stream
    e0, e1 = torch.cuda.Event(enable_timing=True), torch.cuda.Event(enable_timing=True)
    for o in ops:
        L.check(lib.mvldm_op_run(C.byref(o), stream))
    e0.record()
    for _ in range(iters):
        for o in ops:
            lib.mvldm_op_run(C.byref(o), stream)
    e1.record()
    e1.synchronize()
    return e0.elapsed_time(e1) / iters


def autosplit_igemm(ops, meta, skinny=None, keep=None, iters: int = 6):
    new_ops, new_meta, decided = [], [], 0
    for idx, (op, m) in enumerate(zip(ops, meta)):
        d = op.u.igemm if op.kind == L.OP_IGEMM else None
        rows = d.n_img * d.h_out * d.w_out if d is not None else 0
        ok = (d is not None and rows >= _SPLIT_MIN_ROWS and d.act_dtype != L.F32 and d.k_order == 1 and d.stride == 1 and not d.upsample
              and (d.tile & 63) != 15 and not _PIN_TILE() and bool(d.workspace) and idx not in (skinny or {}))
        n1 = 0
        if ok:
            key = _igemm_signature(d)[:-2] + (d.workspace_bytes,)
            if key in _SPLIT_CACHE:
                n1 = _SPLIT_CACHE[key]
            else:
                best_t, t_whole = None, None
                for cand in _split_candidates(d):
                    parts = [_image_range(op, 0, cand), _image_range(op, cand, d.n_img - cand)]
                    try:
                        autotune_igemm(parts, iters=4)
                        if t_whole is None:
                            t_whole = _time_ops([op], iters)
                        t = _time_ops(parts, iters)
                    except L.MvldmError:
                        continue
                    if os.environ.get("MVLDM_BATCH_SPLIT_LOG"):
                        print(f"[batch split] {m.name}: {d.n_img} images x {d.h_out}x{d.w_out}, N {d.n_out}, K {d.k_pad}: whole {t_whole * 1e3:.1f} us (tile {d.tile & 63}, "
                              f"splitk {d.splitk}); {cand} + {d.n_img - cand}: {t * 1e3:.1f} us (tiles {parts[0].u.igemm.tile & 63} / {parts[1].u.igemm.tile & 63}, "
                              f"splitk {parts[1].u.igemm.splitk})", file=sys.stderr, flush=True)
                    if t < 0.97 * t_whole and (best_t is None or t < best_t):
                        best_t, n1 = t, cand
                _SPLIT_CACHE[key] = n1
                decided += 1
        if n1:
            parts = [_image_range(op, 0, n1), _image_range(op, n1, d.n_img - n1)]
            autotune_igemm(parts, iters=4)
            for k, (q, i0, cnt) in enumerate(zip(parts, (0, n1), (n1, d.n_img - n1))):
                q.tag = len(new_ops)
                new_ops.append(q)
                share = cnt / d.n_img
                new_meta.append(OpMeta(m.name if k == 0 else m.name + "[rest]", m.kind, m.flops * share, m.bytes * share))
        else:
            op.tag = len(new_ops)
            new_ops.append(op)
            new_meta.append(m)
    if decided:
        save_tune_cache()
    return new_ops, new_meta


_WGRAD_TARGETS = tuple(int(t) for t in os.environ.get("MVLDM_TUNE_WGRAD_TARGETS", "0,1,2,3,4,5").split(","))


def autotune_wgrad(ops, iters: int = 3) -> int:
    lib = L.load()
    stream = torch.cuda.current_stream().cuda_stream
    e0, e1 = torch.cuda.Event(enable_timing=True), torch.cuda.Event(enable_timing=True)
    timed = 0
    scratch = None
    for op in ops:
        if op.kind != L.OP_WGRAD:
            continue
        d = op.u.wgrad
        if d.act_dtype == L.F32 or (d.accumulate >> 8) & 3:
            continue
        key = (d.c0, d.c1, d.n_img, d.h_in, d.w_in, d.h_out, d.w_out, d.ksize, d.stride, d.pad, d.upsample, d.n_out, d.dy_ld, d.act_dtype,
               int(d.workspace_bytes), d.accumulate & 1)
        best = _WGRAD_CACHE.get(key)
        if best is None:
            trial = L.Op()
            C.memmove(C.byref(trial), C.byref(op), C.sizeof(L.Op))
            need = d.n_out * d.c_in * d.ksize * d.ksize
            if scratch is None or scratch.numel() < need:
                scratch = torch.zeros(need, dtype=torch.float32, device=torch.cuda.current_device())
            else:
                scratch[:need].zero_()
            trial.u.wgrad.grad = scratch.data_ptr()
            results = []
            for form in (1, 2):
                for tcode in _WGRAD_TARGETS:
                    v = form + 4 * tcode
                    trial.u.wgrad.accumulate = (d.accumulate & 1) | (v << 8)
                    if lib.mvldm_op_run(C.byref(trial), stream) != 0:
                        break
                    e0.record()
                    for _ in range(iters):
                        lib.mvldm_op_run(C.byref(trial), stream)
                    e1.record()
                    e1.synchronize()
                    results.append((e0.elapsed_time(e1), v))
            best = min(results)[1] if results else 0
            _WGRAD_CACHE[key] = best
            timed += 1
        d.accumulate = (d.accumulate & 1) | (best << 8)
    if timed:
        save_tune_cache()
    return timed


class Plan:

    def __init__(self, ops, meta, keep, device):
        self.meta, self._keep, self.device = list(meta), list(keep), device
        self.ops = list(ops)
        self.tiles = [int(op.u.igemm.tile) if op.kind == L.OP_IGEMM else None for op in ops]
        arr = (L.Op * max(len(ops), 1))(*ops)
        h = C.c_void_p()
        L.check(L.load().mvldm_plan_create(arr, len(ops), C.byref(h)))
        self._h = h
        self._stream = None
        self.captured = False

    def __len__(self):
        return len(self.meta)

    @staticmethod
    def _cur():
        return torch.cuda.current_stream().cuda_stream

    def run(self, first: int = 0, last: Optional[int] = None):
        last = len(self.meta) if last is None else last
        L.check(L.load().mvldm_plan_run_range(self._h, first, last, self._cur()))

    def capture(self):
        if self._stream is None:
            self._stream = torch.cuda.Stream(device=self.device)
        self._stream.wait_stream(torch.cuda.current_stream())
        L.check(L.load().mvldm_plan_capture(self._h, self._stream.cuda_stream))
        torch.cuda.current_stream().wait_stream(self._stream)
        self.captured = True

    def replay(self):
        L.check(L.load().mvldm_plan_replay(self._h, self._cur()))

    def profile(self, iters: int = 3):
        out = (C.c_float * max(len(self.meta), 1))()
        L.check(L.load().mvldm_plan_profile(self._h, self._cur(), iters, out))
        return [float(v) for v in out[:len(self.meta)]]

    def __del__(self):
        try:
            if getattr(self, "_h", None):
                L.load().mvldm_plan_destroy(self._h)
                self._h = None
        except Exception:
            pass
```

### mv_ldm_amd/vae.py

```python
from __future__ import annotations

from dataclasses import dataclass
from types import SimpleNamespace
from typing import Optional, Sequence

import torch
from torch import nn

from . import ops
import warnings

from .modules import Builder, Conv2d, Downsample2D, GroupNorm, ResnetBlock2D, UNetMidBlock2D, Upsample2D, weights_version
from .runtime import get_compute_dtype, require_gpu

SD21_VAE_CONFIG = dict(in_channels=3, out_channels=3, block_out_channels=(128, 256, 512, 512), layers_per_block=2,
                       latent_channels=4, norm_num_groups=32, scaling_factor=0.18215)


class DownEncoderBlock2D(nn.Module):
    def __init__(self, in_channels, out_channels, num_layers, groups, add_downsample):
        super().__init__()
        self.resnets = nn.ModuleList([ResnetBlock2D(in_channels if i == 0 else out_channels, out_channels, None, groups, 1e-6)
                                      for i in range(num_layers)])
        self.downsamplers = nn.ModuleList([Downsample2D(out_channels, out_channels, padding=0)]) if add_downsample else None


class UpDecoderBlock2D(nn.Module):
    def __init__(self, in_channels, out_channels, num_layers, groups, add_upsample):
        super().__init__()
        self.resnets = nn.ModuleList([ResnetBlock2D(in_channels if i == 0 else out_channels, out_channels, None, groups, 1e-6)
                                      for i in range(num_layers)])
        self.upsamplers = nn.ModuleList([Upsample2D(out_channels, out_channels)]) if add_upsample else None


def _chain(b: Builder, h, mods, prefix, free_first=True):
    first = True
    for name, m in mods:
        with b.scope(f"{prefix}.{name}"):
            nh = m.emit(b, h)
        if not first or free_first:
            b.free(h)
        first = False
        h = nh
    return h


class Encoder(nn.Module):
    def __init__(self, in_channels, latent_channels, boc: Sequence[int], layers_per_block, groups):
        super().__init__()
        self.conv_in = Conv2d(in_channels, boc[0], 3, padding=1)
        self.down_blocks = nn.ModuleList()
        out_c = boc[0]
        for i in range(len(boc)):
            in_c, out_c = out_c, boc[i]
            self.down_blocks.append(DownEncoderBlock2D(in_c, out_c, layers_per_block, groups, i != len(boc) - 1))
        self.mid_block = UNetMidBlock2D(boc[-1], None, num_layers=1, resnet_eps=1e-6, resnet_groups=groups, add_attention=True)
        self.conv_norm_out = GroupNorm(groups, boc[-1], eps=1e-6)
        self.conv_act = nn.SiLU()
        self.conv_out = Conv2d(boc[-1], 2 * latent_channels, 3, padding=1)

    def emit(self, b: Builder, x):
        h = self.conv_in.emit(b, x, name="encoder.conv_in")
        for i, blk in enumerate(self.down_blocks):
            mods = [(f"resnets.{j}", r) for j, r in enumerate(blk.resnets)]
            if blk.downsamplers is not None:
                mods += [("downsamplers.0", blk.downsamplers[0])]
            h = _chain(b, h, mods, f"encoder.down_blocks.{i}")
        with b.scope("encoder.mid_block"):
            h2 = self.mid_block.emit(b, h)
        b.free(h)
        g = self.conv_norm_out.emit(b, h2, silu=True, name="encoder.conv_norm_out+silu")
        b.free(h2)
        out = self.conv_out.emit(b, g, name="encoder.conv_out")
        b.free(g)
        return out


class Decoder(nn.Module):
    def __init__(self, latent_channels, out_channels, boc: Sequence[int], layers_per_block, groups):
        super().__init__()
        self.conv_in = Conv2d(latent_channels, boc[-1], 3, padding=1)
        self.mid_block = UNetMidBlock2D(boc[-1], None, num_layers=1, resnet_eps=1e-6, resnet_groups=groups, add_attention=True)
        self.up_blocks = nn.ModuleList()
        rboc = list(reversed(boc))
        out_c = rboc[0]
        for i in range(len(rboc)):
            prev, out_c = out_c, rboc[i]
            self.up_blocks.append(UpDecoderBlock2D(prev, out_c, layers_per_block + 1, groups, i != len(rboc) - 1))
        self.conv_norm_out = GroupNorm(groups, boc[0], eps=1e-6)
        self.conv_act = nn.SiLU()
        self.conv_out = Conv2d(boc[0], out_channels, 3, padding=1)

    def emit(self, b: Builder, z, out_dtype=None):
        h = self.conv_in.emit(b, z, name="decoder.conv_in")
        with b.scope("decoder.mid_block"):
            h2 = self.mid_block.emit(b, h)
        b.free(h)
        h = h2
        for i, blk in enumerate(self.up_blocks):
            mods = [(f"resnets.{j}", r) for j, r in enumerate(blk.resnets)]
            if blk.upsamplers is not None:
                mods += [("upsamplers.0", blk.upsamplers[0])]
            h = _chain(b, h, mods, f"decoder.up_blocks.{i}")
        g = self.conv_norm_out.emit(b, h, silu=True, name="decoder.conv_norm_out+silu")
        b.free(h)
        out = self.conv_out.emit(b, g, out_dtype=out_dtype, name="decoder.conv_out")
        b.free(g)
        return out


class DiagonalGaussianDistribution:

    def __init__(self, parameters: torch.Tensor):
        self.parameters = parameters
        self.mean, self._raw_logvar = torch.chunk(parameters, 2, dim=1)

    @property
    def logvar(self):
        return torch.clamp(self._raw_logvar, -30.0, 20.0)

    @property
    def std(self):
        return torch.exp(0.5 * self.logvar)

    def sample(self, generator=None, noise=None, scale: float = 1.0):
        if noise is None:
            noise = torch.randn(self.mean.shape, generator=generator, device=self.mean.device, dtype=torch.float32)
        noise = noise.to(self.mean.device, torch.float32).contiguous()
        return ops.posterior_sample(self.parameters.contiguous(), noise, scale)

    def mode(self):
        return self.mean


class AutoencoderKL(nn.Module):
    def __init__(self, in_channels=3, out_channels=3, block_out_channels=(64,), layers_per_block=1, latent_channels=4,
                 norm_num_groups=32, scaling_factor=0.18215, **_ignored):
        super().__init__()
        boc = tuple(block_out_channels)
        self.config = SimpleNamespace(scaling_factor=scaling_factor, latent_channels=latent_channels, block_out_channels=boc,
                                      in_channels=in_channels, out_channels=out_channels)
        self.encoder = Encoder(in_channels, latent_channels, boc, layers_per_block, norm_num_groups)
        self.decoder = Decoder(latent_channels, out_channels, boc, layers_per_block, norm_num_groups)
        self.quant_conv = Conv2d(2 * latent_channels, 2 * latent_channels, 1)
        self.post_quant_conv = Conv2d(latent_channels, latent_channels, 1)
        self._plans = {}

    @classmethod
    def from_pretrained(cls, path, subfolder="vae", config_overrides=None, state_dict=None, allow_random_init=False):
        cfg = dict(SD21_VAE_CONFIG)
        cfg.update(config_overrides or {})
        m = cls(**cfg)
        if state_dict is not None:
            m.load_state_dict(state_dict)
            return m
        from .checkpoint import find_local_weights, load_vae_checkpoint
        f = find_local_weights(path, subfolder)
        if f is not None:
            load_vae_checkpoint(m, f)
        elif not allow_random_init:
            warnings.warn(f"AutoencoderKL.from_pretrained({path!r}): no local weights found and no state_dict given -- the "
                          "module keeps RANDOM initial weights (pass allow_random_init=True to silence)", stacklevel=2)
        return m

    def _compile(self, kind: str, n: int, h: int, w: int, dtype, io=(1.0, 0.0, 1.0, 0.0, False)):
        dev = next(self.parameters()).device
        key = (kind, n, h, w, dtype, str(dev), io)
        st = self._plans.get(key)
        if st is not None and st["weights_version"] == weights_version(self):
            return st
        pre_scale, pre_shift, post_scale, post_shift, clamp01 = io
        e = ops.epc(dtype)
        lc = self.config.latent_channels
        bld = Builder(dev, dtype, record=True)
        if kind == "decode":
            c_pad = (lc + e - 1) // e * e
            src = torch.zeros(n, lc, h, w, dtype=torch.float32, device=dev)
            z = torch.zeros(n, h, w, c_pad, dtype=dtype, device=dev)
            bld.nchw_to_nhwc(src, z, scale=pre_scale, shift=pre_shift)
            pq = self.post_quant_conv
            z2 = torch.zeros(n, h, w, c_pad, dtype=dtype, device=dev)
            bld.conv(z, pq.packed(dtype, c_pad), pq._f32("bias"), out=z2, name="post_quant_conv")
            y = self.decoder.emit(bld, z2)
            out = torch.zeros(n, self.config.out_channels, y.shape[1], y.shape[2], dtype=torch.float32, device=dev)
            bld.nhwc_to_nchw(y, out, scale=post_scale, shift=post_shift, clamp01=clamp01)
# ... 89 lines not shown
```

Before: 50.41.

## Merge four upsample phase convolutions into one igemm launch

Adds an upsample mode 6 in which a single implicit-GEMM launch covers all four 2x2 sub-pixel phases of the nearest-upsample convolution. The M tile index selects the phase and the weight offset into four contiguous phase packs. The plan builder times the merged launch against the four separate launches and keeps whichever is faster, caching the choice, and it applies only to large UNet upsamplers (the VAE opts out). The aim is to remove launch overhead and tail underfill from four small launches. The cost is that the merged path gives up split-K and some tiles.

```diff
diff --git a/include/mvldm.h b/include/mvldm.h
--- a/include/mvldm.h
+++ b/include/mvldm.h
@@ -56,6 +56,7 @@
 
 int mvldm_pack_skinny(const void* packed, void* dst, int n_pad, int k_pad, int geglu, int dtype, mvldm_stream_t stream);
 int mvldm_igemm_skinny_config(const mvldm_igemm_desc* d);
+int mvldm_igemm_config(const mvldm_igemm_desc* d, int* tile, int* splitk);
 
 typedef struct mvldm_pack_job {
     const float* src; void* dst;
diff --git a/mv_ldm_amd/_lib.py b/mv_ldm_amd/_lib.py
--- a/mv_ldm_amd/_lib.py
+++ b/mv_ldm_amd/_lib.py
@@ -186,6 +186,7 @@
     "mvldm_pack_weight": (C.c_int, [vp, vp] + [C.c_int] * 12 + [vp]),
     "mvldm_pack_skinny": (C.c_int, [vp, vp, C.c_int, C.c_int, C.c_int, C.c_int, vp]),
     "mvldm_igemm_skinny_config": (C.c_int, [C.POINTER(IgemmDesc)]),
+    "mvldm_igemm_config": (C.c_int, [C.POINTER(IgemmDesc), C.POINTER(C.c_int), C.POINTER(C.c_int)]),
     "mvldm_pack_job_prepare": (C.c_int, [C.POINTER(PackJob), C.c_int]),
     "mvldm_pack_weight_batch": (C.c_int, [vp, C.c_int, vp, C.c_int, C.c_int, vp]),
     "mvldm_groupnorm_fwd": (C.c_int, [vp, vp, vp, vp, vp, C.c_int, C.c_int, C.c_int, C.c_int, C.c_int, f32, C.c_int, C.c_int, vp, vp, vp]),
diff --git a/mv_ldm_amd/csrc/igemm.hip b/mv_ldm_amd/csrc/igemm.hip
--- a/mv_ldm_amd/csrc/igemm.hip
+++ b/mv_ldm_amd/csrc/igemm.hip
@@ -175,8 +175,16 @@
     const int epc = d.act_dtype == MVLDM_F32 ? 4 : 8;
     const int bk = d.act_dtype == MVLDM_F32 ? 32 : 64;
     MVLDM_REQUIRE(d.src0 && d.weight && d.dst, "igemm: null pointer");
-    const bool phase = d.upsample >= 2;
-    MVLDM_REQUIRE(d.upsample >= 0 && d.upsample <= 5, "igemm: upsample %d", d.upsample);
+    const bool phase = d.upsample >= 2, merged = d.upsample == 6;
+    MVLDM_REQUIRE(d.upsample >= 0 && d.upsample <= 6, "igemm: upsample %d", d.upsample);
+    if (merged) {
+        if (d.act_dtype == MVLDM_F32) return set_error(MVLDM_ERR_UNSUPPORTED, "igemm: the merged phase launch (upsample 6) is 16-bit only");
+        if (d.src1 || d.c1) return set_error(MVLDM_ERR_UNSUPPORTED, "igemm: the merged phase launch (upsample 6) takes one source");
+        if (d.splitk > 1) return set_error(MVLDM_ERR_UNSUPPORTED, "igemm: the merged phase launch (upsample 6) runs one K pass (splitk %d)", d.splitk);
+        const int rq = d.tile & 63;
+        if (rq == 11 || rq == 17) return set_error(MVLDM_ERR_UNSUPPORTED, "igemm: the merged phase launch (upsample 6) does not run on the halo tile %d", rq);
+        if (rq >= 12) return set_error(MVLDM_ERR_UNSUPPORTED, "igemm: the merged phase launch (upsample 6) does not run on tile %d (tiles 2, 7, 10)", rq);
+    }
     MVLDM_REQUIRE(phase ? (d.ksize == 2 && d.stride == 1 && d.h_out == d.h_in && d.w_out == d.w_in && !d.src1 && !d.residual &&
                            !d.row_bias && d.act_dtype != MVLDM_F32 && d.dst_dtype == d.act_dtype && d.k_order == 1)
                         : (d.ksize == 1 || d.ksize == 3),
@@ -195,7 +203,8 @@
     p.n_img = d.n_img; p.h_in = d.h_in; p.w_in = d.w_in; p.h_out = d.h_out; p.w_out = d.w_out;
     p.hw_out = d.h_out * d.w_out;
     p.ksize = d.ksize; p.stride = d.stride; p.pad = d.pad; p.upsample = phase ? 0 : d.upsample; p.taps = d.ksize * d.ksize;
-    p.scatter = phase; p.ph_y = phase ? (d.upsample - 2) >> 1 : 0; p.ph_x = phase ? (d.upsample - 2) & 1 : 0;
+    const int ph0 = phase && !merged ? d.upsample - 2 : 0;
+    p.scatter = merged ? 2 : phase; p.ph_y = ph0 >> 1; p.ph_x = ph0 & 1;
     p.ty0 = phase ? p.ph_y - 1 : -d.pad; p.tx0 = phase ? p.ph_x - 1 : -d.pad;
     p.cy = phase ? 1 - p.ph_y : d.ksize / 2; p.cx = phase ? 1 - p.ph_x : d.ksize / 2;
     p.M = d.n_img * p.hw_out; p.n_out = d.n_out; p.n_pad = d.n_pad; p.k_pad = d.k_pad;
@@ -210,15 +219,15 @@
     tile = d.tile & 63;
     t_force_sync = (d.tile >> 12) & 1;
     const int force_px = (d.tile >> 8) & 15;
-    int splitk = d.splitk;
+    int splitk = merged ? 1 : d.splitk;
     MVLDM_REQUIRE(((tile >= 0 && tile <= kNumTiles) || tile == 17 || deep_tile(tile)) && splitk >= 0, "igemm: tile/splitk");
-    choose_config(d, p.M, p.k_tiles, tile, splitk, d.workspace_bytes);
+    choose_config(d, merged ? 4 * p.M : p.M, p.k_tiles, tile, splitk, d.workspace_bytes);
     if (splitk > 1)
         MVLDM_REQUIRE(d.workspace && (size_t)splitk * p.M * d.n_pad * sizeof(float) <= d.workspace_bytes,
                       "igemm: split-K workspace too small");
     const double es = 2.0;
     const double b0 = (double)d.n_img * d.h_in * d.w_in * d.c0 * es, b1 = (double)d.n_img * d.h_in * d.w_in * d.c1 * es;
-    const double bw = (double)d.n_pad * d.k_pad * es;
+    const double bw = (double)d.n_pad * d.k_pad * es * (merged ? 4 : 1);
     p.use_bl = d.act_dtype != MVLDM_F32 && d.k_order == 1 && !t_force_sync && !kEnvSync &&
                b0 < 4.0e9 && b1 < 4.0e9 && bw < 4.0e9;
     if (d.act_dtype != MVLDM_F32 && d.k_order == 1 && !t_force_sync && !kEnvSync && !p.use_bl) {
@@ -229,7 +238,7 @@
                             "64-bit-address loop (split the batch to avoid this)\n", std::max(std::max(b0, b1), bw) / 1e9);
         }
     }
-    p.src0_bytes = (unsigned)b0; p.src1_bytes = (unsigned)b1; p.w_bytes = (unsigned)bw;
+    p.src0_bytes = (unsigned)b0; p.src1_bytes = (unsigned)b1; p.w_bytes = (unsigned)(merged ? bw / 4 : bw);
     p.fake = kEnvFake;
     p.nt_store = stream_stores((size_t)p.M * (size_t)p.n_dst * (p.dst_f32 || d.act_dtype == MVLDM_F32 ? 4 : 2));
     if (kEnvFake & 1) p.src0_bytes = p.src1_bytes = 0;
@@ -264,14 +273,14 @@
         MVLDM_REQUIRE(p.ty0 + p.cy >= 0 && p.tx0 + p.cx >= 0 && hc < d.h_in && wc < d.w_in,
                       "igemm: conv geometry (pad %d, stride %d) not supported", d.pad, d.stride);
     }
-    p.tiles_m = cdiv(p.M, kTiles[tile].bm);
+    p.tiles_m = (merged ? 4 : 1) * cdiv(p.M, kTiles[tile].bm);
     p.tiles_n = cdiv(d.n_pad, kTiles[tile].bn);
     p.korder = d.k_order;
     if (d.k_order)
         MVLDM_REQUIRE(d.k_order == 1 && p.ctot % bk == 0 && d.c0 % bk == 0 && d.k_pad == p.taps * p.ctot,
                       "igemm: k_order 1 needs channel counts (%d,%d) multiples of %d", d.c0, d.c1, bk);
     {
-        const double a_bytes = (double)d.n_img * d.h_in * d.w_in * p.ctot, w_bytes = (double)d.n_pad * d.k_pad;
+        const double a_bytes = (double)d.n_img * d.h_in * d.w_in * p.ctot, w_bytes = (double)d.n_pad * d.k_pad * (merged ? 4 : 1);
         double best = 1e300;
         for (int px = 1; px <= 8; px *= 2) {
             const int py = 8 / px;
@@ -312,6 +321,8 @@
     int tile = 0;
     if (d.n_img == 0 || d.h_out == 0 || d.w_out == 0) return MVLDM_OK;
     const int req = d.tile & 63;
+    if (d.upsample == 6 && req >= 12)
+        return set_error(MVLDM_ERR_UNSUPPORTED, "igemm: the merged phase launch (upsample 6) does not run on tile %d (tiles 2, 7, 10)", req);
     if (req == 15) return skinny_run(d, s);
     if (req == 12 || req == 13 || req == 14 || req == 19) {
         MVLDM_REQUIRE(d.src0 && d.weight && d.dst, "igemm: null pointer");
@@ -353,6 +364,18 @@
     return igemm_run(*d, (hipStream_t)stream);
 }
 
+extern "C" int mvldm_igemm_config(const mvldm_igemm_desc* d, int* tile, int* splitk) {
+    MVLDM_REQUIRE(d != nullptr && tile != nullptr && splitk != nullptr, "igemm_config: null argument");
+    const int req = d->tile & 63;
+    MVLDM_REQUIRE(!(req >= 12 && req <= 15) && req != 19 && d->k_order != 2, "igemm_config: tile %d has its own checks", req);
+    IgemmParams p;
+    int t = 0;
+    if (int rc = fill_params(*d, p, t)) return rc;
+    *tile = t;
+    *splitk = p.splitk;
+    return MVLDM_OK;
+}
+
 extern "C" size_t mvldm_igemm_workspace_bytes(const mvldm_igemm_desc* d) {
     if (!d) return 0;
     const size_t M = (size_t)d->n_img * d->h_out * d->w_out;
diff --git a/mv_ldm_amd/csrc/igemm_bl.h b/mv_ldm_amd/csrc/igemm_bl.h
--- a/mv_ldm_amd/csrc/igemm_bl.h
+++ b/mv_ldm_amd/csrc/igemm_bl.h
@@ -207,8 +207,26 @@
     }
 }
 
+template <int KS>
+__device__ __forceinline__ const IgemmParams& phase_view(const IgemmParams& p, IgemmParams& q, int& tm) {
+    if constexpr (KS != 2) {
+        return p;
+    } else {
+        const int tiles_m_phase = p.scatter == 2 ? p.tiles_m >> 2 : p.tiles_m;
+        const int k = tm / tiles_m_phase;
+        const int ph = 2 * p.ph_y + p.ph_x + k, py = ph >> 1, px = ph & 1;
+        q = p;
+        tm -= k * tiles_m_phase;
+        q.ph_y = py; q.ph_x = px;
+        q.ty0 = py - 1; q.tx0 = px - 1;
+        q.cy = 1 - py; q.cx = 1 - px;
+        q.weight = reinterpret_cast<const char*>(p.weight) + (size_t)k * p.w_bytes;
+        return q;
+    }
+}
+
 template <typename T, int BM, int BN, int WM, int WN, int KS, bool DUAL, int STAGES, bool UPS>
-__global__ __launch_bounds__(WM* WN * 64) void igemm_bl_kernel(const IgemmParams p) {
+__global__ __launch_bounds__(WM* WN * 64) void igemm_bl_kernel(const IgemmParams p_launch) {
     using M_ = Mma<T>;
     static_assert(sizeof(T) == 2, "16-bit activation types only");
     constexpr int NW = WM * WN, TAPS = KS * KS;
@@ -222,7 +240,9 @@
 
     const auto [lane, wave, wm, wn, hi, l31] = wave_lane<WN>();
     int split, tm, tn;
-    if (!map_block(p, split, tm, tn)) return;
+    if (!map_block(p_launch, split, tm, tn)) return;
+    IgemmParams p_phase;
+    const IgemmParams& p = phase_view<KS>(p_launch, p_phase, tm);
     const int cb0 = split * (p.k_tiles_per_split / TAPS);
     const int cb1 = min(cb0 + p.k_tiles_per_split / TAPS, p.k_tiles / TAPS);
 
diff --git a/mv_ldm_amd/csrc/skinny.hip b/mv_ldm_amd/csrc/skinny.hip
--- a/mv_ldm_amd/csrc/skinny.hip
+++ b/mv_ldm_amd/csrc/skinny.hip
@@ -695,6 +695,7 @@
     if (d.act_dtype == MVLDM_F32 || d.k_order != 2) return false;
     if (!(d.ksize == 1 || d.ksize == 3 || (d.ksize == 2 && d.upsample >= 2)) || (d.upsample == 1)) return false;
     if (d.ksize != 2 && d.upsample != 0) return false;
+    if (d.upsample > 5) return false;
     if (d.c0 % 64 || d.c1 % 64 || d.c0 <= 0 || (d.c1 == 0) != (d.src1 == nullptr)) return false;
     if (d.k_pad != d.ksize * d.ksize * (d.c0 + d.c1) || d.n_pad % 64 || d.n_out % 4 || d.n_out > d.n_pad) return false;
     if (d.dst_dtype != d.act_dtype && d.dst_dtype != MVLDM_F32) return false;
diff --git a/mv_ldm_amd/modules.py b/mv_ldm_amd/modules.py
--- a/mv_ldm_amd/modules.py
+++ b/mv_ldm_amd/modules.py
@@ -393,16 +393,17 @@
 
 
 class Upsample2D(nn.Module):
-    def __init__(self, channels, out_channels=None):
+    def __init__(self, channels, out_channels=None, merge_phases=True):
         super().__init__()
         self.conv = Conv2d(channels, out_channels or channels, 3, padding=1)
+        self.merge_phases = merge_phases
 
     def emit(self, b: Builder, x):
         c = x.shape[-1]
         if b.dtype != torch.float32 and c % ops.block_k(b.dtype) == 0 and self.conv.out_channels % 8 == 0:
             pws = self.conv._cache(("wphase", b.dtype), [self.conv.weight],
-                                   lambda: [ops.pack_weight(w, b.dtype) for w in ops.upsample_phase_weights(self.conv.weight)])
-            return b.conv_upsample_phases(x, pws, self.conv._f32("bias"), name="upsample")
+                                   lambda: ops.stack_phase_packs([ops.pack_weight(w, b.dtype) for w in ops.upsample_phase_weights(self.conv.weight)]))
+            return b.conv_upsample_phases(x, pws, self.conv._f32("bias"), name="upsample", merge=self.merge_phases)
         return self.conv.emit(b, x, upsample=True, name="upsample")
 
     def forward(self, x):
diff --git a/mv_ldm_amd/ops.py b/mv_ldm_amd/ops.py
--- a/mv_ldm_amd/ops.py
+++ b/mv_ldm_amd/ops.py
@@ -168,6 +168,9 @@
                bias=None, row_bias=None, residual=None, epilogue=L.EPI_NONE, out_scale=1.0, ws=None, splitk=0,
                tile=0, into=None) -> L.IgemmDesc:
     d = L.IgemmDesc() if into is None else into
+    if int(upsample) == 6:
+        assert phase_packs_contiguous(pw), "the merged phase launch reads four packs that are contiguous in memory (ops.stack_phase_packs)"
+        pw = pw[0]
     c0 = src0.shape[-1]
     c1 = 0 if src1 is None else src1.shape[-1]
     assert c0 + c1 == pw.c_pad, f"weight packed for {pw.c_pad} channels, sources give {c0}+{c1}"
@@ -233,10 +236,42 @@
     return out
 
 
-def conv2d_upsample_phases(x: torch.Tensor, pws, bias=None, tile=0, splitk=0) -> torch.Tensor:
+def phase_packs_contiguous(pws) -> bool:
+    if not isinstance(pws, (list, tuple)) or len(pws) != 4 or len({id(q) for q in pws}) != 4:
+        return False
+    p0 = pws[0]
+    if any((q.n_out, q.n_pad, q.k_pad, q.c_pad, q.ksize, q.k_order, q.data.dtype) != (p0.n_out, p0.n_pad, p0.k_pad, p0.c_pad, p0.ksize, p0.k_order, p0.data.dtype)
+           for q in pws):
+        return False
+    if all(q.data.numel() == 0 for q in pws):
+        return True
+    step = p0.n_pad * p0.k_pad * p0.data.element_size()
+    return all(q.data.is_contiguous() and q.data.numel() == p0.n_pad * p0.k_pad and q.data.data_ptr() == p0.data.data_ptr() + i * step
+               for i, q in enumerate(pws))
+
+
+def stack_phase_packs(pws) -> list:
+    pws = list(pws)
+    if not phase_packs_contiguous(pws):
+        buf = torch.stack([q.data for q in pws])
+        for i, q in enumerate(pws):
+            q.data = buf[i]
+    return pws
+
+
+def pack_upsample_phases(w: torch.Tensor, dtype: torch.dtype) -> list:
+    return stack_phase_packs([pack_weight(t, dtype) for t in upsample_phase_weights(w)])
+
+
+def conv2d_upsample_phases(x: torch.Tensor, pws, bias=None, tile=0, splitk=0, merged=False) -> torch.Tensor:
     n, h, w, _ = x.shape
     out = torch.empty(n, 2 * h, 2 * w, pws[0].n_out, dtype=x.dtype, device=x.device)
     scratch = workspace(min(16 * n * h * w * pws[0].n_pad * 4, 256 << 20), x.device)
+    if merged:
+        d = igemm_desc(x, None, pws, out, n_img=n, h_in=h, w_in=w, h_out=h, w_out=w, stride=1, pad=0, upsample=6,
+                       bias=bias, splitk=splitk or 1, tile=tile, ws=scratch if splitk > 1 else None)
+        L.check(L.load().mvldm_igemm_fwd(C.byref(d), stream()))
+        return out
     for phase, pw in enumerate(pws):
         d = igemm_desc(x, None, pw, out, n_img=n, h_in=h, w_in=w, h_out=h, w_out=w, stride=1, pad=0, upsample=2 + phase,
                        bias=bias, splitk=splitk, tile=tile, ws=scratch)
diff --git a/mv_ldm_amd/plan.py b/mv_ldm_amd/plan.py
--- a/mv_ldm_amd/plan.py
+++ b/mv_ldm_amd/plan.py
@@ -10,7 +10,7 @@
 import torch
 
 from . import _lib as L
-from .ops import PackedWeight, conv_out_hw, dt, igemm_desc, ptr, use_skinny
+from .ops import PackedWeight, conv_out_hw, dt, igemm_desc, phase_packs_contiguous, ptr, use_skinny
 
 
 def _PIN_TILE() -> int:
@@ -194,10 +194,15 @@
         limit = int(os.environ.get("MVLDM_PAR_ROWS", "0"))
         return self.record and rows * max(n_out, 1) <= limit * 640 and limit > 0
 
-    def conv_upsample_phases(self, x, pws, bias=None, name="upsample"):
+    def conv_upsample_phases(self, x, pws, bias=None, name="upsample", merge=True):
         n, h, w, c0 = x.shape
         out = self.empty(n, 2 * h, 2 * w, pws[0].n_out, dtype=x.dtype)
         lanes = self.parallel() if self.small_launch(n * h * w, pws[0].n_out) else None
+        mergeable = merge and lanes is None and self.record and type(self) is Builder and merge_phases_enabled() and phase_packs_contiguous(pws)
+        if mergeable and os.environ.get("MVLDM_AUTOTUNE", "1") == "0" and self._merge_rule(x, pws, bias, out):
+            self._merged_phase_conv(x, pws, bias, out, name)
+            return out
+        first = len(self.ops)
         if lanes is not None:
             lanes.__enter__()
         for phase, pw in enumerate(pws):
@@ -206,7 +211,35 @@
             self._phase_conv(x, pw, bias, out, phase, name)
         if lanes is not None:
             lanes.__exit__(None, None, None)
+        if mergeable:
+            self.__dict__.setdefault("_phase_groups", []).append((self.ops[first:first + 4], list(pws)))
         return out
+
+    def _merge_rule(self, x, pws, bias, out) -> bool:
+        n, h, w, c0 = x.shape
+        pw = pws[0]
+        d = igemm_desc(x, None, pw, out, n_img=n, h_in=h, w_in=w, h_out=h, w_out=w, stride=1, pad=0, upsample=2, bias=bias, ws=self.splitk_ws())
+        lib = L.load()
+        if self.skinny and skinny_candidate(pw, n * h * w, c0, 0, 2, x.dtype) and x.is_cuda and lib.mvldm_igemm_skinny_config(C.byref(d)) > 0 \
+                and skinny_rule(n * h * w, pw.n_pad):
+            return False
+        if not d.weight:
+            d.weight = d.src0
+        tile, splitk = C.c_int(0), C.c_int(0)
+        return lib.mvldm_igemm_config(C.byref(d), C.byref(tile), C.byref(splitk)) == 0 and tile.value in (2, 7, 10) and splitk.value == 1
+
+    def _merged_phase_conv(self, x, pws, bias, out, name, tile=0):
+        n, h, w, c0 = x.shape
+        pw = pws[0]
+        assert pw.ksize == 2 and pw.k_order == 1 and c0 == pw.c_pad
+        m = n * h * w
+        es = x.element_size()
+        nbytes = (4 * pw.n_out * 4 * c0 + m * c0) * es + 4 * m * pw.n_out * es
+        op = L.Op()
+        op.kind = L.OP_IGEMM
+        igemm_desc(x, None, pws, out, n_img=n, h_in=h, w_in=w, h_out=h, w_out=w, stride=1, pad=0, upsample=6, bias=bias, splitk=1, tile=tile,
+                   into=op.u.igemm)
+        self._emit(op, f"{name}.merged", 4 * 2.0 * m * pw.n_out * 4 * c0, nbytes, (x, *(q.data for q in pws), bias, out))
 
     def _phase_conv(self, x, pw, bias, out, phase, name, tile=0, splitk=0):
         n, h, w, c0 = x.shape
@@ -393,12 +426,15 @@
             autotune_wgrad(self.ops)
             if type(self) is Builder and _BATCH_SPLIT:
                 self.ops, self.meta = autosplit_igemm(self.ops, self.meta, skinny=self._skinny_pw, keep=self.keep)
+            if type(self) is Builder and self.__dict__.get("_phase_groups") and merge_phases_enabled():
+                self.ops, self.meta = automerge_phases(self.ops, self.meta, self._phase_groups)
         return Plan(self.ops, self.meta, self.keep, self.device)
 
 
 _TUNE_CACHE = {}
 _WGRAD_CACHE = {}
 _SPLIT_CACHE = {}
+_MERGE_CACHE = {}
 _VALIDATED = set()
 _TUNE_TILES = tuple(int(t) for t in os.environ["MVLDM_TUNE_TILES"].split(",")) if os.environ.get("MVLDM_TUNE_TILES") else (0, 1, 2, 3, 4, 5, 6, 7, 8, 9, 10, 11, 12, 13, 14)
 
@@ -406,7 +442,8 @@
 def tune_cache_state() -> dict:
     return {"version": 2, "igemm": {json.dumps(list(k)): (int(v) if isinstance(v, int) else list(v)) for k, v in _TUNE_CACHE.items()},
             "wgrad": {json.dumps(list(k)): int(v) for k, v in _WGRAD_CACHE.items()},
-            "split": {json.dumps(list(k)): int(v) for k, v in _SPLIT_CACHE.items()}}
+            "split": {json.dumps(list(k)): int(v) for k, v in _SPLIT_CACHE.items()},
+            "merge": {json.dumps(list(k)): int(v) for k, v in _MERGE_CACHE.items()}}
 
 
 def set_tune_cache_state(state: dict, replace: bool = False) -> None:
@@ -414,9 +451,13 @@
         _TUNE_CACHE.clear()
         _WGRAD_CACHE.clear()
         _SPLIT_CACHE.clear()
-    for name, cache in (("igemm", _TUNE_CACHE), ("wgrad", _WGRAD_CACHE), ("split", _SPLIT_CACHE)):
+        _MERGE_CACHE.clear()
+
+    def _key(x):
+        return tuple(_key(e) for e in x) if isinstance(x, list) else x
+    for name, cache in (("igemm", _TUNE_CACHE), ("wgrad", _WGRAD_CACHE), ("split", _SPLIT_CACHE), ("merge", _MERGE_CACHE)):
         for k, v in (state.get(name) or {}).items():
-            cache[tuple(json.loads(k))] = int(v) if isinstance(v, int) else list(v)
+            cache[_key(json.loads(k))] = int(v) if isinstance(v, int) else list(v)
 
 
 def save_tune_cache(path: Optional[str] = None) -> Optional[str]:
@@ -436,7 +477,7 @@
         return 0
     with open(path) as f:
         set_tune_cache_state(json.load(f))
-    return len(_TUNE_CACHE) + len(_WGRAD_CACHE) + len(_SPLIT_CACHE)
+    return len(_TUNE_CACHE) + len(_WGRAD_CACHE) + len(_SPLIT_CACHE) + len(_MERGE_CACHE)
 
 
 def broadcast_tune_cache(dist, src: int = 0, device=None) -> None:
@@ -709,6 +750,70 @@
     return new_ops, new_meta
 
 
+_MERGE_TILES = (2, 7, 10)
+_MERGE_MIN_ROWS = 2048
+
+
+def merge_phases_enabled() -> bool:
+    return os.environ.get("MVLDM_UPSAMPLE_MERGE", "1") != "0"
+
+
+def _merged_op(op0, pws, tile: int):
+    q = L.Op()
+    C.memmove(C.byref(q), C.byref(op0), C.sizeof(L.Op))
+    d = q.u.igemm
+    d.upsample, d.tile, d.splitk = 6, tile, 1
+    d.weight, d.k_order = ptr(pws[0].data), pws[0].k_order
+    d.workspace, d.workspace_bytes = None, 0
+    return q
+
+
+def automerge_phases(ops, meta, groups, iters: int = 6):
+    pos = {id(o): i for i, o in enumerate(ops)}
+    drop, put, decided = set(), {}, 0
+    for four, pws in groups:
+        idx = [pos.get(id(o)) for o in four]
+        if len(four) != 4 or None in idx or idx != list(range(idx[0], idx[0] + 4)):
+            continue
+        d0 = four[0].u.igemm
+        if d0.n_img * d0.h_out * d0.w_out < _MERGE_MIN_ROWS or not phase_packs_contiguous(pws):
+            continue
+        key = _igemm_signature(d0)[:-2] + ("merged",) + tuple((o.u.igemm.tile, o.u.igemm.splitk) for o in four)
+        tile = _MERGE_CACHE.get(key)
+        if tile is None:
+            t_four = _time_ops(four, iters)
+            best_t, tile = None, 0
+            for cand in _MERGE_TILES:
+                try:
+                    t = _time_ops([_merged_op(four[0], pws, cand)], iters)
+                except L.MvldmError:
+                    continue
+                if t < 0.97 * t_four and (best_t is None or t < best_t):
+                    best_t, tile = t, cand
+            if os.environ.get("MVLDM_MERGE_LOG"):
+                print(f"[phase merge] {meta[idx[0]].name}: four launches {t_four * 1e3:.1f} us, merged tile {tile}: "
+                      f"{'-' if best_t is None else round(best_t * 1e3, 1)} us", file=sys.stderr, flush=True)
+            _MERGE_CACHE[key] = tile
+            decided += 1
+        if tile:
+            m0 = meta[idx[0]]
+            name = (m0.name[:-3] if m0.name.endswith(".p0") else m0.name) + ".merged"
+            put[idx[0]] = (_merged_op(four[0], pws, tile),
+                           OpMeta(name, m0.kind, sum(meta[i].flops for i in idx), sum(meta[i].bytes for i in idx)))
+            drop.update(idx[1:])
+    new_ops, new_meta = [], []
+    for i, (o, m) in enumerate(zip(ops, meta)):
+        if i in drop:
+            continue
+        o, m = put.get(i, (o, m))
+        o.tag = len(new_ops)
+        new_ops.append(o)
+        new_meta.append(m)
+    if decided:
+        save_tune_cache()
+    return new_ops, new_meta
+
+
 _WGRAD_TARGETS = tuple(int(t) for t in os.environ.get("MVLDM_TUNE_WGRAD_TARGETS", "0,1,2,3,4,5").split(","))
 
 
diff --git a/mv_ldm_amd/vae.py b/mv_ldm_amd/vae.py
--- a/mv_ldm_amd/vae.py
+++ b/mv_ldm_amd/vae.py
@@ -30,7 +30,7 @@
         super().__init__()
         self.resnets = nn.ModuleList([ResnetBlock2D(in_channels if i == 0 else out_channels, out_channels, None, groups, 1e-6)
                                       for i in range(num_layers)])
-        self.upsamplers = nn.ModuleList([Upsample2D(out_channels, out_channels)]) if add_upsample else None
+        self.upsamplers = nn.ModuleList([Upsample2D(out_channels, out_channels, merge_phases=False)]) if add_upsample else None
 
 
 def _chain(b: Builder, h, mods, prefix, free_first=True):
```

Result: no change. 50.72 (median of 6 runs) (+0.6%).
